# jzr99/Geo4D

Measured on AMD Instinct MI355X. Metric: denoised latent frames/sec (16x320x512, 50-step DDIM), higher is better.
Workload: dtype bf16x3m

## Files before the change

### geo4d_amd/_lib.py

```python
import ctypes as C
import os

import torch

_HERE = os.path.dirname(os.path.abspath(__file__))
LIB_PATH = os.environ.get("GEO4D_HIP_LIB") or os.path.join(_HERE, "csrc", "libgeo4d_hip.so")
ABI_VERSION = 9

F32, BF16, F16, BF16X3, F16X2 = 0, 1, 2, 3, 4


class Geo4DNativeError(RuntimeError):
    pass


class ConvGemm(C.Structure):
    _fields_ = [
        ("A", C.c_void_p), ("W", C.c_void_p), ("O", C.c_void_p),
        ("bias", C.c_void_p), ("rowbias", C.c_void_p), ("R", C.c_void_p),
        ("zeros", C.c_void_p), ("workspace", C.c_void_p), ("workspace_bytes", C.c_size_t),
        ("lda", C.c_long), ("ldw", C.c_long), ("ldo", C.c_long), ("ldr", C.c_long), ("ldrb", C.c_long),
        ("a_bs", C.c_long), ("w_bs", C.c_long), ("o_bs", C.c_long), ("r_bs", C.c_long),
        ("M", C.c_int), ("N", C.c_int), ("K", C.c_int), ("batch", C.c_int),
        ("Cin", C.c_int),
# ... 16 lines not shown
    _fields_ = [("tile_hint", C.c_int), ("generation", C.c_int), ("bm", C.c_int), ("bn", C.c_int), ("wm", C.c_int), ("wn", C.c_int),
                ("geglu", C.c_int)]


class GroupNorm(C.Structure):
    _fields_ = [
        ("x", C.c_void_p), ("y", C.c_void_p), ("gamma", C.c_void_p), ("beta", C.c_void_p),
        ("workspace", C.c_void_p), ("workspace_bytes", C.c_size_t),
        ("ldx", C.c_long), ("ldy", C.c_long),
        ("F", C.c_int), ("HW", C.c_int), ("C", C.c_int), ("groups", C.c_int), ("frames_per_stat", C.c_int),
        ("act", C.c_int), ("dtype", C.c_int), ("eps", C.c_float), ("colsum", C.c_void_p), ("split_out", C.c_int), ("colsum_rows", C.c_int),
        ("sat_count", C.c_void_p),
    ]


class GroupNormSrc(C.Structure):
    _fields_ = [("colsum", C.c_void_p), ("rows", C.c_int), ("c0", C.c_int), ("channels", C.c_int)]


class GroupNorm2(C.Structure):
    _fields_ = [("base", GroupNorm), ("src", GroupNormSrc * 2), ("nsrc", C.c_int), ("path", C.c_int), ("fuse_fraction", C.c_float),
                ("min_workgroups", C.c_int)]


class GroupNormPlan(C.Structure):
    _fields_ = [("path", C.c_int), ("launches", C.c_int), ("rows_per_wg", C.c_int), ("nchunk", C.c_int), ("channel_slices", C.c_int),
                ("stat_slices", C.c_int), ("workspace_bytes", C.c_size_t)]


GN_PATH_AUTO, GN_PATH_PARTIAL, GN_PATH_COLS, GN_PATH_FUSED, GN_PATH_SLICED = 0, 1, 2, 3, 4


class Attention(C.Structure):
    _fields_ = [
        ("q", C.c_void_p), ("o", C.c_void_p),
        ("k", C.c_void_p * 2), ("vt", C.c_void_p * 2), ("zeros", C.c_void_p),
        ("ldq", C.c_long), ("ldo", C.c_long), ("ldk", C.c_long * 2), ("ldvt", C.c_long * 2), ("vt_bs", C.c_long * 2),
        ("Nk", C.c_int * 2), ("kv_div", C.c_int * 2),
        ("B", C.c_int), ("H", C.c_int), ("Nq", C.c_int), ("nseg", C.c_int), ("head_dim", C.c_int), ("dtype", C.c_int),
        ("scale", C.c_float), ("split_out", C.c_int), ("variant", C.c_int), ("qkv_split", C.c_int),
    ]


class AttentionPlan(C.Structure):
    _fields_ = [("kernel", C.c_int), ("nseg", C.c_int), ("qb", C.c_int), ("occ", C.c_int), ("ps", C.c_int), ("rows_per_wg", C.c_int),
                ("grid", C.c_uint * 3), ("variant", C.c_int)]


class Align(C.Structure):
    _fields_ = [
        ("pred", C.c_void_p), ("conf", C.c_void_p), ("logdepth", C.c_void_p), ("cams", C.c_void_p), ("slot_trf", C.c_void_p),
        ("slot_ptr", C.c_void_p), ("slot_idx", C.c_void_p),
        ("grad_logdepth", C.c_void_p), ("img_sums", C.c_void_p), ("slot_sums", C.c_void_p),
        ("workspace", C.c_void_p), ("workspace_bytes", C.c_size_t),
        ("img_part", C.c_void_p), ("slot_part", C.c_void_p),
        ("invdepth", C.c_void_p), ("slot_st", C.c_void_p),
        ("n_imgs", C.c_int), ("n_slots", C.c_int), ("H", C.c_int), ("W", C.c_int), ("chunk_pixels", C.c_int), ("max_slots_per_image", C.c_int),
        ("conf_clamp", C.c_float), ("inv_area", C.c_float), ("depth_weight", C.c_float),
    ]


class AlignSmall(C.Structure):
    _fields_ = [
        ("im_poses", C.c_void_p), ("im_focals", C.c_void_p), ("pw_poses", C.c_void_p), ("cams", C.c_void_p), ("slot_trf", C.c_void_p),
        ("img_sums", C.c_void_p), ("slot_sums", C.c_void_p), ("group_ptr", C.c_void_p), ("group_entries", C.c_void_p), ("group_sums", C.c_void_p),
        ("scale_terms", C.c_void_p),
        ("grad_im_poses", C.c_void_p), ("grad_im_focals", C.c_void_p), ("grad_pw_poses", C.c_void_p), ("grad_s_depth", C.c_void_p),
        ("grad_t_depth", C.c_void_p), ("loss", C.c_void_p),
        ("slot_st", C.c_void_p), ("s_depth", C.c_void_p), ("t_depth", C.c_void_p), ("depth_ok", C.c_void_p),
        ("traj", C.c_void_p), ("traj_align", C.c_void_p), ("traj_valid", C.c_void_p), ("slot_img", C.c_void_p), ("img_slot_ptr", C.c_void_p),
        ("img_slot_idx", C.c_void_p), ("grad_traj", C.c_void_p),
        ("n_imgs", C.c_int), ("n_groups", C.c_int), ("n_slots", C.c_int), ("slots_per_group", C.c_int), ("n_listed_slots", C.c_int),
        ("n_focals", C.c_int), ("norm_pw_scale", C.c_int),
        ("focal_break", C.c_float), ("base_scale", C.c_float), ("ppx", C.c_float), ("ppy", C.c_float), ("smooth_weight", C.c_float),
        ("translation_weight", C.c_float), ("traj_weight", C.c_float),
    ]


SIGNATURES = {
    "geo4d_conv_gemm": (C.c_int, [C.POINTER(ConvGemm), C.c_void_p]),
    "geo4d_conv_gemm_plan": (C.c_int, [C.POINTER(ConvGemm), C.POINTER(ConvGemmPlan)]),
    "geo4d_conv_gemm_tiles": (C.c_int, [C.POINTER(ConvGemmTile), C.c_int]),
    "geo4d_conv_gemm_colsum_rows": (C.c_int, [C.POINTER(ConvGemm)]),
    "geo4d_groupnorm_workspace": (C.c_size_t, [C.c_int, C.c_int, C.c_int, C.c_int]),
    "geo4d_groupnorm": (C.c_int, [C.POINTER(GroupNorm), C.c_void_p]),
    "geo4d_groupnorm_plan": (C.c_int, [C.POINTER(GroupNorm2), C.POINTER(GroupNormPlan)]),
    "geo4d_groupnorm2": (C.c_int, [C.POINTER(GroupNorm2), C.c_void_p]),
    "geo4d_layernorm": (C.c_int, [C.c_void_p, C.c_long, C.c_void_p, C.c_long, C.c_int, C.c_int, C.c_float, C.c_void_p,
                                  C.c_void_p, C.c_int, C.c_void_p]),
    "geo4d_layernorm_split": (C.c_int, [C.c_void_p, C.c_long, C.c_void_p, C.c_long, C.c_int, C.c_int, C.c_float, C.c_void_p,
                                        C.c_void_p, C.c_int, C.c_void_p, C.c_void_p]),
    "geo4d_softmax_rows": (C.c_int, [C.c_void_p, C.c_long, C.c_void_p, C.c_long, C.c_long, C.c_int, C.c_float, C.c_int,
                                     C.c_void_p]),
    "geo4d_softmax_rows_causal": (C.c_int, [C.c_void_p, C.c_long, C.c_void_p, C.c_long, C.c_long, C.c_int, C.c_float, C.c_int,
                                            C.c_int, C.c_void_p]),
    "geo4d_attention_plan": (C.c_int, [C.POINTER(Attention), C.POINTER(AttentionPlan)]),
    "geo4d_attention": (C.c_int, [C.POINTER(Attention), C.c_void_p]),
    "geo4d_temporal_attention": (C.c_int, [C.c_void_p, C.c_long, C.c_void_p, C.c_long, C.c_void_p, C.c_long, C.c_void_p,
                                           C.c_long, C.c_int, C.c_int, C.c_int, C.c_int, C.c_int, C.c_float, C.c_int,
                                           C.c_void_p]),
    "geo4d_temporal_attention2": (C.c_int, [C.c_void_p, C.c_long, C.c_void_p, C.c_long, C.c_void_p, C.c_long, C.c_void_p,
                                            C.c_long, C.c_int, C.c_int, C.c_int, C.c_int, C.c_int, C.c_float, C.c_int,
                                            C.c_int, C.c_void_p]),
    "geo4d_tokens_from_ncthw": (C.c_int, [C.c_void_p, C.c_int, C.c_void_p, C.c_int, C.c_void_p, C.c_int, C.c_int, C.c_int,
                                          C.c_int, C.c_int, C.c_void_p]),
    "geo4d_cast_rows_f16": (C.c_int, [C.c_void_p, C.c_long, C.c_void_p, C.c_long, C.c_long, C.c_int, C.c_void_p, C.c_void_p]),
    "geo4d_split_rows_bf16": (C.c_int, [C.c_void_p, C.c_long, C.c_void_p, C.c_long, C.c_long, C.c_int, C.c_void_p]),
    "geo4d_concat_channels": (C.c_int, [C.c_void_p, C.c_long, C.c_int, C.c_void_p, C.c_long, C.c_int, C.c_void_p, C.c_long,
                                        C.c_long, C.c_int, C.c_void_p]),
    "geo4d_timestep_embedding": (C.c_int, [C.c_void_p, C.c_void_p, C.c_void_p, C.c_int, C.c_int, C.c_void_p]),
    "geo4d_linear_small": (C.c_int, [C.c_void_p, C.c_long, C.c_void_p, C.c_long, C.c_void_p, C.c_void_p, C.c_long,
                                     C.c_void_p, C.c_long, C.c_int, C.c_int, C.c_int, C.c_int, C.c_int, C.c_void_p]),
    "geo4d_ddim_step": (C.c_int, [C.c_void_p, C.c_void_p, C.c_void_p, C.c_void_p, C.c_void_p, C.c_void_p, C.c_long,
                                  C.c_void_p]),
    "geo4d_philox_fill": (C.c_int, [C.c_void_p, C.c_int, C.c_void_p, C.c_int, C.c_long, C.c_void_p, C.c_int, C.c_int, C.c_int, C.c_float,
                                    C.c_void_p]),
    "geo4d_ddim_step_rng": (C.c_int, [C.c_void_p, C.c_void_p, C.c_void_p, C.c_void_p, C.c_void_p, C.c_void_p, C.c_int, C.c_long, C.c_int,
                                      C.c_float, C.c_void_p]),
    "geo4d_cfg_combine_workspace": (C.c_size_t, [C.c_int]),
    "geo4d_cfg_combine": (C.c_int, [C.c_void_p, C.c_void_p, C.c_void_p, C.c_void_p, C.c_int, C.c_long, C.c_float, C.c_float,
                                    C.c_float, C.c_void_p, C.c_size_t, C.c_void_p]),
    "geo4d_embed_tokens": (C.c_int, [C.c_void_p, C.c_void_p, C.c_void_p, C.c_void_p, C.c_long, C.c_long, C.c_int, C.c_int, C.c_int,
                                     C.c_int, C.c_void_p]),
    "geo4d_advance_index": (C.c_int, [C.c_void_p, C.c_int, C.c_void_p]),
    "geo4d_gather_timestep": (C.c_int, [C.c_void_p, C.c_void_p, C.c_void_p, C.c_int, C.c_void_p]),
    "geo4d_plucker_cameras_workspace": (C.c_size_t, [C.c_int, C.c_int, C.c_int]),
    "geo4d_plucker_cameras": (C.c_int, [C.c_void_p, C.c_void_p, C.c_long, C.c_long, C.c_int, C.c_int, C.c_int, C.c_void_p,
                                        C.c_size_t, C.c_void_p, C.c_void_p]),
    "geo4d_align_workspace": (C.c_size_t, [C.c_int, C.c_int, C.c_int, C.c_int, C.c_int]),
    "geo4d_align_residual": (C.c_int, [C.POINTER(Align), C.c_void_p]),
    "geo4d_adam_step": (C.c_int, [C.c_void_p, C.c_void_p, C.c_void_p, C.c_void_p, C.c_long, C.c_float, C.c_float, C.c_float, C.c_float,
                                  C.c_int, C.c_void_p]),
    "geo4d_adam_step_dev": (C.c_int, [C.c_void_p, C.c_void_p, C.c_void_p, C.c_void_p, C.c_long, C.c_void_p, C.c_float, C.c_float, C.c_float,
                                      C.c_void_p]),
    "geo4d_lad_workspace": (C.c_size_t, [C.c_int, C.c_long]),
    "geo4d_lad_target": (C.c_int, [C.c_void_p, C.c_void_p, C.c_void_p, C.c_int, C.c_int, C.c_void_p]),
    "geo4d_lower_median": (C.c_int, [C.c_void_p, C.c_int, C.c_long, C.c_void_p, C.c_void_p, C.c_size_t, C.c_void_p]),
    "geo4d_lad_fit": (C.c_int, [C.c_void_p, C.c_void_p, C.c_int, C.c_long, C.c_void_p, C.c_float, C.c_int, C.c_float, C.c_void_p, C.c_void_p,
                                C.c_void_p, C.c_size_t, C.c_void_p]),
    "geo4d_lad_delta": (C.c_int, [C.c_void_p, C.c_void_p, C.c_void_p, C.c_void_p, C.c_int, C.c_long, C.c_float, C.c_float, C.c_float,
                                  C.c_void_p, C.c_void_p]),
    "geo4d_bicubic_resize": (C.c_int, [C.c_void_p, C.c_void_p, C.c_int, C.c_int, C.c_int, C.c_int, C.c_int, C.c_void_p]),
    "geo4d_masked_select_workspace": (C.c_size_t, [C.c_long]),
    "geo4d_masked_select": (C.c_int, [C.c_void_p, C.c_void_p, C.c_long, C.c_float, C.c_void_p, C.c_float, C.c_float, C.c_void_p, C.c_void_p,
                                      C.c_void_p, C.c_void_p, C.c_size_t, C.c_void_p]),
    "geo4d_depth_metrics_workspace": (C.c_size_t, [C.c_long]),
    "geo4d_depth_metrics": (C.c_int, [C.c_void_p, C.c_void_p, C.c_long, C.c_float, C.c_void_p, C.c_void_p, C.c_float, C.c_float, C.c_float,
                                      C.c_float, C.c_void_p, C.c_void_p, C.c_void_p, C.c_void_p, C.c_size_t, C.c_void_p]),
    "geo4d_scene_clean": (C.c_int, [C.c_void_p, C.c_void_p, C.c_void_p, C.c_void_p, C.c_int, C.c_int, C.c_int, C.c_double, C.c_float, C.c_void_p]),
    "geo4d_scene_points_workspace": (C.c_size_t, [C.c_int, C.c_int, C.c_int]),
    "geo4d_scene_points": (C.c_int, [C.c_void_p, C.c_void_p, C.c_void_p, C.c_int, C.c_int, C.c_int, C.c_void_p, C.c_void_p, C.c_void_p,
                                     C.c_void_p, C.c_size_t, C.c_void_p]),
    "geo4d_scene_mesh_faces_workspace": (C.c_size_t, [C.c_int, C.c_int, C.c_int]),
    "geo4d_scene_mesh_faces": (C.c_int, [C.c_void_p, C.c_int, C.c_int, C.c_int, C.c_void_p, C.c_void_p, C.c_void_p, C.c_size_t, C.c_void_p]),
    "geo4d_focal_shift_workspace": (C.c_size_t, [C.c_int, C.c_int, C.c_int]),
    "geo4d_focal_shift": (C.c_int, [C.c_void_p, C.c_long, C.c_void_p, C.c_long, C.c_float, C.c_void_p, C.c_int, C.c_int, C.c_int, C.c_int,
                                    C.c_int, C.c_int, C.c_void_p, C.c_void_p, C.c_void_p, C.c_void_p, C.c_size_t, C.c_void_p]),
    "geo4d_pnp_ransac_workspace": (C.c_size_t, [C.c_int, C.c_int, C.c_int, C.c_int, C.c_int, C.c_int]),
    "geo4d_pnp_ransac": (C.c_int, [C.c_void_p, C.c_long, C.c_void_p, C.c_long, C.c_float, C.c_void_p, C.c_double, C.c_double, C.c_double,
                                   C.c_int, C.c_int, C.c_void_p, C.c_void_p, C.c_void_p, C.c_void_p, C.c_int, C.c_int, C.c_int, C.c_int,
                                   C.c_int, C.c_void_p, C.c_void_p, C.c_void_p, C.c_void_p, C.c_void_p, C.c_size_t, C.c_void_p]),
    "geo4d_last_error": (C.c_char_p, []),
    "geo4d_align_refresh": (C.c_int, [C.POINTER(AlignSmall), C.c_void_p]),
    "geo4d_align_small_grads": (C.c_int, [C.POINTER(AlignSmall), C.c_void_p]),
    "geo4d_abi_version": (C.c_int, []),
    "geo4d_abi_struct_size": (C.c_size_t, [C.c_int]),
# ... 39 lines not shown
```

### geo4d_amd/csrc/gemm.hip

```cpp
#include "gemm_kernel.h"

namespace geo4d_gemm {
extern template int launch_typed<float>(const geo4d_conv_gemm_t&, const Plan&, hipStream_t);
extern template int launch_typed<bf16_t>(const geo4d_conv_gemm_t&, const Plan&, hipStream_t);
extern template int launch_typed<f16_t>(const geo4d_conv_gemm_t&, const Plan&, hipStream_t);
extern template int launch_typed<bf16x3_t>(const geo4d_conv_gemm_t&, const Plan&, hipStream_t);
extern template int launch_v2_typed<bf16_t>(const geo4d_conv_gemm_t&, const Plan&, hipStream_t);
extern template int launch_v2_typed<bf16x3_t>(const geo4d_conv_gemm_t&, const Plan&, hipStream_t);
extern template int launch_v2_typed<f16x2p_t>(const geo4d_conv_gemm_t&, const Plan&, hipStream_t);
extern template int launch_v3_typed<bf16_t>(const geo4d_conv_gemm_t&, const Plan&, hipStream_t);
extern template int launch_v3_typed<bf16x3_t>(const geo4d_conv_gemm_t&, const Plan&, hipStream_t);
extern template int launch_v3_typed<f16x2p_t>(const geo4d_conv_gemm_t&, const Plan&, hipStream_t);

template <typename T>
static int launch_v23(const geo4d_conv_gemm_t& p, const Plan& plan, hipStream_t s) {
    return generation(plan.hint) == 2 ? launch_v2_typed<T>(p, plan, s) : launch_v3_typed<T>(p, plan, s);
}
}
using namespace geo4d_gemm;

static_assert(MAX_TAPS == MAXTAP, "gemm_plan.h validates the tap count the kernels' gather tables hold");

static int conv_gemm_plan(const geo4d_conv_gemm_t* p, Plan& plan) {
    if (!p) return GEO4D_EINVAL;
    const char* error = validate(*p);
    if (!error) {
        plan = resolve(*p);
        error = plan.error;
    }
    if (error) geo4d_set_error(error);
    return error ? GEO4D_EINVAL : GEO4D_OK;
}

extern "C" int geo4d_conv_gemm(const geo4d_conv_gemm_t* pp, void* stream) {
    Plan plan;
    const int rc = conv_gemm_plan(pp, plan);
    if (rc != GEO4D_OK) return rc;
    const geo4d_conv_gemm_t& p = *pp;
    hipStream_t s = (hipStream_t)stream;
    const bool gen1 = generation(plan.hint) == 1;
    switch (p.dtype) {
        case GEO4D_F32: return launch_typed<float>(p, plan, s);
        case GEO4D_BF16: return gen1 ? launch_typed<bf16_t>(p, plan, s) : launch_v23<bf16_t>(p, plan, s);
        case GEO4D_BF16X3: return gen1 ? launch_typed<bf16x3_t>(p, plan, s) : launch_v23<bf16x3_t>(p, plan, s);
        case GEO4D_F16X2: return launch_v23<f16x2p_t>(p, plan, s);
        default: return launch_typed<f16_t>(p, plan, s);
    }
}

extern "C" int geo4d_conv_gemm_plan(const geo4d_conv_gemm_t* pp, geo4d_conv_gemm_plan_t* out) {
    Plan plan;
    if (!out) return GEO4D_EINVAL;
    const int rc = conv_gemm_plan(pp, plan);
    if (rc != GEO4D_OK) return rc;
    const Tile& t = *find_tile(plan.hint);
    *out = {t.hint, generation(t.hint), t.bm, t.bn, t.wm, t.wn, plan.splits, plan.hot, plan.osplit, plan.colsum_rows};
    return GEO4D_OK;
}

extern "C" int geo4d_conv_gemm_tiles(geo4d_conv_gemm_tile_t* out, int cap) {
    int n = 0;
    for (const Tile& t : TILES) {
        if (out && n < cap) out[n] = {t.hint, generation(t.hint), t.bm, t.bn, t.wm, t.wn, t.geglu()};
        ++n;
    }
    return n;
}

extern "C" int geo4d_conv_gemm_colsum_rows(const geo4d_conv_gemm_t* pp) {
    if (!pp || pp->Hout <= 0 || pp->Wout <= 0) return 0;
    return resolve(*pp).colsum_rows;
}
```

### geo4d_amd/csrc/gemm_epilogue.h

```cpp
#pragma once
#include "common.h"
#include "geo4d_hip.h"

namespace geo4d_gemm {

__device__ __forceinline__ void store_out(void* O, long idx, float v, int dt) {
    if (dt == GEO4D_F32) ((float*)O)[idx] = v;
    else if (dt == GEO4D_BF16) ((unsigned short*)O)[idx] = f32_to_bf16_bits(v);
    else ((unsigned short*)O)[idx] = f32_to_f16_bits(v);
}
__device__ __forceinline__ float load_res(const void* R, long idx, int dt) {
    if (dt == GEO4D_F32) return ((const float*)R)[idx];
    if (dt == GEO4D_BF16) return bf16_bits_to_f32(((const unsigned short*)R)[idx]);
    return f16_bits_to_f32(((const unsigned short*)R)[idx]);
}

struct EpiDest { void* O; long ldo, obase; int odt, oesz, nout; bool geglu; };
__device__ __forceinline__ EpiDest epi_dest(const geo4d_conv_gemm_t& p, const bool partial, const int kz, const long bz) {
    const int odt = partial ? GEO4D_F32 : p.out_dtype;
    void* O = partial ? (void*)((float*)p.workspace + ((long)kz * p.batch + bz) * (long)p.M * p.N) : p.O;
    const bool geglu = !partial && p.act == 2;
    return EpiDest{O, partial ? (long)p.N : p.ldo, partial ? 0 : bz * p.o_bs, odt, odt == GEO4D_F32 ? 4 : 2, geglu ? (p.N >> 1) : p.N, geglu};
}

template <bool GELU = true>
__device__ __forceinline__ float epi_value(const geo4d_conv_gemm_t& p, const float acc, const float brow, const long rboff, const int n, const bool inb = true) {
    float v = acc * p.alpha + brow;
    if (inb) {
        if (p.bias && !p.bias_per_row) v += p.bias[n];
        if (p.rowbias) v += p.rowbias[rboff + n];
    }
    if (p.act == 1) v = silu_f(v);
    else if (GELU && p.act == 3) v = gelu_erf_f(v);
    return v;
}
__device__ __forceinline__ float geglu_value(const float alpha, const float xacc, const float gacc, const float xbias, const float gbias) {
    const float xv = xacc * alpha + xbias;
    const float gv = gacc * alpha + gbias;
    return xv * gelu_erf_f(gv);
}

__device__ __forceinline__ u32x2 pack4_16(const float (&e)[4], const bool isbf) {
    return isbf ? u32x2{f32x2_to_bf16x2(e[0], e[1]), f32x2_to_bf16x2(e[2], e[3])} : u32x2{f32x2_to_f16x2(e[0], e[1]), f32x2_to_f16x2(e[2], e[3])};
}
__device__ __forceinline__ void unpack4_16(const u32x2 r, const bool isbf, float (&f)[4]) {
    if (isbf) {
        f[0] = __uint_as_float(r[0] << 16); f[1] = __uint_as_float(r[0] & 0xffff0000u);
        f[2] = __uint_as_float(r[1] << 16); f[3] = __uint_as_float(r[1] & 0xffff0000u);
    } else {
        f[0] = f16_bits_to_f32((unsigned short)(r[0] & 0xffffu)); f[1] = f16_bits_to_f32((unsigned short)(r[0] >> 16));
        f[2] = f16_bits_to_f32((unsigned short)(r[1] & 0xffffu)); f[3] = f16_bits_to_f32((unsigned short)(r[1] >> 16));
    }
}

constexpr unsigned EPI_OOB = 0x80000000u;
constexpr int EPI_RSRC_FLAGS = 0x00020000;
__device__ __forceinline__ void* uniform_ptr(const void* q) {
    const unsigned long long v = (unsigned long long)q;
    const unsigned lo = __builtin_amdgcn_readfirstlane((unsigned)v), hi = __builtin_amdgcn_readfirstlane((unsigned)(v >> 32));
    return (void*)(((unsigned long long)hi << 32) | lo);
}
__device__ __forceinline__ __amdgpu_buffer_rsrc_t tile_rsrc(const void* corner, const bool present = true) {
    return __builtin_amdgcn_make_buffer_rsrc(uniform_ptr(corner), 0, present ? EPI_OOB : 0u, EPI_RSRC_FLAGS);
}
__device__ __forceinline__ __amdgpu_buffer_rsrc_t bias_rsrc(const geo4d_conv_gemm_t& p, const bool has, const int n_w0) {
    const int nleft = p.N - n_w0;
    return __builtin_amdgcn_make_buffer_rsrc(uniform_ptr(has ? (const void*)(p.bias + n_w0) : p.zeros), 0, (has && nleft > 0) ? (unsigned)nleft * 4u : 0u, EPI_RSRC_FLAGS);
}

struct StoreF32 {
    static constexpr unsigned ES = 4;
    static __device__ __forceinline__ u32x4 pack(const geo4d_conv_gemm_t&, const float (&e)[4]) {
        return u32x4{__float_as_uint(e[0]), __float_as_uint(e[1]), __float_as_uint(e[2]), __float_as_uint(e[3])};
    }
    static __device__ __forceinline__ void store(const u32x4 v, const __amdgpu_buffer_rsrc_t rs, const unsigned off) { __builtin_amdgcn_raw_buffer_store_b128(v, rs, off, 0, 0); }
};
struct StoreSplit {
    static constexpr unsigned ES = 4;
    static __device__ __forceinline__ u32x4 pack(const geo4d_conv_gemm_t&, const float (&e)[4]) {
        unsigned int h0, h1, l0, l1;
        h0 = f32x2_to_bf16x2(e[0], e[1]); h1 = f32x2_to_bf16x2(e[2], e[3]);
        l0 = f32x2_to_bf16x2(e[0] - __uint_as_float(h0 << 16), e[1] - __uint_as_float(h0 & 0xffff0000u));
        l1 = f32x2_to_bf16x2(e[2] - __uint_as_float(h1 << 16), e[3] - __uint_as_float(h1 & 0xffff0000u));
        const u32x2 s0 = __builtin_amdgcn_permlane16_swap(h0, l0, false, false);
        const u32x2 s1 = __builtin_amdgcn_permlane16_swap(h1, l1, false, false);
        return u32x4{s0[0], s1[0], s0[1], s1[1]};
    }
    static __device__ __forceinline__ void store(const u32x4 v, const __amdgpu_buffer_rsrc_t rs, const unsigned off) { __builtin_amdgcn_raw_buffer_store_b128(v, rs, off, 0, 0); }
};
struct StoreRows16 {
    static constexpr unsigned ES = 2;
    static __device__ __forceinline__ bool isbf(const geo4d_conv_gemm_t& p) { return p.out_dtype == GEO4D_BF16; }
    static __device__ __forceinline__ u32x2 pack(const geo4d_conv_gemm_t& p, const float (&e)[4]) { return pack4_16(e, isbf(p)); }
    static __device__ __forceinline__ void store(const u32x2 v, const __amdgpu_buffer_rsrc_t rs, const unsigned off) { __builtin_amdgcn_raw_buffer_store_b64(v, rs, off, 0, 0); }
};
struct StoreF16Sat {
    static constexpr unsigned ES = 2;
    static __device__ __forceinline__ u32x2 pack(const geo4d_conv_gemm_t& p, const float (&e)[4]) {
        count_f16_saturation(p.sat_count, e);
        return pack4_f16_sat(e);
    }
    static __device__ __forceinline__ void store(const u32x2 v, const __amdgpu_buffer_rsrc_t rs, const unsigned off) { __builtin_amdgcn_raw_buffer_store_b64(v, rs, off, 0, 0); }
};

template <int MB, int NB, typename Store>
__device__ __forceinline__ void geglu_fast(const geo4d_conv_gemm_t& p, const f32x4 (&acc)[MB][NB], const void* corner, const long ldo,
// ... 65 lines not shown
```

### geo4d_amd/csrc/gemm_kernel.h

```cpp
#pragma once
#include <type_traits>
#include "common.h"
#include "geo4d_hip.h"
#include "gemm_plan.h"
#include "gemm_epilogue.h"

namespace geo4d_gemm {

constexpr int PITCH = 128;
constexpr int BKC = 8;
constexpr int MAXTAP = 9;
static_assert(BKC * 16 == KSLAB_BYTES, "gemm_plan.h counts K slabs of BKC 16-byte chunks");

template <int BM, int NT>
__device__ __forceinline__ void fill_gather_table(const geo4d_conv_gemm_t& p, const int tm, const int ntap, const int hw, int* rowpix, const int tid) {
    const int hlim = p.ups == 2 ? 2 * p.Hin : p.Hin, wlim = p.ups == 2 ? 2 * p.Win : p.Win;
    const int ush = p.ups == 2 ? 1 : 0;
    for (int e = tid; e < BM * ntap; e += NT) {
        const int row = e / ntap, tap = e - row * ntap;
        const int m = tm * BM + row;
        int pix = -1;
        if (m < p.M) {
            const int f = m / hw, rem = m - f * hw;
            const int oy = rem / p.Wout, ox = rem - oy * p.Wout;
            const int kt = tap / (p.KH * p.KW), r2 = tap - kt * (p.KH * p.KW);
            const int ky = r2 / p.KW, kx = r2 - ky * p.KW;
            const int iy = oy * p.stride - p.ph + ky, ix = ox * p.stride - p.pw + kx;
            const int tt = (f % p.T) + kt - p.pt;
            if ((unsigned)iy < (unsigned)hlim && (unsigned)ix < (unsigned)wlim && (unsigned)tt < (unsigned)p.T)
                pix = ((f + kt - p.pt) * p.Hin + (iy >> ush)) * p.Win + (ix >> ush);
        }
        rowpix[e] = pix;
    }
}
template <int HOT> __device__ __forceinline__ bool a_is_split(const geo4d_conv_gemm_t& p) { return HOT ? (HOT == 2) : (p.a_split != 0); }
template <int HOT> __device__ __forceinline__ bool w_is_split(const geo4d_conv_gemm_t& p) { return HOT ? true : (p.w_split != 0); }

template <int BM, int BN, int WM, int WN, int ST>
constexpr int stage_bytes() {
    constexpr int ring = ST * (BM + BN) * PITCH;
    constexpr int epi = WM * WN * 32 * ((((BN / WN / 32) % 2 == 0) ? 64 : 32) + 4) * 4;
    return ring > epi ? ring : epi;
}
template <int BM, int BN, int WM, int WN, int ST>
constexpr int smem_bytes() {
    return stage_bytes<BM, BN, WM, WN, ST>() + BM * MAXTAP * 4;
}

template <typename T, int BM, int BN, int WM, int WN, int ST, int HOT = 0>
__global__ __launch_bounds__(WM * WN * 64) void conv_gemm_kernel(const geo4d_conv_gemm_t p) {
    constexpr int NT = WM * WN * 64;
    constexpr int EPC = Elem<T>::EPC;
    constexpr int BK = BKC * EPC;
    constexpr int MB = BM / WM / 32, NB = BN / WN / 32;
    constexpr int ACH = BM * BKC / NT, BCH = BN * BKC / NT;
    constexpr int RSTEP = NT / 8;
    constexpr int WTM = MB * 32, WTN = NB * 32;
    constexpr int CG = (NB % 2 == 0) ? 64 : 32;
    constexpr int NG = WTN / CG;
    constexpr int SP = CG + 4;
    static_assert(WM * WN == 4 || WM * WN == 5 || WM * WN == 8 || WM * WN == 10, "4, 5, 8 or 10 waves");
    static_assert((BM * BKC) % NT == 0 && (BN * BKC) % NT == 0 && (NT / 8) % 2 == 0, "staging passes must tile the panel");
    static_assert(MB >= 1 && NB >= 1 && ACH >= 1 && BCH >= 1, "tile too small");
    extern __shared__ __attribute__((aligned(16))) char smem[];
    int* rowpix = (int*)(smem + stage_bytes<BM, BN, WM, WN, ST>());

    const int tid = threadIdx.x, lane = tid & 63, wave = tid >> 6;
    const int li = lane & 31, g = lane >> 5;
    const int wr = wave / WN, wc = wave % WN;
    const long lid = xcd_remap((long)blockIdx.x, (long)gridDim.x);
    const int tiles_n = (p.N + BN - 1) / BN;
    const int tm = (int)(lid / tiles_n), tn = (int)(lid - (long)tm * tiles_n);
    const long bz = blockIdx.y;
    const int kz = blockIdx.z;
    const T* __restrict__ A = (const T*)p.A + bz * p.a_bs;
    const T* __restrict__ W = (const T*)p.W + bz * p.w_bs;
    const int ntap = p.KT * p.KH * p.KW;
    const int hw = p.Hout * p.Wout;

    const bool direct_rows = ntap == 1 && p.stride == 1 && p.ups == 1 && p.ph == 0 && p.pw == 0 && p.pt == 0 &&
                             p.Hin * p.Win == hw;
    if (!direct_rows) {
        fill_gather_table<BM, NT>(p, tm, ntap, hw, rowpix, tid);
        __syncthreads();
    }

    const int ccol = tid & 7;
    const int r0 = tid >> 3;
    const int csrc = (ccol ^ ((r0 >> 1) & 7)) * EPC;
    constexpr bool SWZ_CONST = ((RSTEP / 2) % 8) == 0;
    auto csrc_of = [&](int i) { return SWZ_CONST ? csrc : (ccol ^ (((r0 + i * RSTEP) >> 1) & 7)) * EPC; };
    const T* __restrict__ Z = (const T*)p.zeros;
    const T* wptr[BCH];
#pragma unroll
    for (int i = 0; i < BCH; ++i) {
        const int n = tn * BN + r0 + i * RSTEP;
        wptr[i] = n < p.N ? W + (long)n * p.ldw + csrc_of(i) : nullptr;
    }

    const int nslab_all = p.K / BK;
    const int per = (nslab_all + (int)gridDim.z - 1) / (int)gridDim.z;
    const int s_begin = kz * per;
    const int s_end = min(nslab_all, s_begin + per);
    const int nslab = s_end - s_begin;

    int pix[ACH];
    int tap = s_begin % ntap;
    int c0 = (s_begin / ntap) * BK;
    auto fetch_pix = [&]() {
        if (direct_rows) {
#pragma unroll
            for (int i = 0; i < ACH; ++i) {
                const int m = tm * BM + r0 + i * RSTEP;
                pix[i] = m < p.M ? m : -1;
            }
            return;
// ... 367 lines not shown
    }
    const long rboff = p.rowbias ? (long)(m / p.rowbias_div) * (p.ldrb ? p.ldrb : (long)p.N) : 0;
#pragma unroll
    for (int j = 0; j < 8; ++j) {
        float v = e[j] * p.alpha;
        if (p.bias) v += p.bias[n + j];
        if (p.rowbias) v += p.rowbias[rboff + n + j];
        if (p.R) v += ((const float*)p.R)[(long)m * p.ldr + n + j];
        e[j] = v;
    }
    *(f32x4*)((float*)p.O + (long)m * p.ldo + n) = f32x4{e[0], e[1], e[2], e[3]};
    *(f32x4*)((float*)p.O + (long)m * p.ldo + n + 4) = f32x4{e[4], e[5], e[6], e[7]};
    float q[8];
#pragma unroll
    for (int j = 0; j < 8; ++j) q[j] = e[j] * e[j];
#pragma unroll
    for (int o = CG; o < 64; o <<= 1) {
#pragma unroll
        for (int j = 0; j < 8; ++j) { e[j] += __shfl_xor(e[j], o); q[j] += __shfl_xor(q[j], o); }
    }
    if (lane < CG) {
#pragma unroll
        for (int j = 0; j < 8; ++j) { part[wave][lane * 8 + j][0] = e[j]; part[wave][lane * 8 + j][1] = q[j]; }
    }
    __syncthreads();
    if (tid < CG * 8) {
        float s0 = part[0][tid][0], s1 = part[0][tid][1];
        for (int w2 = 1; w2 < 4; ++w2) { s0 += part[w2][tid][0]; s1 += part[w2][tid][1]; }
        float* dst = p.gn_colsum + ((long)bm * p.N + bn * CG * 8 + tid) * 2;
        dst[0] = s0; dst[1] = s1;
    }
}
template <typename T, bool COLSUM = true>
int launch_splitk_reduce(const geo4d_conv_gemm_t& p, const Plan& plan, hipStream_t stream) {
    if constexpr (COLSUM) {
        if (p.gn_colsum) {
            if (plan.colsum_rows == 32) hipLaunchKernelGGL((splitk_reduce_colsum_kernel<T, 32>), dim3((unsigned)((p.M / 32) * (p.N / 64))), dim3(256), 0, stream, p, plan.splits);
            else hipLaunchKernelGGL((splitk_reduce_colsum_kernel<T, 8>), dim3((unsigned)((p.M / 8) * (p.N / 256))), dim3(256), 0, stream, p, plan.splits);
            GEO4D_CHECK_LAUNCH();
            return GEO4D_OK;
        }
    }
    const long tot = (long)p.batch * p.M * (p.N / 8);
    hipLaunchKernelGGL(splitk_reduce_kernel<T>, dim3((unsigned)((tot + 255) / 256)), dim3(256), 0, stream, p, plan.splits);
    GEO4D_CHECK_LAUNCH();
    return GEO4D_OK;
}

template <typename T, int BM, int BN, int WM, int WN, int ST, int HOT>
int launch_kernel(const geo4d_conv_gemm_t& p, int splits, hipStream_t stream) {
    constexpr int smem = smem_bytes<BM, BN, WM, WN, ST>();
    static bool attr_set = false;
    auto kern = conv_gemm_kernel<T, BM, BN, WM, WN, ST, HOT>;
    if (!attr_set) {
        if (hipFuncSetAttribute((const void*)kern, hipFuncAttributeMaxDynamicSharedMemorySize, smem) != hipSuccess) {
            geo4d_set_error("hipFuncSetAttribute(max dynamic LDS) failed");
            return GEO4D_EIO;
        }
        attr_set = true;
    }
    const long tiles = (long)((p.M + BM - 1) / BM) * ((p.N + BN - 1) / BN);
    dim3 grid((unsigned)tiles, (unsigned)p.batch, (unsigned)splits);
    hipLaunchKernelGGL(kern, grid, dim3(WM * WN * 64), smem, stream, p);
    GEO4D_CHECK_LAUNCH();
    return GEO4D_OK;
}

template <typename T, int BM, int BN, int WM, int WN, int ST>
int launch_cfg(const geo4d_conv_gemm_t& p, const Plan& plan, hipStream_t stream) {
    int rc;
    if constexpr (IsX3<T>::value) {
        if (plan.hot == 1) rc = launch_kernel<T, BM, BN, WM, WN, ST, 1>(p, plan.splits, stream);
        else if (plan.hot == 2) rc = launch_kernel<T, BM, BN, WM, WN, ST, 2>(p, plan.splits, stream);
        else rc = launch_kernel<T, BM, BN, WM, WN, ST, 0>(p, plan.splits, stream);
    } else {
        rc = launch_kernel<T, BM, BN, WM, WN, ST, 0>(p, plan.splits, stream);
    }
    if (rc != GEO4D_OK || plan.splits == 1) return rc;
    return launch_splitk_reduce<T, false>(p, plan, stream);
}

template <typename T> int launch_v2_typed(const geo4d_conv_gemm_t& p, const Plan& plan, hipStream_t stream);
template <typename T> int launch_v3_typed(const geo4d_conv_gemm_t& p, const Plan& plan, hipStream_t stream);

template <typename T>
int launch_typed(const geo4d_conv_gemm_t& p, const Plan& plan, hipStream_t stream) {
    switch (plan.hint) {
        case 1: return launch_cfg<T, 128, 128, 2, 2, 2>(p, plan, stream);
        case 2: return launch_cfg<T, 128, 64, 4, 1, 2>(p, plan, stream);
        case 3: return launch_cfg<T, 64, 128, 2, 2, 2>(p, plan, stream);
        case 4: return launch_cfg<T, 64, 64, 2, 2, 2>(p, plan, stream);
        case 5: return launch_cfg<T, 128, 32, 4, 1, 2>(p, plan, stream);
        case 11: return launch_cfg<T, 256, 128, 4, 2, 2>(p, plan, stream);
        case 13: return launch_cfg<T, 256, 256, 4, 2, 2>(p, plan, stream);
        case 16: return launch_cfg<T, 160, 320, 5, 2, 2>(p, plan, stream);
        case 17: return launch_cfg<T, 160, 160, 5, 1, 2>(p, plan, stream);
    }
    geo4d_set_error("conv_gemm: unknown tile_hint");
    return GEO4D_EINVAL;
}

}
```

### geo4d_amd/csrc/gemm_kernel_v2.h

```cpp
#pragma once
#include "gemm_kernel.h"

namespace geo4d_gemm {

template <typename T> __device__ __forceinline__ void mma16(f32x4& acc, const u32x4& a, const u32x4& b);
template <> __device__ __forceinline__ void mma16<bf16_t>(f32x4& acc, const u32x4& a, const u32x4& b) {
    acc = __builtin_amdgcn_mfma_f32_16x16x32_bf16(__builtin_bit_cast(bf16x8_t, a), __builtin_bit_cast(bf16x8_t, b), acc, 0, 0, 0);
}
template <> __device__ __forceinline__ void mma16<f16_t>(f32x4& acc, const u32x4& a, const u32x4& b) {
    acc = __builtin_amdgcn_mfma_f32_16x16x32_f16(__builtin_bit_cast(f16x8_t, a), __builtin_bit_cast(f16x8_t, b), acc, 0, 0, 0);
}
__device__ __forceinline__ void mma16_x3(f32x4& acc, const u32x4& ah, const u32x4& al, const u32x4& bh, const u32x4& bl) {
    acc = __builtin_amdgcn_mfma_f32_16x16x32_bf16(__builtin_bit_cast(bf16x8_t, al), __builtin_bit_cast(bf16x8_t, bh), acc, 0, 0, 0);
    acc = __builtin_amdgcn_mfma_f32_16x16x32_bf16(__builtin_bit_cast(bf16x8_t, ah), __builtin_bit_cast(bf16x8_t, bl), acc, 0, 0, 0);
    acc = __builtin_amdgcn_mfma_f32_16x16x32_bf16(__builtin_bit_cast(bf16x8_t, ah), __builtin_bit_cast(bf16x8_t, bh), acc, 0, 0, 0);
}

__device__ __forceinline__ void mma16_x2(f32x4& acc, const u32x4& bh, const u32x4& bl, const u32x4& ah) {
    acc = __builtin_amdgcn_mfma_f32_16x16x32_f16(__builtin_bit_cast(f16x8_t, bl), __builtin_bit_cast(f16x8_t, ah), acc, 0, 0, 0);
    acc = __builtin_amdgcn_mfma_f32_16x16x32_f16(__builtin_bit_cast(f16x8_t, bh), __builtin_bit_cast(f16x8_t, ah), acc, 0, 0, 0);
}

template <typename T> __device__ __forceinline__ int swz_key(int row) {
    const int p = (row >> 1) & 7;
    if constexpr (IsX3<T>::value) return p ^ ((((p >> 2) ^ (p >> 1)) & 1) << 1);
    else return p;
}

template <typename T> __device__ __forceinline__ void frag_offsets(const int lr, const int lq, int (&foff)[2]) {
    const int fkey = swz_key<T>(lr);
    if constexpr (IsX3<T>::value) {
        foff[0] = lr * PITCH + (((2 * lq) ^ fkey) << 4);
        foff[1] = lr * PITCH + (((2 * lq + 1) ^ fkey) << 4);
    } else {
        foff[0] = lr * PITCH + ((lq ^ fkey) << 4);
        foff[1] = lr * PITCH + (((4 + lq) ^ fkey) << 4);
    }
}

__device__ __forceinline__ void tile_of(long t, int tiles_n, int tiles_mn, int group_m, int& tm, int& tn) {
    const int tiles_m = tiles_mn / tiles_n;
    if (group_m <= 1 || tiles_n < 2 || tiles_m < 2) {
        tm = (int)(t / tiles_n);
        tn = (int)(t - (long)tm * tiles_n);
        return;
    }
    const int per_band = group_m * tiles_n;
    const int band = (int)(t / per_band);
    const int first_m = band * group_m;
    const int rows = min(tiles_m - first_m, group_m);
    const int r = (int)(t - (long)band * per_band);
    tn = r / rows;
    tm = first_m + (r - tn * rows);
}
__device__ __forceinline__ int tile_group_m(const geo4d_conv_gemm_t& p) { return (p.debug_ablate >= 16 && p.debug_ablate < 48) ? p.debug_ablate - 16 : 1; }

__device__ __forceinline__ int swz_key_a64(int row) { return (4 - ((row >> 2) & 3)) & 3; }
constexpr int PITCH_A64 = 64;

__device__ __forceinline__ float row16_sum(float v) {
    v += __int_as_float(__builtin_amdgcn_mov_dpp(__float_as_int(v), 0xB1, 0xF, 0xF, true));
    v += __int_as_float(__builtin_amdgcn_mov_dpp(__float_as_int(v), 0x4E, 0xF, 0xF, true));
    v += __int_as_float(__builtin_amdgcn_mov_dpp(__float_as_int(v), 0x141, 0xF, 0xF, true));
    v += __int_as_float(__builtin_amdgcn_mov_dpp(__float_as_int(v), 0x140, 0xF, 0xF, true));
    return v;
}
template <int MB, int NB, typename Store>
__device__ __forceinline__ void wide_plain(const geo4d_conv_gemm_t& p, const f32x4 (&acc)[MB][NB], const EpiDest& d, const bool partial, const bool has_res, const long rbase,
                                           const int m_w0, const int n_w0, const int lr, const int lq) {
    constexpr unsigned OOB = EPI_OOB;
    const long ldo = d.ldo;
    const float alpha = partial ? 1.0f : p.alpha;
    const bool hb = !partial && p.bias != nullptr && !p.bias_per_row;
    const bool hr = !partial && p.bias != nullptr && p.bias_per_row;
    const bool ht = !partial && p.rowbias != nullptr;
    const __amdgpu_buffer_rsrc_t rsO = tile_rsrc((float*)d.O + d.obase + (long)m_w0 * ldo + n_w0);
    const __amdgpu_buffer_rsrc_t rsR = tile_rsrc(has_res ? (const void*)((const float*)p.R + rbase + (long)m_w0 * p.ldr + n_w0) : p.zeros, has_res);
    const int mleft = p.M - m_w0;
    const __amdgpu_buffer_rsrc_t rsB = bias_rsrc(p, hb, n_w0);
    const __amdgpu_buffer_rsrc_t rsBr = __builtin_amdgcn_make_buffer_rsrc(
        uniform_ptr(hr ? (const void*)(p.bias + m_w0) : p.zeros), 0, (hr && mleft > 0) ? (unsigned)mleft * 4u : 0u, EPI_RSRC_FLAGS);
    const __amdgpu_buffer_rsrc_t rsT = tile_rsrc(ht ? (const void*)(p.rowbias + n_w0) : p.zeros, ht);
    const unsigned offO = (unsigned)(lr * (int)ldo + 4 * lq) * 4u, offR = (unsigned)(lr * (int)p.ldr + 4 * lq) * 4u;
    const unsigned rowO = (unsigned)ldo * 64u, rowR = (unsigned)p.ldr * 64u;
    const bool gn = !partial && p.gn_colsum != nullptr && m_w0 < p.M;
    const __amdgpu_buffer_rsrc_t rsC = tile_rsrc(gn ? (const void*)(p.gn_colsum + ((long)(m_w0 / (16 * MB)) * p.N + n_w0) * 2) : p.zeros, gn);
    unsigned offT[MB];
#pragma unroll
    for (int a = 0; a < MB; ++a) offT[a] = 0u;
    if (ht) {
        const unsigned ldt = (unsigned)(p.ldrb ? p.ldrb : (long)p.N);
#pragma unroll
        for (int a = 0; a < MB; ++a) {
            const int m = m_w0 + a * 16 + lr;
            offT[a] = ((unsigned)((m < p.M ? m : p.M - 1) / p.rowbias_div) * ldt + 4u * lq) * 4u;
        }
    }
#pragma unroll
    for (int b = 0; b < NB; ++b) {
        const bool colok = n_w0 + 16 * b + 4 * lq < p.N;
        const u32x4 bcu = __builtin_amdgcn_raw_buffer_load_b128(rsB, (unsigned)(4 * lq) * 4u + 64u * b, 0, 0);
        u32x4 ru = __builtin_amdgcn_raw_buffer_load_b128(rsR, ((colok && m_w0 + lr < p.M) ? offR : OOB) + 64u * b, 0, 0);
        u32x4 tu = __builtin_amdgcn_raw_buffer_load_b128(rsT, (colok ? offT[0] : OOB) + 64u * b, 0, 0);
        unsigned bru = __builtin_amdgcn_raw_buffer_load_b32(rsBr, (unsigned)lr * 4u, 0, 0);
        float cs[4] = {0.f, 0.f, 0.f, 0.f}, cq[4] = {0.f, 0.f, 0.f, 0.f};
#pragma unroll
        for (int a = 0; a < MB; ++a) {
            const bool ok = colok && m_w0 + a * 16 + lr < p.M;
            const float brow = __uint_as_float(bru);
            float e[4];
#pragma unroll
            for (int j = 0; j < 4; ++j)
                e[j] = (((acc[a][b][j] * alpha + brow) + __uint_as_float(bcu[j])) + __uint_as_float(tu[j])) + __uint_as_float(ru[j]);
            if (gn) {
#pragma unroll
                for (int j = 0; j < 4; ++j) { cs[j] += e[j]; cq[j] += e[j] * e[j]; }
            }
            const u32x4 c = Store::pack(p, e);
            if (a + 1 < MB) {
                ru = __builtin_amdgcn_raw_buffer_load_b128(rsR, ((colok && m_w0 + (a + 1) * 16 + lr < p.M) ? offR : OOB) + 64u * b, (a + 1) * rowR, 0);
                tu = __builtin_amdgcn_raw_buffer_load_b128(rsT, (colok ? offT[a + 1 < MB ? a + 1 : a] : OOB) + 64u * b, 0, 0);
                bru = __builtin_amdgcn_raw_buffer_load_b32(rsBr, (unsigned)(lr + 16 * (a + 1)) * 4u, 0, 0);
            }
            Store::store(c, rsO, (ok ? offO + a * rowO : OOB) + 64u * b);
        }
        if (gn) {
#pragma unroll
            for (int j = 0; j < 4; ++j) { cs[j] = row16_sum(cs[j]); cq[j] = row16_sum(cq[j]); }
            const unsigned offC = (lr == 0 && colok) ? (unsigned)(16 * b + 4 * lq) * 8u : OOB;
            __builtin_amdgcn_raw_buffer_store_b128(u32x4{__float_as_uint(cs[0]), __float_as_uint(cq[0]), __float_as_uint(cs[1]), __float_as_uint(cq[1])}, rsC, offC, 0, 0);
            __builtin_amdgcn_raw_buffer_store_b128(u32x4{__float_as_uint(cs[2]), __float_as_uint(cq[2]), __float_as_uint(cs[3]), __float_as_uint(cq[3])}, rsC, offC + 16u, 0, 0);
        }
    }
}

template <bool OSPLIT>
__device__ __forceinline__ void store4_generic(const EpiDest& d, const bool vec_ok, const long row, const int col, const float (&e)[4]) {
    const long oidx = row + col;
    if (!vec_ok) {
#pragma unroll
        for (int j = 0; j < 4; ++j) store_out(d.O, oidx + j, e[j], d.odt);
        return;
    }
    if constexpr (OSPLIT) store_split4((float*)d.O + row, col >> 2, e);
    else if (d.odt == GEO4D_F32) *(f32x4*)((float*)d.O + oidx) = f32x4{e[0], e[1], e[2], e[3]};
    else *(u32x2*)((unsigned short*)d.O + oidx) = pack4_16(e, d.odt == GEO4D_BF16);
}

template <int MB, int NB, bool OSPLIT>
__device__ __forceinline__ void generic_rows(const geo4d_conv_gemm_t& p, const f32x4 (&acc)[MB][NB], const EpiDest& d, const bool partial, const bool vec_ok,
                                             const bool has_res, const long rbase, const int m_w0, const int n_w0, const int lr, const int lq) {
    const int odt = d.odt;
#pragma unroll
    for (int a = 0; a < MB; ++a) {
        const int m = m_w0 + a * 16 + lr;
        if (m >= p.M) continue;
        const float brow = (!partial && p.bias && p.bias_per_row) ? p.bias[m] : 0.f;
        const long rboff = (!partial && p.rowbias) ? (long)(m / p.rowbias_div) * (p.ldrb ? p.ldrb : (long)p.N) : 0;
        const long orow = d.obase + (long)m * d.ldo;
        if (d.geglu) {
            if constexpr (NB % 4 == 0) {
#pragma unroll
                for (int b = 0; b < NB; ++b) {
                    if ((b & 3) >= 2) continue;
                    const int n = n_w0 + 16 * b + 4 * lq;
                    if (n + 32 >= p.N) continue;
                    const int oc = (n_w0 >> 1) + 32 * (b >> 2) + 16 * (b & 1) + 4 * lq;
                    float e[4];
#pragma unroll
                    for (int j = 0; j < 4; ++j)
                        e[j] = geglu_value(p.alpha, acc[a][b][j], acc[a][b + 2 < NB ? b + 2 : b][j], p.bias ? p.bias[n + j] : 0.f, p.bias ? p.bias[n + 32 + j] : 0.f);
                    store4_generic<OSPLIT>(d, vec_ok, orow, oc, e);
                }
            }
            continue;
        }
#pragma unroll
        for (int b = 0; b < NB; ++b) {
            const int n = n_w0 + 16 * b + 4 * lq;
            if (n >= p.N) continue;
            float e[4];
#pragma unroll
            for (int j = 0; j < 4; ++j) e[j] = acc[a][b][j];
            if (!partial) {
#pragma unroll
                for (int j = 0; j < 4; ++j) e[j] = epi_value(p, e[j], brow, rboff, n + j, n + j < p.N);
            }
            if (vec_ok) {
                if (has_res) {
                    if (odt == GEO4D_F32) {
                        const f32x4 r = *(const f32x4*)((const float*)p.R + rbase + (long)m * p.ldr + n);
#pragma unroll
                        for (int j = 0; j < 4; ++j) e[j] += r[j];
                    } else {
                        float rf[4];
                        unpack4_16(*(const u32x2*)((const unsigned short*)p.R + rbase + (long)m * p.ldr + n), odt == GEO4D_BF16, rf);
#pragma unroll
                        for (int j = 0; j < 4; ++j) e[j] += rf[j];
                    }
                }
                store4_generic<OSPLIT>(d, true, orow, n, e);
            } else {
#pragma unroll
                for (int j = 0; j < 4; ++j) {
                    if (n + j >= p.N) continue;
                    float v = e[j];
                    if (has_res) v += load_res(p.R, rbase + (long)m * p.ldr + n + j, odt);
                    store_out(d.O, orow + n + j, v, odt);
                }
            }
        }
    }
}

template <typename T, int MB, int NB, bool OSPLIT, bool VECONLY = false>
__device__ __forceinline__ void reg_epilogue(const geo4d_conv_gemm_t& p, const f32x4 (&acc)[MB][NB], const int m_w0, const int n_w0,
                                             const long e_bz, const int e_kz, const bool partial, const int lr, const int lq) {
    const EpiDest d = epi_dest(p, partial, e_kz, e_bz);
    const int odt = d.odt, oesz = d.oesz;
    const bool geglu = d.geglu;
    const bool has_res = !partial && p.R != nullptr;
    const long rbase = e_bz * p.r_bs;
    const bool vec_ok = VECONLY || ((d.nout & 3) == 0 && (d.ldo & 3) == 0 && (((uintptr_t)d.O + d.obase * oesz) % (4 * oesz)) == 0 &&
                                    (!has_res || ((p.ldr & 3) == 0 && (((uintptr_t)p.R + rbase * oesz) % (4 * oesz)) == 0)));
    if constexpr (OSPLIT && IsTwoPass<T>::value) {
        const unsigned short* corner = (unsigned short*)p.O + e_bz * p.o_bs + (long)m_w0 * p.ldo + (geglu ? (n_w0 >> 1) : n_w0);
        if (geglu) geglu_fast<MB, NB, StoreF16Sat>(p, acc, corner, p.ldo, m_w0, n_w0, lr, lq);
        else plain_fast16<MB, NB, false, StoreF16Sat>(p, acc, corner, p.ldo, nullptr, false, m_w0, n_w0, lr, lq);
        return;
    }
    using Wide = std::conditional_t<OSPLIT, StoreSplit, StoreF32>;
    const bool wide = vec_ok && odt == GEO4D_F32;
    if (wide && !geglu && (partial || p.act == 0)) return wide_plain<MB, NB, Wide>(p, acc, d, partial, has_res, rbase, m_w0, n_w0, lr, lq);
    if (wide && geglu) return geglu_fast<MB, NB, Wide>(p, acc, (float*)d.O + d.obase + (long)m_w0 * d.ldo + (n_w0 >> 1), d.ldo, m_w0, n_w0, lr, lq);
    if constexpr (!IsX3<T>::value) {
        const unsigned short* row0 = (unsigned short*)d.O + d.obase + (long)m_w0 * d.ldo;
        if (vec_ok && odt != GEO4D_F32 && !geglu && p.act == 0 && !p.rowbias && !(p.bias && p.bias_per_row))
            return plain_fast16<MB, NB, true, StoreRows16>(p, acc, row0 + n_w0, d.ldo, (const unsigned short*)p.R + rbase + (long)m_w0 * p.ldr + n_w0, has_res, m_w0, n_w0, lr, lq);
        if (vec_ok && odt != GEO4D_F32 && geglu) return geglu_fast<MB, NB, StoreRows16>(p, acc, row0 + (n_w0 >> 1), d.ldo, m_w0, n_w0, lr, lq);
    }
    generic_rows<MB, NB, OSPLIT>(p, acc, d, partial, vec_ok, has_res, rbase, m_w0, n_w0, lr, lq);
}

template <int BM, int BN>
constexpr int v2_smem_bytes() { return (2 * BM + 2 * BN) * PITCH + BM * MAXTAP * 4; }

template <typename T, int BM, int BN, int WM, int WN, int HOT, bool OSPLIT = false>
__global__ __launch_bounds__(WM * WN * 64) void conv_gemm_v2_kernel(const geo4d_conv_gemm_t p, const int splits, const int tiles_mn) {
    constexpr int NT = WM * WN * 64;
    constexpr int EPC = Elem<T>::EPC;
    constexpr int BK = BKC * EPC;
    constexpr int WTM = BM / WM, WTN = BN / WN;
    constexpr int MB = WTM / 16, NB = WTN / 16;
    constexpr int RSTEP = NT / 8;
    constexpr bool A64 = IsTwoPass<T>::value;
    constexpr int RSTEP_A = A64 ? NT / 4 : RSTEP;
    constexpr int ACH = (BM + RSTEP_A - 1) / RSTEP_A, BCH = (BN + RSTEP - 1) / RSTEP;
    constexpr int RING = (2 * BM + 2 * BN) * PITCH;
    static_assert(BM % (WM * 16) == 0 && BN % (WN * 16) == 0 && BM % 8 == 0 && BN % 8 == 0, "wave tiles are multiples of 16");
    static_assert(!std::is_same<T, float>::value, "v2 serves the 16-bit MFMA forms (bf16, bf16x3)");
    extern __shared__ __attribute__((aligned(16))) char smem[];
    int* rowpix = (int*)(smem + RING);

    const int tid = threadIdx.x, lane = tid & 63, wave = tid >> 6;
    const int lr = lane & 15, lq = lane >> 4;
    const int wr = wave / WN, wc = wave % WN;
    const int tiles_n = (p.N + BN - 1) / BN;
    const int ntap = p.KT * p.KH * p.KW;
    const int hw = p.Hout * p.Wout;
    const long total = (long)tiles_mn * p.batch * splits;
    const long G = gridDim.x;
    const bool direct_rows = ntap == 1 && p.stride == 1 && p.ups == 1 && p.ph == 0 && p.pw == 0 && p.pt == 0 && p.Hin * p.Win == hw;
    const int nslab_all = p.K / BK;
    const int per = (nslab_all + splits - 1) / splits;
    const T* __restrict__ Z = (const T*)p.zeros;
    const int ccol = tid & 7;
    const int r0 = tid >> 3;
    const int r0a = A64 ? (tid >> 2) : r0;

    int tm = 0, tn = 0, kz = 0, nslab = 0, tap = 0, c0 = 0, tapB = 0, c0B = 0;
    long bz = 0;
    const T* __restrict__ A = nullptr;
    int pix[ACH];
    const T* wptr[BCH];
    int cA[ACH], cB[BCH];
#pragma unroll
    for (int i = 0; i < ACH; ++i)
        cA[i] = A64 ? ((tid & 3) ^ swz_key_a64(r0a + i * RSTEP_A)) * 16
                    : (ccol ^ swz_key<T>(r0 + i * RSTEP)) * EPC;
#pragma unroll
    for (int i = 0; i < BCH; ++i) cB[i] = (ccol ^ swz_key<T>(r0 + i * RSTEP)) * EPC;

    auto fetch_pix = [&]() {
#pragma unroll
        for (int i = 0; i < ACH; ++i) {
            const int row = r0a + i * RSTEP_A;
            if (direct_rows) {
                const int m = tm * BM + row;
                pix[i] = (row < BM && m < p.M) ? m : -1;
            } else {
                pix[i] = row < BM ? rowpix[row * ntap + tap] : -1;
            }
        }
    };
    auto setup_tile = [&](long w) {
        const long t = w % tiles_mn, rest = w / tiles_mn;
        bz = rest % p.batch;
        kz = (int)(rest / p.batch);
        tile_of(t, tiles_n, tiles_mn, tile_group_m(p), tm, tn);
        A = A64 ? (const T*)((const char*)p.A + bz * p.a_bs * 2) : (const T*)p.A + bz * p.a_bs;
        const T* __restrict__ W = (const T*)p.W + bz * p.w_bs;
#pragma unroll
        for (int i = 0; i < BCH; ++i) {
            const int row = r0 + i * RSTEP, n = tn * BN + row;
            wptr[i] = (row < BN && n < p.N) ? W + (long)n * p.ldw + cB[i] : nullptr;
        }
        const int s_begin = kz * per;
        nslab = min(nslab_all, s_begin + per) - s_begin;
        if (!direct_rows) {
            fill_gather_table<BM, NT>(p, tm, ntap, hw, rowpix, tid);
            __syncthreads();
        }
        tap = tapB = s_begin % ntap;
        c0 = c0B = (s_begin / ntap) * BK;
        fetch_pix();
    };
    auto issue_A = [&](int ab) {
        char* base = smem + ab * BM * PITCH + wave * 1024;
#pragma unroll
        for (int j = 0; j < ACH; ++j) {
            if ((ACH * RSTEP_A == BM) || (wave * (A64 ? 16 : 8) + j * RSTEP_A < BM)) {
                const T* src = pix[j] < 0 ? Z : A64 ? (const T*)((const char*)A + ((long)pix[j] * p.lda + c0) * 2 + cA[j]) : A + (long)pix[j] * p.lda + c0 + cA[j];
                __builtin_amdgcn_global_load_lds((const __attribute__((address_space(1))) void*)src,
                                                 (__attribute__((address_space(3))) void*)(base + j * RSTEP * PITCH), 16, 0, 0);
            }
        }
        if (++tap == ntap) { tap = 0; c0 += BK; }
        if (ntap > 1 && c0 < p.Cin) fetch_pix();
    };
    auto issue_B = [&](int bb) {
        char* base = smem + (2 * BM + bb * BN) * PITCH + wave * 1024;
#pragma unroll
        for (int i = 0; i < BCH; ++i) {
            if ((BCH * RSTEP == BN) || (wave * 8 + i * RSTEP < BN)) {
                const T* src = wptr[i] ? wptr[i] + (long)tapB * p.Cin + c0B : Z;
                __builtin_amdgcn_global_load_lds((const __attribute__((address_space(1))) void*)src,
                                                 (__attribute__((address_space(3))) void*)(base + i * RSTEP * PITCH), 16, 0, 0);
            }
        }
        if (++tapB == ntap) { tapB = 0; c0B += BK; }
    };
    f32x4 acc[MB][NB];
    int foff[2];
    frag_offsets<T>(lr, lq, foff);
    const bool a_split = a_is_split<HOT>(p), w_split = w_is_split<HOT>(p);
    auto compute_slab = [&](int buf) {
        const char* abase = smem + (buf * BM + wr * WTM) * PITCH;
        const char* bbase = smem + (2 * BM + buf * BN + wc * WTN) * PITCH;
        if constexpr (IsTwoPass<T>::value) {
            u32x4 ah[MB];
            const char* abase64 = smem + buf * BM * PITCH + (wr * WTM) * PITCH_A64 + lr * PITCH_A64 + ((lq ^ swz_key_a64(lr)) << 4);
#pragma unroll
            for (int a = 0; a < MB; ++a) ah[a] = *(const u32x4*)(abase64 + a * 16 * PITCH_A64);
#pragma unroll
            for (int b = 0; b < NB; ++b) {
                const u32x4 bh = *(const u32x4*)(bbase + b * 16 * PITCH + foff[0]);
                const u32x4 bl = *(const u32x4*)(bbase + b * 16 * PITCH + foff[1]);
#pragma unroll
                for (int a = 0; a < MB; ++a) mma16_x2(acc[a][b], bh, bl, ah[a]);
            }
        } else if constexpr (IsX3<T>::value) {
            u32x4 ah[MB], al[MB];
#pragma unroll
            for (int a = 0; a < MB; ++a) {
                const u32x4 x0 = *(const u32x4*)(abase + a * 16 * PITCH + foff[0]);
                const u32x4 x1 = *(const u32x4*)(abase + a * 16 * PITCH + foff[1]);
                if (a_split) { ah[a] = x0; al[a] = x1; }
                else split8_bf16(x0, x1, ah[a], al[a]);
            }
#pragma unroll
            for (int b = 0; b < NB; ++b) {
                const u32x4 y0 = *(const u32x4*)(bbase + b * 16 * PITCH + foff[0]);
                const u32x4 y1 = *(const u32x4*)(bbase + b * 16 * PITCH + foff[1]);
                u32x4 bh, bl;
                if (w_split) { bh = y0; bl = y1; }
                else split8_bf16(y0, y1, bh, bl);
#pragma unroll
                for (int a = 0; a < MB; ++a) mma16_x3(acc[a][b], bh, bl, ah[a], al[a]);
            }
        } else {
#pragma unroll
            for (int h = 0; h < 2; ++h) {
                u32x4 fa[MB];
#pragma unroll
                for (int a = 0; a < MB; ++a) fa[a] = *(const u32x4*)(abase + a * 16 * PITCH + foff[h]);
#pragma unroll
                for (int b = 0; b < NB; ++b) {
                    const u32x4 fb = *(const u32x4*)(bbase + b * 16 * PITCH + foff[h]);
#pragma unroll
                    for (int a = 0; a < MB; ++a) mma16<T>(acc[a][b], fb, fa[a]);
                }
            }
        }
    };

    const bool partial = splits > 1;
    auto epilogue = [&](int e_tm, int e_tn, long e_bz, int e_kz) {
        reg_epilogue<T, MB, NB, OSPLIT>(p, acc, e_tm * BM + wr * WTM, e_tn * BN + wc * WTN, e_bz, e_kz, partial, lr, lq);
    };

    long w = xcd_remap((long)blockIdx.x, G);
    if (w >= total) return;
    setup_tile(w);
    auto prologue = [&]() {
        if (nslab > 0) { issue_A(0); issue_B(0); }
    };
    prologue();
    while (true) {
#pragma unroll
        for (int a = 0; a < MB; ++a)
#pragma unroll
            for (int b = 0; b < NB; ++b) acc[a][b] = f32x4{0.f, 0.f, 0.f, 0.f};
        const int ns = nslab;
        asm volatile("s_waitcnt vmcnt(0)" ::: "memory");
        __syncthreads();
        for (int s = 0; s < ns; ++s) {
            const int buf = s & 1;
            if (s + 1 < ns) { issue_A(buf ^ 1); issue_B(buf ^ 1); }
            compute_slab(buf);
            asm volatile("s_waitcnt vmcnt(0)" ::: "memory");
            __syncthreads();
        }
        const int e_tm = tm, e_tn = tn, e_kz = kz;
        const long e_bz = bz;
        const long wn = w + G;
        const bool more = wn < total;
        if (more) {
            setup_tile(wn);
            prologue();
        }
        epilogue(e_tm, e_tn, e_bz, e_kz);
        if (!more) break;
        w = wn;
    }
}

struct GenV2 {
    template <typename T, int BM, int BN, int WM, int WN, int HOT, bool OSPLIT>
    static auto kernel() { return conv_gemm_v2_kernel<T, BM, BN, WM, WN, HOT, OSPLIT>; }
    template <int BM, int BN> static constexpr int smem() { return v2_smem_bytes<BM, BN>(); }
};

template <typename G, typename T, int BM, int BN, int WM, int WN, int HOT, bool OSPLIT = false>
int launch_persistent(const geo4d_conv_gemm_t& p, const Plan& plan, hipStream_t stream) {
    constexpr int smem = G::template smem<BM, BN>();
    static_assert(smem <= 160 * 1024, "LDS");
    static int resident = 0;
    auto kern = G::template kernel<T, BM, BN, WM, WN, HOT, OSPLIT>();
    if (!resident) {
        if (hipFuncSetAttribute((const void*)kern, hipFuncAttributeMaxDynamicSharedMemorySize, smem) != hipSuccess) {
            geo4d_set_error("hipFuncSetAttribute(max dynamic LDS) failed");
            return GEO4D_EIO;
        }
        int dev = 0, cus = 0, occ = 0;
        if (hipGetDevice(&dev) != hipSuccess || hipDeviceGetAttribute(&cus, hipDeviceAttributeMultiprocessorCount, dev) != hipSuccess ||
            hipOccupancyMaxActiveBlocksPerMultiprocessor(&occ, (const void*)kern, WM * WN * 64, smem) != hipSuccess || cus <= 0 || occ <= 0) {
            geo4d_set_error("conv_gemm: occupancy query failed");
            return GEO4D_EIO;
        }
        resident = cus * occ;
    }
    const int tiles_mn = ((p.M + BM - 1) / BM) * ((p.N + BN - 1) / BN);
    const long total = (long)tiles_mn * p.batch * plan.splits;
    const long cap = p.debug_ablate == 2 ? 3 : resident;
    const unsigned grid = (unsigned)(total < cap ? total : cap);
    hipLaunchKernelGGL(kern, dim3(grid), dim3(WM * WN * 64), smem, stream, p, plan.splits, tiles_mn);
    GEO4D_CHECK_LAUNCH();
    if (plan.splits > 1) return launch_splitk_reduce<T>(p, plan, stream);
    return GEO4D_OK;
}

template <typename G, typename T, int BM, int BN, int WM, int WN>
int launch_persistent_cfg(const geo4d_conv_gemm_t& p, const Plan& plan, hipStream_t stream) {
    if constexpr (IsX3<T>::value) {
        if (plan.osplit) return launch_persistent<G, T, BM, BN, WM, WN, 2, true>(p, plan, stream);
        if (plan.hot == 2) return launch_persistent<G, T, BM, BN, WM, WN, 2>(p, plan, stream);
        if constexpr (!IsTwoPass<T>::value) {
            if (plan.hot == 1) return launch_persistent<G, T, BM, BN, WM, WN, 1>(p, plan, stream);
        }
    }
    if constexpr (!IsTwoPass<T>::value) return launch_persistent<G, T, BM, BN, WM, WN, 0>(p, plan, stream);
    return GEO4D_EINVAL;
}

template <typename T>
int launch_v2_typed(const geo4d_conv_gemm_t& p, const Plan& plan, hipStream_t stream) {
    if constexpr (std::is_same<T, bf16_t>::value || IsX3<T>::value) {
        switch (plan.hint) {
            case 22:
                if constexpr (IsTwoPass<T>::value) break;
                else return launch_persistent_cfg<GenV2, T, 256, 256, 4, 2>(p, plan, stream);
            case 23: return launch_persistent_cfg<GenV2, T, 160, 320, 2, 4>(p, plan, stream);
            case 25: return launch_persistent_cfg<GenV2, T, 128, 128, 2, 2>(p, plan, stream);
            case 27: return launch_persistent_cfg<GenV2, T, 64, 128, 2, 2>(p, plan, stream);
            case 28: return launch_persistent_cfg<GenV2, T, 64, 64, 2, 2>(p, plan, stream);
        }
    }
    geo4d_set_error("conv_gemm: no second-generation kernel for this tile_hint and element type");
    return GEO4D_EINVAL;
}

}
```

### geo4d_amd/csrc/gemm_kernel_v3.h

```cpp
#pragma once
#include "gemm_kernel_v2.h"

namespace geo4d_gemm {

template <int BM, int BN>
constexpr int v3_smem_bytes() { return 2 * (BM + BN) * PITCH; }

#define GEO4D_V3_BAR()                          \
    do {                                        \
        __builtin_amdgcn_sched_barrier(0);      \
        __builtin_amdgcn_s_barrier();           \
        __builtin_amdgcn_sched_barrier(0);      \
    } while (0)

template <typename T, int BM, int BN, int WM, int WN, int HOT, bool OSPLIT = false>
__global__ __launch_bounds__(512) void conv_gemm_v3_kernel(const geo4d_conv_gemm_t p, const int splits, const int tiles_mn) {
    static_assert(WM * WN == 8, "two groups of four waves");
    static_assert(!std::is_same<T, float>::value, "v3 serves the 16-bit MFMA forms (bf16, bf16x3)");
    constexpr int EPC = Elem<T>::EPC;
    constexpr int BK = BKC * EPC;
    constexpr int WTM = BM / WM, WTN = BN / WN;
    constexpr int MB = WTM / 16, NB = WTN / 16;
    constexpr int MB0 = (MB + 1) / 2, MB1 = MB - MB0, NB0 = (NB + 1) / 2, NB1 = NB - NB0;
    static_assert(BM % (WM * 16) == 0 && BN % (WN * 16) == 0 && MB1 >= 1 && NB1 >= 1, "wave tiles of at least 32 x 32");
    constexpr int RA0 = WM * MB0 * 16, RA1 = WM * MB1 * 16, RB0 = WN * NB0 * 16, RB1 = WN * NB1 * 16;
    constexpr bool A64 = IsTwoPass<T>::value;
    constexpr int PITCH_A = A64 ? PITCH_A64 : PITCH, RPA = A64 ? 128 : 64, RWA = A64 ? 16 : 8;
    constexpr int OA0 = 0, OA1 = RA0 * PITCH_A, OB0 = BM * PITCH, OB1 = (BM + RB0) * PITCH;
    constexpr int STAGE = (BM + BN) * PITCH;
    constexpr int PA0 = (RA0 + RPA - 1) / RPA, PA1 = (RA1 + RPA - 1) / RPA, PB0 = (RB0 + 63) / 64, PB1 = (RB1 + 63) / 64;
    constexpr int CA0 = RA0 / RPA, CA1 = RA1 / RPA, CB0 = RB0 / 64, CB1 = RB1 / 64;
    constexpr int NWAIT = CA0 + CA1 + CB0 + CB1;
    extern __shared__ __attribute__((aligned(16))) char smem[];

    const int tid = threadIdx.x, lane = tid & 63;
    const int wave = __builtin_amdgcn_readfirstlane(tid >> 6);
    const int lr = lane & 15, lq = lane >> 4;
    const int wr = wave / WN, wc = wave % WN;
    const int tiles_n = (p.N + BN - 1) / BN;
    const int ntap = p.KT * p.KH * p.KW;
    const int hw = p.Hout * p.Wout;
    const long total = (long)tiles_mn * p.batch * splits;
    const long G = gridDim.x;
    const bool direct_rows = ntap == 1 && p.stride == 1 && p.ups == 1 && p.ph == 0 && p.pw == 0 && p.pt == 0 && p.Hin * p.Win == hw;
    const int ns = p.K / BK / splits;
    const int ccol = tid & 7;
    const int r0 = tid >> 3;
    const int r0a = A64 ? (tid >> 2) : r0;

    constexpr unsigned OOB = 0x80000000u;
    constexpr int ESZ = 16 / EPC;
    constexpr int ESZ_A = A64 ? 2 : ESZ;
    auto tile_row = [&](int r, int rows, int per_wave, int wt, int off) { return r < rows ? (r / per_wave) * wt + off + r % per_wave : -1; };
    auto rowA = [&](int h, int j) { return h ? tile_row(r0a + RPA * j, RA1, MB1 * 16, WTM, MB0 * 16) : tile_row(r0a + RPA * j, RA0, MB0 * 16, WTM, 0); };
    auto rowB = [&](int h, int j) { return h ? tile_row(r0 + 64 * j, RB1, NB1 * 16, WTN, NB0 * 16) : tile_row(r0 + 64 * j, RB0, NB0 * 16, WTN, 0); };
    auto chunk = [&](int j) { return (ccol ^ swz_key<T>(r0 + 64 * j)) * EPC; };
    auto chunkA = [&](int j) { return A64 ? ((tid & 3) ^ swz_key_a64(r0a + RPA * j)) * 8 : chunk(j); };
    const int khw = p.KH * p.KW;

    long wS = 0;
    bool validS = false;
    int tmS = 0, tnS = 0, kzS = 0;
    long bzS = 0;
    unsigned voffA[2][PA0], maskA[2][PA0];
    unsigned voffB[2][PB0];
    __amdgpu_buffer_rsrc_t rA = __builtin_amdgcn_make_buffer_rsrc((void*)p.zeros, 0, 0, 0x00020000);
    __amdgpu_buffer_rsrc_t rB = rA;
    int ktA = 0, kyA = 0, kxA = 0, c0A = 0, tapB = 0, c0B = 0, tap_beg = 0, c0_beg = 0;
    unsigned soffA = 0, bitA = 0, soffB = 0;
    auto refresh_A = [&]() {
        soffA = __builtin_amdgcn_readfirstlane((unsigned)((((long)ktA * p.Hin + kyA) * p.Win + kxA) * p.lda + c0A) * ESZ_A);
        bitA = __builtin_amdgcn_readfirstlane((unsigned)((ktA * p.KH + kyA) * p.KW + kxA));
    };
    auto refresh_B = [&]() { soffB = __builtin_amdgcn_readfirstlane((unsigned)(tapB * p.Cin + c0B) * ESZ); };
    auto begin_A = [&]() {
        ktA = tap_beg / khw;
        const int r2 = tap_beg - ktA * khw;
        kyA = r2 / p.KW;
        kxA = r2 - kyA * p.KW;
        c0A = c0_beg;
        refresh_A();
    };
    auto step_A = [&]() {
        if (++kxA == p.KW) {
            kxA = 0;
            if (++kyA == p.KH) {
                kyA = 0;
                if (++ktA == p.KT) {
                    ktA = 0;
                    c0A += BK;
                }
            }
        }
        refresh_A();
    };
    auto step_B = [&]() {
        if (++tapB == ntap) {
            tapB = 0;
            c0B += BK;
        }
        refresh_B();
    };
    auto tap0_pixel = [&](int m) -> long {
        const int f = m / hw, rem = m - f * hw;
        const int oy = rem / p.Wout, ox = rem - oy * p.Wout;
        return ((long)(f - p.pt) * p.Hin + (oy * p.stride - p.ph)) * p.Win + (ox * p.stride - p.pw);
    };
    auto window_A = [&](bool valid, int tm_, long bz_) {
        const long P0 = valid ? tap0_pixel(tm_ * BM) : 0;
        rA = __builtin_amdgcn_make_buffer_rsrc((void*)((const char*)p.A + (bz_ * p.a_bs + P0 * p.lda) * ESZ_A), 0, OOB, 0x00020000);
#pragma unroll
        for (int h = 0; h < 2; ++h) {
#pragma unroll
            for (int j = 0; j < (h ? PA1 : PA0); ++j) {
                const int row = rowA(h, j);
                const int m = tm_ * BM + row;
                unsigned off = 0, mask = 0;
                if (valid && row >= 0 && m < p.M) {
                    const int f = m / hw, rem = m - f * hw;
                    const int oy = rem / p.Wout, ox = rem - oy * p.Wout;
                    const int iy0 = oy * p.stride - p.ph, ix0 = ox * p.stride - p.pw, ft = (f % p.T) - p.pt;
                    const long px0 = ((long)(f - p.pt) * p.Hin + iy0) * p.Win + ix0;
                    off = (unsigned)(((px0 - P0) * p.lda + chunkA(j)) * ESZ_A);
                    unsigned bit = 1;
                    for (int kt = 0; kt < p.KT; ++kt)
                        for (int ky = 0; ky < p.KH; ++ky)
                            for (int kx = 0; kx < p.KW; ++kx, bit <<= 1)
                                if ((unsigned)(ft + kt) < (unsigned)p.T && (unsigned)(iy0 + ky) < (unsigned)p.Hin && (unsigned)(ix0 + kx) < (unsigned)p.Win)
                                    mask |= bit;
                }
                voffA[h][j] = off;
                maskA[h][j] = mask;
            }
        }
    };
    auto stage_tile = [&](long w_) {
        wS = w_;
        validS = w_ < total;
        if (!validS) {
#pragma unroll
            for (int h = 0; h < 2; ++h)
#pragma unroll
                for (int j = 0; j < PB0; ++j) voffB[h][j] = OOB;
            return;
        }
        const long t = w_ % tiles_mn, rest = w_ / tiles_mn;
        bzS = rest % p.batch;
        kzS = (int)(rest / p.batch);
        tile_of(t, tiles_n, tiles_mn, tile_group_m(p), tmS, tnS);
        rB = __builtin_amdgcn_make_buffer_rsrc((void*)((const T*)p.W + bzS * p.w_bs + (long)tnS * BN * p.ldw), 0, OOB, 0x00020000);
#pragma unroll
        for (int h = 0; h < 2; ++h) {
#pragma unroll
            for (int j = 0; j < (h ? PB1 : PB0); ++j) {
                const int row = rowB(h, j);
                voffB[h][j] = (row >= 0 && tnS * BN + row < p.N) ? (unsigned)(((long)row * p.ldw + chunk(j)) * ESZ) : OOB;
            }
        }
        const int s_begin = kzS * ns;
        tap_beg = s_begin % ntap;
        c0_beg = (s_begin / ntap) * BK;
    };
    auto issue_A = [&](auto hc, int st) {
        constexpr int H = decltype(hc)::value;
        constexpr int R = H ? RA1 : RA0;
        char* base = smem + st * STAGE + (H ? OA1 : OA0) + wave * 1024;
#pragma unroll
        for (int j = 0; j < (H ? PA1 : PA0); ++j) {
            if ((j + 1) * RPA <= R || wave * RWA + j * RPA < R) {
                const unsigned v = ((maskA[H][j] >> bitA) & 1u) ? voffA[H][j] : OOB;
                __builtin_amdgcn_raw_ptr_buffer_load_lds(rA, (__attribute__((address_space(3))) void*)(base + j * RPA * PITCH_A), 16, (int)v, (int)soffA, 0, 0);
            }
        }
    };
    auto issue_B = [&](auto hc, int st) {
        constexpr int H = decltype(hc)::value;
        constexpr int R = H ? RB1 : RB0;
        char* base = smem + st * STAGE + (H ? OB1 : OB0) + wave * 1024;
#pragma unroll
        for (int j = 0; j < (H ? PB1 : PB0); ++j) {
            if ((j + 1) * 64 <= R || wave * 8 + j * 64 < R)
                __builtin_amdgcn_raw_ptr_buffer_load_lds(rB, (__attribute__((address_space(3))) void*)(base + j * 64 * PITCH), 16, (int)voffB[H][j], (int)soffB, 0, 0);
        }
    };
    int sA = 0, sB = 0;
    auto advance_B = [&]() {
        if (++sB == ns) {
            sB = 0;
            stage_tile(wS + G);
            tapB = tap_beg;
            c0B = c0_beg;
            refresh_B();
        } else {
            step_B();
        }
    };
    auto advance_A = [&]() {
        if (++sA == ns) {
            sA = 0;
            window_A(validS, tmS, bzS);
            begin_A();
        } else {
            step_A();
        }
// ... 83 lines not shown
        } else {
#pragma unroll
            for (int h = 0; h < 2; ++h) {
#pragma unroll
                for (int b = 0; b < NBH; ++b) {
#pragma unroll
                    for (int a = 0; a < MBH; ++a) mma16<T>(acc[AO + a][BO + b], fb[HB][h][b], fa[HA][h][a]);
                }
            }
        }
    };
    using H0 = std::integral_constant<int, 0>;
    using H1 = std::integral_constant<int, 1>;
    const bool partial = splits > 1;

    const long w0 = xcd_remap((long)blockIdx.x, G);
    if (w0 >= total) return;
    stage_tile(w0);
    window_A(true, tmS, bzS);
    begin_A();
    tapB = tap_beg;
    c0B = c0_beg;
    refresh_B();
    issue_A(H0{}, 0);
    issue_B(H0{}, 0);
    issue_B(H1{}, 0);
    advance_B();
    issue_A(H1{}, 0);
    advance_A();
    issue_A(H0{}, 1);
    issue_B(H1{}, 1);
    issue_B(H0{}, 1);
    advance_B();
    int tmC = tmS, tnC = tnS, kzC = kzS;
    long bzC = bzS;
    asm volatile("s_waitcnt vmcnt(%0)" ::"n"(NWAIT) : "memory");
    __syncthreads();
    read_A(H0{}, smem);
    read_B(H0{}, smem);

    while (true) {
#pragma unroll
        for (int a = 0; a < MB; ++a)
#pragma unroll
            for (int b = 0; b < NB; ++b) acc[a][b] = f32x4{0.f, 0.f, 0.f, 0.f};
        auto slab = [&](auto xc) __attribute__((always_inline)) {
            constexpr int X = decltype(xc)::value, Y = 1 - X;
            using HX = std::integral_constant<int, X>;
            using HY = std::integral_constant<int, Y>;
            const char* sb = smem + X * STAGE;
            const char* so = smem + Y * STAGE;
            auto phase = [&](auto jc, auto issue, auto read, auto split, auto mma, auto after) __attribute__((always_inline)) {
                constexpr int J = decltype(jc)::value;
                constexpr int NW = J == 2 ? 2 * (X ? CB1 : CB0) + CA1 + CA0 : NWAIT;
                issue();
                read();
                split();
                mma();
                after();
                asm volatile("s_waitcnt vmcnt(%0)" ::"n"(NW) : "memory");
            };
            phase(std::integral_constant<int, 0>{}, [&] { issue_A(H1{}, Y); }, [&] { read_B(HY{}, sb); },
                  [&] { split_A(H0{}); split_B(HX{}); }, [&] { mma_quadrant(H0{}, HX{}); }, [&] { advance_A(); });
            GEO4D_V3_BAR();
            phase(std::integral_constant<int, 1>{}, [&] { issue_A(H0{}, X); }, [&] { read_A(H1{}, sb); },
                  [&] { split_B(HY{}); }, [&] { mma_quadrant(H0{}, HY{}); }, [&] {});
            GEO4D_V3_BAR();
            phase(std::integral_constant<int, 2>{}, [&] { issue_B(HX{}, X); }, [&] { read_A(H0{}, so); },
                  [&] { split_A(H1{}); }, [&] { mma_quadrant(H1{}, HY{}); }, [&] {});
            GEO4D_V3_BAR();
            phase(std::integral_constant<int, 3>{}, [&] { issue_B(HY{}, X); }, [&] { read_B(HY{}, so); },
                  [&] {}, [&] { mma_quadrant(H1{}, HX{}); }, [&] { advance_B(); });
        };
        for (int t = 0; t < ns; t += 2) {
            slab(H0{});
            GEO4D_V3_BAR();
            slab(H1{});
            if (t + 2 < ns) GEO4D_V3_BAR();
        }
        GEO4D_V3_BAR();
        {
            int lr_ = lr, lq_ = lq;
            asm volatile("" : "+v"(lr_), "+v"(lq_));
            reg_epilogue<T, MB, NB, OSPLIT, true>(p, acc, tmC * BM + wr * WTM, tnC * BN + wc * WTN, bzC, kzC, partial, lr_, lq_);
        }
        __builtin_amdgcn_s_waitcnt(0x0F70);
        if (!validS) break;
        tmC = tmS; tnC = tnS; kzC = kzS; bzC = bzS;
    }
    asm volatile("s_waitcnt vmcnt(0)" ::: "memory");
}

struct GenV3 {
    template <typename T, int BM, int BN, int WM, int WN, int HOT, bool OSPLIT>
    static auto kernel() { return conv_gemm_v3_kernel<T, BM, BN, WM, WN, HOT, OSPLIT>; }
    template <int BM, int BN> static constexpr int smem() { return v3_smem_bytes<BM, BN>(); }
};

template <typename T>
int launch_v3_typed(const geo4d_conv_gemm_t& p, const Plan& plan, hipStream_t stream) {
    if constexpr (std::is_same<T, bf16_t>::value || IsX3<T>::value) {
        switch (plan.hint) {
            case 71: return launch_persistent_cfg<GenV3, T, 192, 256, 2, 4>(p, plan, stream);
            case 72: return launch_persistent_cfg<GenV3, T, 160, 320, 2, 4>(p, plan, stream);
            case 73: return launch_persistent_cfg<GenV3, T, 256, 128, 2, 4>(p, plan, stream);
            case 74: return launch_persistent_cfg<GenV3, T, 128, 256, 2, 4>(p, plan, stream);
        }
    }
    geo4d_set_error("conv_gemm: no third-generation kernel for this tile_hint and element type");
    return GEO4D_EINVAL;
}

#undef GEO4D_V3_BAR

}
```

### geo4d_amd/csrc/gemm_plan.h

```cpp
#pragma once
#include <cstddef>
#include <cstdint>
#include "geo4d_hip.h"

namespace geo4d_gemm {

constexpr int KSLAB_BYTES = 128;
constexpr int MAX_TAPS = 9;

constexpr int generation(int hint) { return hint >= 71 ? 3 : hint >= 21 ? 2 : 1; }

struct Tile {
    int hint, bm, bn, wm, wn, alt, alt_geglu;
    constexpr bool geglu() const { return (bn / wn) % 64 == 0; }
    constexpr int colsum_rows() const { return generation(hint) == 1 ? 32 : bm / wm; }
};
constexpr Tile TILES[] = {
    {1, 128, 128, 2, 2, 25, 25},  {2, 128, 64, 4, 1, 25, 25},   {3, 64, 128, 2, 2, 27, 27},   {4, 64, 64, 2, 2, 28, 27},    {5, 128, 32, 4, 1, 25, 25},
    {11, 256, 128, 4, 2, 22, 22}, {13, 256, 256, 4, 2, 22, 22}, {16, 160, 320, 5, 2, 23, 22}, {17, 160, 160, 5, 1, 25, 25},
    {22, 256, 256, 4, 2, 23, 25}, {23, 160, 320, 2, 4, 0, 0},   {25, 128, 128, 2, 2, 0, 0},   {27, 64, 128, 2, 2, 0, 0},    {28, 64, 64, 2, 2, 0, 0},
    {71, 192, 256, 2, 4, 22, 22}, {72, 160, 320, 2, 4, 23, 23}, {73, 256, 128, 2, 4, 25, 25}, {74, 128, 256, 2, 4, 25, 25},
};
constexpr int N_SCORED = 5;
constexpr float SCORED_EFF[N_SCORED] = {1.00f, 0.85f, 0.80f, 0.62f, 0.50f};
constexpr int V2_DEFAULT = 25;
constexpr int TWO_PASS_SMALL = 25, TWO_PASS_LARGE = 72, TWO_PASS_LARGE_GEGLU = 71;

inline const Tile* find_tile(int hint) {
    for (const Tile& t : TILES)
        if (t.hint == hint) return &t;
    return nullptr;
}

struct Plan {
    int hint = 0;
    int splits = 1;
    int hot = 0;
    bool osplit = false;
    int colsum_rows = 0;
    const char* error = nullptr;
};

inline bool aligned(const void* ptr, int bytes) { return ((uintptr_t)ptr % bytes) == 0; }

inline bool colsum_gen1_ok(const geo4d_conv_gemm_t& p, int split_k) {
    const int oesz = p.out_dtype == GEO4D_F32 ? 4 : 2;
    return !(p.M % 32) && !(p.N % 8) && !p.out_nchw && p.act != 2 && p.batch == 1 && split_k == 1 && !((p.ldo * oesz) % 16) && aligned(p.O, 16) &&
           (!p.R || (!((p.ldr * oesz) % 16) && aligned(p.R, 16)));
}
inline bool colsum_fast_ok(const geo4d_conv_gemm_t& p, int sp) {
    return sp == 1 && p.act == 0 && !p.o_split && !p.out_nchw && p.batch == 1 && p.out_dtype == GEO4D_F32 && (p.N & 3) == 0 && (p.ldo & 3) == 0 &&
           aligned(p.O, 16) && (!p.R || ((p.ldr & 3) == 0 && aligned(p.R, 16)));
}
inline int splitk_colsum_rows(const geo4d_conv_gemm_t& p, int sp) {
    if (sp <= 1 || p.batch != 1 || p.act != 0 || p.o_split || p.out_nchw || p.out_dtype != GEO4D_F32 || p.bias_per_row || (p.ldo & 3) || !aligned(p.O, 16) ||
        (p.R && !aligned(p.R, 4))) return 0;
    const int hw = p.Hout * p.Wout;
    if (hw % 32 == 0 && p.M % 32 == 0 && p.N % 64 == 0) return 32;
    if (hw % 8 == 0 && p.M % 8 == 0 && p.N % 256 == 0) return 8;
    return 0;
}

inline bool o_split_ok(const geo4d_conv_gemm_t& p, int splits) {
    const long nout = p.act == 2 ? (p.N >> 1) : p.N;
    return splits == 1 && p.w_split && p.a_split && (nout & 7) == 0 && (p.ldo & 7) == 0 && aligned(p.O, 32) &&
           (p.batch == 1 || (p.o_bs & 7) == 0) && (!p.R || ((p.ldr & 3) == 0 && aligned(p.R, 16) && (p.batch == 1 || (p.r_bs & 3) == 0)));
}
inline bool o_f16_ok(const geo4d_conv_gemm_t& p, int splits) {
    const long nout = p.act == 2 ? (p.N >> 1) : p.N;
    return splits == 1 && p.w_split && p.a_split == 2 && (p.act == 0 || p.act == 2) && !p.R && !p.rowbias && !p.bias_per_row && (nout & 7) == 0 && (p.ldo & 7) == 0 &&
           aligned(p.O, 16) && (p.batch == 1 || (p.o_bs & 7) == 0);
}

inline bool v3_native(const geo4d_conv_gemm_t& p, int sp, int nslab, long esz, long esz_a) {
    const bool geglu = sp == 1 && p.act == 2;
    const long nout = geglu ? (p.N >> 1) : p.N;
    const long oesz = (sp > 1 || p.out_dtype == GEO4D_F32) ? 4 : 2;
    bool vec_ok = (nout & 3) == 0;
    if (sp > 1) {
        vec_ok = vec_ok && aligned(p.workspace, 16);
    } else {
        vec_ok = vec_ok && (p.ldo & 3) == 0 && aligned(p.O, 4 * oesz) && (p.batch == 1 || (p.o_bs & 3) == 0);
        if (p.R) vec_ok = vec_ok && (p.ldr & 3) == 0 && aligned(p.R, 4 * oesz) && (p.batch == 1 || (p.r_bs & 3) == 0);
    }
    const long frames = 256 / ((long)p.Hout * p.Wout) + 2 + p.KT;
    const bool window_ok = p.ups == 1 && frames * p.Hin * p.Win * p.lda * esz_a < (1L << 31) && (320L * p.ldw + p.K) * esz < (1L << 31);
    const bool forward = (long)p.Wout - 1 <= p.Win && ((long)(p.Hout - 1) * p.Win + (p.Wout - 1)) * p.stride <= (long)p.Hin * p.Win;
    return !(nslab % sp || ((nslab / sp) & 1) || nslab / sp < 4 || !vec_ok || !window_ok || !forward);
}

inline bool score_tiles(const geo4d_conv_gemm_t& p, int nslab, int& hint, int& splits) {
    const bool can_split = p.workspace && p.act != 2 && !p.out_nchw && (p.N % 8) == 0 && p.split_k != 1;
    int best = -1, best_split = 1;
    float best_score = -1.f;
    for (int i = 0; i < N_SCORED; ++i) {
        const Tile& c = TILES[i];
        if (p.act == 2 && !c.geglu()) continue;
        if (hint && c.hint != hint) continue;
        const double tm = (p.M + c.bm - 1) / c.bm, tn = (p.N + c.bn - 1) / c.bn;
        const double tiles = tm * tn * p.batch;
        const double useful = ((double)p.M * p.N * p.batch) / (tiles * c.bm * c.bn);
        for (int s = 1; s <= 16; s *= 2) {
            if (s > 1 && (!can_split || nslab / s < 8)) break;
            if (p.split_k > 1 && s != p.split_k) continue;
            if (s > 1 && (size_t)s * p.batch * p.M * p.N * 4 > p.workspace_bytes) break;
            const double wgs = tiles * s;
            const double waves = (double)(long)((wgs + 511) / 512);
            const double fill = wgs / (waves * 512);
            const double split_cost = s > 1 ? 0.92 : 1.0;
            const float score = (float)(SCORED_EFF[i] * useful * (0.30 + 0.70 * fill) * split_cost);
            if (score > best_score) { best_score = score; best = i; best_split = s; }
        }
    }
    if (best < 0) return false;
    hint = TILES[best].hint;
    splits = best_split;
    return true;
}

inline const char* validate(const geo4d_conv_gemm_t& p) {
    const int esz = (p.dtype == GEO4D_F32 || p.dtype == GEO4D_BF16X3 || p.dtype == GEO4D_F16X2) ? 4 : 2;
    const int bk = KSLAB_BYTES / esz;
// ... 8 lines not shown
            return "conv_gemm: o_split needs a pre-split x pre-split bf16x3 launch, f32 row-major output, stored columns % 8 == 0, 32-byte aligned rows, no split-K";
    }
    if (p.M <= 0 || p.N <= 0 || p.K <= 0 || p.batch <= 0) return "conv_gemm: empty problem";
    if (p.KT <= 0 || p.KH <= 0 || p.KW <= 0 || p.KT * p.KH * p.KW > MAX_TAPS) return "conv_gemm: at most 9 taps";
    if (p.Cin % bk || p.K != p.Cin * p.KT * p.KH * p.KW) return "conv_gemm: Cin must be a multiple of the 128-byte K slab and K = taps*Cin";
    const int esz_a = p.dtype == GEO4D_F16X2 ? 2 : esz;
    if ((p.lda * esz_a) % 16 || (p.ldw * esz) % 16 || ((uintptr_t)p.A % 16) || ((uintptr_t)p.W % 16) || (p.a_bs * esz_a) % 16 || (p.w_bs * esz) % 16)
        return "conv_gemm: operands must be 16-byte aligned";
    if (p.T <= 0 || p.Hout <= 0 || p.Wout <= 0 || p.Hin <= 0 || p.Win <= 0 || p.M % (p.Hout * p.Wout)) return "conv_gemm: bad geometry";
    if ((p.M / (p.Hout * p.Wout)) % p.T) return "conv_gemm: frames not a multiple of T";
    if ((long)(p.M / (p.Hout * p.Wout)) * p.Hin * p.Win > 2147483647L) return "conv_gemm: more than 2^31 input pixels";
    if (p.ups != 1 && p.ups != 2) return "conv_gemm: ups must be 1 or 2";
    if (p.act == 2 && (p.N % 64 || p.out_nchw || p.R)) return "conv_gemm: GEGLU needs N % 64 == 0, row-major output, no residual";
    if (p.act < 0 || p.act > 3) return "conv_gemm: act must be 0 (none), 1 (SiLU), 2 (GEGLU) or 3 (GELU)";
    if (p.act == 3) {
        const int oesz = p.out_dtype == GEO4D_F32 ? 4 : 2;
        if (p.out_nchw || p.R || (p.N % 8) || ((p.ldo * oesz) % 16) || ((uintptr_t)p.O % 16) || ((p.o_bs * oesz) % 16))
            return "conv_gemm: GELU needs a row-major output with N % 8 == 0, 16-byte aligned rows and no residual";
    }
    if (p.rowbias && p.rowbias_div <= 0) return "conv_gemm: rowbias_div";
    if (p.batch > 65535) return "conv_gemm: batch too large";
    if (!p.zeros || ((uintptr_t)p.zeros % 16)) return "conv_gemm: `zeros` must point at 16 zero bytes (16-byte aligned) in device memory";
    if (p.workspace && ((uintptr_t)p.workspace % 16)) return "conv_gemm: workspace alignment";
    return nullptr;
}

inline Plan resolve(const geo4d_conv_gemm_t& p) {
    Plan pl;
    auto refuse = [&pl](const char* why) { pl.error = why; pl.colsum_rows = 0; return pl; };
    const bool two_pass = p.dtype == GEO4D_F16X2, wide = two_pass || p.dtype == GEO4D_BF16X3;
    const long esz = (wide || p.dtype == GEO4D_F32) ? 4 : 2, esz_a = two_pass ? 2 : esz;
    const int nslab = p.K / (KSLAB_BYTES / (int)esz);
    int hint = p.tile_hint, split_k = p.split_k;
    if (two_pass) {
        if (hint == 0) hint = p.M < 4096 ? TWO_PASS_SMALL : p.act == 2 ? TWO_PASS_LARGE_GEGLU : TWO_PASS_LARGE;
        if (split_k == 0) split_k = 1;
    }
    const Tile* t = find_tile(hint);
    if (generation(hint) == 1 && p.o_split) {
        hint = !t ? V2_DEFAULT : p.act == 2 ? t->alt_geglu : t->alt;
        t = find_tile(hint);
    }
    int gen = generation(hint);
    if (gen > 1 && !wide && p.dtype != GEO4D_BF16)
        return refuse("conv_gemm: tile hints 22..28 and 71..74 serve bf16 / bf16x3 / f16x2 (the exact-f32 and the f16 modes stay on hints 0..17)");
    if (gen > 1 && p.out_nchw) return refuse("conv_gemm: tile hints 22..28 and 71..74 have no NCTHW epilogue");
    if (gen == 1 && hint <= N_SCORED) {
        if (!score_tiles(p, nslab, hint, pl.splits)) return refuse("conv_gemm: no tile configuration (split_k / tile_hint not applicable to this problem?)");
        t = find_tile(hint);
    } else if (split_k > 1) {
        if (!p.workspace || p.act == 2 || (gen == 1 && p.out_nchw) || (p.N % 8) || (size_t)split_k * p.batch * p.M * p.N * 4 > p.workspace_bytes || nslab / split_k < 1)
            return refuse("conv_gemm: split_k not applicable (workspace too small / epilogue not splittable)");
        pl.splits = split_k;
    }
    if (!t) return refuse("conv_gemm: unknown tile_hint");
    if (gen == 3 && !v3_native(p, pl.splits, nslab, esz, esz_a)) {
        t = find_tile(t->alt);
        gen = 2;
    }
    if (gen == 2 && two_pass && t->alt) t = find_tile(p.act == 2 ? t->alt_geglu : t->alt);
    pl.hint = t->hint;
    if (p.act == 2 && !t->geglu()) return refuse("conv_gemm: GEGLU needs wave tiles that are a multiple of 64 columns wide");
    if (p.o_split) {
        if (!wide) return refuse("conv_gemm: o_split is a bf16x3 / f16x2 option");
        if (two_pass ? !o_f16_ok(p, pl.splits) : !o_split_ok(p, pl.splits))
            return refuse(two_pass ? "conv_gemm: o_split = 2 (plain f16 rows out) needs no split-K / residual / row biases / SiLU / GELU, stored columns % 8 == 0 and 16-byte aligned output rows"
                                   : "conv_gemm: o_split needs pre-split x pre-split operands, no split-K, N % 8 == 0 and 32-byte aligned output rows");
        pl.hot = 2;
        pl.osplit = true;
    } else if (two_pass) {
        pl.hot = 2;
    } else if (wide && p.w_split) {
        pl.hot = p.a_split ? 2 : 1;
    }
    if (gen == 1) pl.colsum_rows = colsum_gen1_ok(p, split_k) ? t->colsum_rows() : 0;
    else if (pl.splits > 1) pl.colsum_rows = splitk_colsum_rows(p, pl.splits);
    else pl.colsum_rows = (colsum_fast_ok(p, 1) && p.M % t->colsum_rows() == 0) ? t->colsum_rows() : 0;
    if (p.gn_colsum && (!pl.colsum_rows || (pl.splits == 1 && !aligned(p.gn_colsum, 16))))
        return refuse("conv_gemm: this launch cannot emit gn_colsum (geo4d_conv_gemm_colsum_rows): it needs a row-major 16-byte aligned output, batch 1, no GEGLU, "
                      "M a multiple of the rows per entry; first generation: no split-K; later generations: f32 rows, no activation");
    return pl;
}

}
```

### geo4d_amd/ops.py

```python
import ctypes as C

import torch

from . import _lib
from ._lib import BF16, BF16X3, F16, F16X2, F32, Attention, AttentionPlan, ConvGemm, ConvGemmPlan, ConvGemmTile, GroupNorm2, GroupNormPlan
from .precision import resolve as _resolve_precision

_DT = {torch.float32: F32, torch.bfloat16: BF16, torch.float16: F16}
_TD = {F32: torch.float32, BF16: torch.bfloat16, F16: torch.float16}


def dt_code(dtype):
    try:
        return _DT[dtype]
    except KeyError:
        raise TypeError(f"geo4d_amd: unsupported dtype {dtype} (float32, bfloat16, float16 only)")


def k_align(dtype):
    return 32 if _resolve_precision(dtype).storage == torch.float32 else 64


class X2Weight(torch.Tensor):
    _KEEP = {"to", "clone", "detach", "contiguous", "cuda", "cpu", "pin_memory"}
# ... 233 lines not shown
                         tile_hint=0, split_k=0, x3=False):
    _dev(a, "A", True); _dev(w, "W", True); _dev(out, "out", True)
    for opt, nm in ((bias, "bias"), (rowbias, "rowbias"), (residual, "residual")):
        if opt is not None:
            _dev(opt, nm)
    if isinstance(out, SplitAct) and batch == 1:
        _split_out_ok(out, M)
    a_split, w_split = is_split(a, w), is_split(w, a)
    assert not is_x2_weight(a), "a pack.split_f16 weight is the W operand"
    if isinstance(w, X2Weight):
        assert is_x2_weight(w), "a two-pass weight without its scale"
        assert a.dtype == torch.float16 and not isinstance(a, SplitAct), "a pack.split_f16 weight multiplies plain float16 activation rows (the two-pass form has no raw-f32 launch)"
        assert out.dtype in (torch.float16, torch.float32) and not isinstance(out, SplitAct) and not out_nchw, "the two-pass f16 GEMM writes plain f32 rows or plain f16 rows"
        assert ldw % 2 == 0 and w_bs % 2 == 0
        a_split, w_split = 2, True
        code = F16X2
        alpha = alpha * w._x2_alpha
        ldw, w_bs = ldw // 2, w_bs // 2
    elif isinstance(a, SplitAct) or isinstance(w, SplitAct):
        assert a.dtype == torch.bfloat16 and w.dtype == torch.bfloat16 and lda % 2 == 0 and ldw % 2 == 0 and a_bs % 2 == 0 and w_bs % 2 == 0
        a_split = w_split = True
        code = BF16X3
        lda, a_bs, ldw, w_bs = lda // 2, a_bs // 2, ldw // 2, w_bs // 2
    elif a_split or w_split:
        code = BF16X3
        if a_split:
            assert lda % 2 == 0 and a_bs % 2 == 0
            lda, a_bs = lda // 2, a_bs // 2
        else:
            assert ldw % 2 == 0 and w_bs % 2 == 0
            ldw, w_bs = ldw // 2, w_bs // 2
    else:
        assert a.dtype == w.dtype, (a.dtype, w.dtype)
        code = dt_code(a.dtype)
        if x3:
            assert a.dtype == torch.float32, "x3=True multiplies two f32 operands with the bf16x3 scheme"
            code = BF16X3
    p = ConvGemm()
    p.A, p.W, p.O = a.data_ptr(), w.data_ptr(), out.data_ptr()
    p.bias, p.rowbias, p.R = _ptr(bias), _ptr(rowbias), _ptr(residual)
    if bias is not None:
        assert bias.dtype == torch.float32 and bias.is_contiguous()
    if rowbias is not None:
        assert rowbias.dtype == torch.float32 and rowbias.dim() == 2 and rowbias.stride(1) == 1
        p.ldrb = rowbias.stride(0)
    if residual is not None:
        assert residual.dtype == (torch.float32 if isinstance(out, SplitAct) else out.dtype)
    p.lda, p.ldw, p.ldo, p.ldr = lda, ldw, ldo, ldr
    p.a_bs, p.w_bs, p.o_bs, p.r_bs = a_bs, w_bs, o_bs, r_bs
    p.M, p.N, p.K, p.batch, p.Cin = M, N, K, batch, Cin
    p.T, p.Hin, p.Win, p.Hout, p.Wout = T, Hin, Win, Hout, Wout
    p.KT, p.KH, p.KW, p.pt, p.ph, p.pw, p.stride, p.ups = KT, KH, KW, pt, ph, pw, stride, ups
    p.rowbias_div, p.bias_per_row, p.act = rowbias_div, int(bias_per_row), act
    p.dtype, p.out_dtype, p.out_nchw, p.tile_hint = code, (F32 if code == F16X2 else dt_code(out.dtype)), int(out_nchw), tile_hint
    p.alpha, p.split_k = alpha, split_k
    p.debug_ablate = DEBUG_ABLATE
    p.a_split, p.w_split = int(a_split), int(w_split)
    p.o_split = 1 if isinstance(out, SplitAct) else 2 if (code == F16X2 and out.dtype == torch.float16) else 0
    if p.o_split == 1:
        assert code == BF16X3, "pre-split (bf16 hi | lo) outputs come from bf16x3 launches"
        assert ldo % 2 == 0 and o_bs % 2 == 0
        p.ldo, p.o_bs, p.out_dtype = ldo // 2, o_bs // 2, F32
    elif p.o_split == 2:
        assert residual is None and rowbias is None and not bias_per_row and act in (0, 2), "the f16-row epilogue of the two-pass GEMM: column bias (+ GEGLU) only"
    p.gn_colsum = 0
    p.sat_count = _ptr(SAT_COUNTER) if p.o_split == 2 else 0
    ws, zeros = workspace(a.device)
    p.workspace, p.workspace_bytes, p.zeros = ws.data_ptr(), ws.numel(), zeros.data_ptr()
    return p


def conv_gemm_plan(p):
    plan = ConvGemmPlan()
    _lib.check(_lib.load().geo4d_conv_gemm_plan(C.byref(p), C.byref(plan)), "geo4d_conv_gemm_plan")
    return plan


def _plan_on(p, tile_hint, split_k):
    p.tile_hint, p.split_k = tile_hint, split_k
    plan = ConvGemmPlan()
    return plan if _lib.load().geo4d_conv_gemm_plan(C.byref(p), C.byref(plan)) == 0 else None


def _launch_config(p, launch):
    def may_measure():
        return AUTOTUNE and not torch.cuda.is_current_stream_capturing()
    key = f"{p.dtype}/{p.out_dtype}|{p.M}x{p.N}x{p.K}|c{p.Cin}|t{p.KT}{p.KH}{p.KW}s{p.stride}u{p.ups}|a{p.act}r{int(bool(p.R))}n{p.out_nchw}|b{p.batch}"
    if p.dtype in (BF16X3, F16X2):
        key += f"|x{int(bool(p.a_split))}{p.w_split}" + ("o" if p.o_split else "")
    cfg = _tuned_config(_tune_table(), key, p.dtype, p.a_split, p.w_split, p.o_split, may_measure)
    if cfg is None and may_measure():
        cfg = _autotune(launch, key, lambda tile, split: _plan_on(p, tile, split) is not None)
    cfg = cfg if cfg is not None else (0, 0)
    return _f16_rows_config(cfg, p.act) if p.o_split == 2 else cfg


def _offer_colsums(p, out, tile_hint, split_k):
    def rows_on(tile, split):
        return getattr(_plan_on(p, tile, split), "colsum_rows", 0)
    rows = rows_on(tile_hint, split_k) if (_generation(tile_hint) > 1 or int(GN_FUSED_STATS) >= 2) else 0
    if split_k > 1 and not SPLITK_COLSUM:
        rows = 0
    if rows == 0 and int(GN_FUSED_STATS) >= 2:
        first = (tile_hint if _generation(tile_hint) == 1 else 0), 1
        rows = rows_on(*first)
        if rows > 0:
            tile_hint, split_k = first
    if rows > 0:
        split_k = split_k or 1
        cs = torch.empty((p.M // rows, p.N, 2), device=out.device, dtype=torch.float32)
        p.gn_colsum = cs.data_ptr()
        out._gn_colsum, out._gn_colsum_rows = cs, rows
        out._gn_colsum_tag = (out.data_ptr(), out._version)
    return tile_hint, split_k


def conv_gemm(a, w, out, *, tile_hint=0, split_k=0, gn_stats=False, **problem):
    lib = _lib.load()
    p = conv_gemm_descriptor(a, w, out, tile_hint=tile_hint, split_k=split_k, **problem)
    if getattr(out, "_gn_colsum", None) is not None:
        out._gn_colsum, out._gn_colsum_rows, out._gn_colsum_tag = None, 32, None

    def launch(tile, split):
        p.tile_hint, p.split_k = tile, split
        _lib.check(lib.geo4d_conv_gemm(C.byref(p), _stream()), "geo4d_conv_gemm")

    if tile_hint == 0 and split_k == 0:
        tile_hint, split_k = _launch_config(p, launch)
    if gn_stats and GN_FUSED_STATS and not p.o_split and p.batch == 1 and out.dim() == 2 and out.shape[0] == p.M:
        tile_hint, split_k = _offer_colsums(p, out, tile_hint, split_k)
    if GEMM_TIMELINE is None:
        launch(tile_hint, split_k)
    else:
        _on_timeline(GEMM_TIMELINE, lambda: launch(tile_hint, split_k), 2.0 * p.M * p.N * p.K * p.batch, {BF16X3: 3, F16X2: 2}.get(p.dtype, 1))
    return out


def _out_dtype(x, out_dtype, w=None):
    return out_dtype or (torch.float32 if (isinstance(x, SplitAct) or (w is not None and is_x2_weight(w))) else x.dtype)


def linear(x, w, bias=None, *, residual=None, act=0, out=None, out_dtype=None, alpha=1.0, tile_hint=0, split_k=0, gn_stats=False,
           split_out=False):
    M, K = x.shape[0], act_k(x)
    N = w.shape[0]
    assert kdim(w, x) == K, (w.shape, x.shape)
    if out is None:
        nout = N // 2 if act == 2 else N
        out = new_split(M, nout, x.device, split_fmt(split_out)[1]) if split_out else torch.empty((M, nout), device=x.device, dtype=_out_dtype(x, out_dtype, w))
    return conv_gemm(x, w, out, M=M, N=N, K=K, Cin=K, lda=_ld(x), ldw=_ld(w), ldo=_ld(out), bias=bias,
                     residual=residual, ldr=_ld(residual) if residual is not None else 0, act=act, alpha=alpha,
                     tile_hint=tile_hint, split_k=split_k, gn_stats=gn_stats)


def conv2d(x, w, bias, *, F, Hin, Win, KH, KW, stride=1, pad=0, pad_end=0, ups=1, T=1, rowbias=None, rowbias_div=0,
           residual=None, act=0, out=None, out_dtype=None, out_nchw=False, nchw_channels=None, tile_hint=0, split_k=0, gn_stats=False):
    Cin = act_k(x)
    N = w.shape[0]
    Hs, Ws = Hin * ups, Win * ups
    Hout = (Hs + 2 * pad + pad_end - KH) // stride + 1
    Wout = (Ws + 2 * pad + pad_end - KW) // stride + 1
    M = F * Hout * Wout
    assert x.shape[0] == F * Hin * Win, (x.shape, F, Hin, Win)
    assert kdim(w, x) == KH * KW * Cin, (w.shape, KH, KW, Cin)
    if out is None:
        if out_nchw:
            out = torch.empty((F // T, N, T, Hout, Wout), device=x.device, dtype=out_dtype or torch.float32)
        else:
            out = torch.empty((M, N), device=x.device, dtype=_out_dtype(x, out_dtype, w))
    conv_gemm(x, w, out, M=M, N=N, K=KH * KW * Cin, Cin=Cin, lda=_ld(x), ldw=_ld(w), ldo=(nchw_channels or N) if out_nchw else _ld(out), T=T,
              Hin=Hin, Win=Win, Hout=Hout, Wout=Wout, KH=KH, KW=KW, ph=pad, pw=pad, stride=stride, ups=ups, bias=bias,
              rowbias=rowbias, rowbias_div=rowbias_div, residual=residual,
              ldr=_ld(residual) if residual is not None else 0, act=act, out_nchw=out_nchw, tile_hint=tile_hint,
              split_k=split_k, gn_stats=gn_stats)
    return out, Hout, Wout


def conv_temporal(x, w, bias, *, B, T, HW, residual=None, out=None, gn_stats=False, tile_hint=0, split_k=0):
    Cin = act_k(x)
    N = w.shape[0]
    M = B * T * HW
    assert x.shape[0] == M and kdim(w, x) == 3 * Cin
    if out is None:
        out = torch.empty((M, N), device=x.device, dtype=_out_dtype(x, None, w))
    return conv_gemm(x, w, out, M=M, N=N, K=3 * Cin, Cin=Cin, lda=_ld(x), ldw=_ld(w), ldo=_ld(out), T=T, Hin=HW, Win=1,
                     Hout=HW, Wout=1, KT=3, pt=1, bias=bias, residual=residual,
                     ldr=_ld(residual) if residual is not None else 0, gn_stats=gn_stats, tile_hint=tile_hint, split_k=split_k)


def batched_gemm(a, b, out, *, batch, M, N, K, a_bs, b_bs, o_bs, bias=None, bias_per_row=False, alpha=1.0, x3=False):
    return conv_gemm(a, b, out, M=M, N=N, K=K, Cin=K, lda=_ld(a), ldw=_ld(b), ldo=_ld(out), batch=batch, a_bs=a_bs,
                     w_bs=b_bs, o_bs=o_bs, bias=bias, bias_per_row=bias_per_row, alpha=alpha, x3=x3)


_gn_ws = {}


def _gn_sums(t, stat_rows):
    cs = getattr(t, "_gn_colsum", None)
    if cs is None or getattr(t, "_gn_colsum_tag", None) != (t.data_ptr(), t._version):
        return None
    rows = getattr(t, "_gn_colsum_rows", 32)
    if stat_rows % rows or tuple(cs.shape) != (t.shape[0] // rows, t.shape[1], 2):
        return None
    return cs, rows


def concat_parts(buf, left, right):
    buf._gn_parts = (left, right)


def _gn_sources(x, stat_rows):
    one = _gn_sums(x, stat_rows)
    if one is not None:
        return [(one[0], one[1], 0, x.shape[1])]
    parts = getattr(x, "_gn_parts", None)
    if not parts or not GN_ONE_LAUNCH:
        return []
    src, c0 = [], 0
    for v in parts:
        if v.dim() != 2 or v.shape[0] != x.shape[0] or v.stride() != x.stride() or v.data_ptr() != x.data_ptr() + c0 * x.element_size():
            return []
        sums = _gn_sums(v, stat_rows)
        if sums is None:
            return []
        src.append((sums[0], sums[1], c0, v.shape[1]))
        c0 += v.shape[1]
    return src if c0 == x.shape[1] else []


def _gn_descriptor(x, out, gamma, beta, *, F, HW, eps, groups, frames_per_stat, silu, split_out, sources, path):
    q = GroupNorm2()
    p = q.base
    p.x, p.y, p.gamma, p.beta = x.data_ptr(), out.data_ptr(), gamma.data_ptr(), beta.data_ptr()
    p.ldx, p.ldy = _ld(x), (_ld(out) // 2 if split_out == 1 else _ld(out))
    p.split_out = int(split_out)
    p.sat_count = _ptr(SAT_COUNTER) if split_out == 2 else 0
    p.F, p.HW, p.C, p.groups, p.frames_per_stat = F, HW, x.shape[1], groups, frames_per_stat
    p.act, p.dtype, p.eps = int(silu), dt_code(x.dtype), eps
    q.nsrc = len(sources)
    for i, (cs, rows, c0, nc) in enumerate(sources):
        q.src[i].colsum, q.src[i].rows, q.src[i].c0, q.src[i].channels = cs.data_ptr(), rows, c0, nc
    q.path = path
    q.fuse_fraction, q.min_workgroups = GN_TUNE
    return q


def groupnorm_plan(q):
    plan = GroupNormPlan()
    _lib.check(_lib.load().geo4d_groupnorm_plan(C.byref(q), C.byref(plan)), "geo4d_groupnorm_plan")
    return plan


def groupnorm(x, gamma, beta, *, F, HW, eps, groups=32, frames_per_stat=1, silu=False, out=None, split_out=False, path=None):
    lib = _lib.load()
    _dev(x, "x")
    assert not isinstance(x, SplitAct), "GroupNorm reads plain activations"
    Cc = x.shape[1]
# ... 572 lines not shown
```

### geo4d_amd/pack.py

```python
import torch

from .ops import X2Weight, k_align
from .precision import resolve


def split_bf16(w):
    n, k = w.shape
    assert k % 8 == 0
    w = w.float()
    hi = w.to(torch.bfloat16)
    lo = (w - hi.float()).to(torch.bfloat16)
    return torch.stack([hi.reshape(n, k // 8, 8), lo.reshape(n, k // 8, 8)], dim=2).reshape(n, 2 * k).contiguous()


def split_f16(w):
    n, k = w.shape
    assert k % 8 == 0
    w = w.float()
    amax = float(w.abs().max())
    e = 0 if amax == 0.0 or not torch.isfinite(torch.tensor(amax)) else 13 - int(torch.floor(torch.log2(torch.tensor(amax))))
    e = max(-24, min(24, e))
    ws = w * (2.0 ** e)
    hi = ws.to(torch.float16)
    lo = (ws - hi.float()).to(torch.float16)
    out = torch.stack([hi.reshape(n, k // 8, 8), lo.reshape(n, k // 8, 8)], dim=2).reshape(n, 2 * k).contiguous()
    return X2Weight.wrap(out, 2.0 ** -e)


def pack_conv2d_x2(w, dtype, cin_pad=None):
    co, ci, kh, kw = w.shape
    cp = cin_pad or pad_to(ci, k_align(dtype))
    w = w.permute(0, 2, 3, 1)
    if cp != ci:
        w = torch.nn.functional.pad(w, (0, cp - ci))
    return split_f16(w.reshape(co, kh * kw * cp))


def pack_conv3d_t_x2(w, dtype):
    co, ci, kt, kh, kw = w.shape
    assert kh == 1 and kw == 1
    return split_f16(w.reshape(co, ci, kt).permute(0, 2, 1).reshape(co, kt * ci))


def pack_linear_x2(w, dtype):
    w = w.reshape(w.shape[0], -1)
    kp = pad_to(w.shape[1], k_align(dtype))
    if kp != w.shape[1]:
        w = torch.nn.functional.pad(w, (0, kp - w.shape[1]))
    return split_f16(w)


def pack_geglu_x2(w, b, dtype):
    inner = w.shape[0] // 2
    perm = geglu_perm(inner, w.device)
    return pack_linear_x2(w[perm], dtype), b[perm].float().contiguous()


def cast(w, dtype):
    prec = resolve(dtype)
    return split_bf16(w) if prec.x3 else w.to(prec.storage).contiguous()


def pad_to(n, m):
    return (n + m - 1) // m * m


def pack_linear(w, dtype):
    w = w.reshape(w.shape[0], -1)
    kp = pad_to(w.shape[1], k_align(dtype))
    if kp != w.shape[1]:
        w = torch.nn.functional.pad(w, (0, kp - w.shape[1]))
    return cast(w, dtype)


def pack_conv2d(w, dtype, cin_pad=None):
    co, ci, kh, kw = w.shape
    cp = cin_pad or pad_to(ci, k_align(dtype))
    w = w.permute(0, 2, 3, 1)
    if cp != ci:
        w = torch.nn.functional.pad(w, (0, cp - ci))
    return cast(w.reshape(co, kh * kw * cp), dtype)


def pack_conv3d_t(w, dtype):
    co, ci, kt, kh, kw = w.shape
    assert kh == 1 and kw == 1
    return cast(w.reshape(co, ci, kt).permute(0, 2, 1).reshape(co, kt * ci), dtype)


def geglu_perm(inner, device=None):
    assert inner % 32 == 0
    j = torch.arange(inner // 32, device=device)
    blk = torch.arange(32, device=device)
    val = (j[:, None] * 32 + blk[None, :])
    gate = val + inner
    return torch.cat([val, gate], dim=1).reshape(-1)


def pack_geglu(w, b, dtype):
    inner = w.shape[0] // 2
    perm = geglu_perm(inner, w.device)
    return pack_linear(w[perm], dtype), b[perm].float().contiguous()
```

### geo4d_amd/unet.py

```python
import math
import os

import torch
import torch.nn as nn

from . import ops, pack
from .precision import resolve as resolve_dtype


class ParamTree(nn.Module):

    def __init__(self):
        super().__init__()

    def insert(self, dotted, shape):
        node = self
        parts = dotted.split(".")
        for part in parts[:-1]:
            child = node._modules.get(part)
            if child is None:
                child = ParamTree()
                node.add_module(part, child)
            node = child
        node.register_parameter(parts[-1], nn.Parameter(torch.empty(shape), requires_grad=False))
# ... 218 lines not shown
        P = {}
        f32 = lambda n: sd[n].float().contiguous()

        def norm(p):
            return f32(p + ".weight"), f32(p + ".bias")

        x2 = lambda cls: bool(dt.two_pass(cls) and self.presplit)
        lin_ln = pack.pack_linear_x2 if x2("ln") else pack.pack_linear

        def block(p, cross):
            b = {"x2ln": x2("ln"), "x2ff": x2("ff"), "x2attn": bool(cross and x2("attn")), "x2tattn": bool(not cross and x2("tattn") and x2("ln")),
                 "x2cattn": bool(cross and x2("cattn") and x2("ln"))}
            for a in ("attn1", "attn2"):
                x2o = False
                if a == "attn2" and cross:
                    b[a + ".q"] = lin_ln(sd[f"{p}.{a}.to_q.weight"], dt)
                    x2o = b["x2cattn"]
                elif cross:
                    wqk = torch.cat([sd[f"{p}.{a}.to_q.weight"], sd[f"{p}.{a}.to_k.weight"]], 0)
                    if b["x2attn"]:
                        b[a + ".qk"] = pack.pack_linear_x2(wqk, dt)
                        b[a + ".v"] = pack.pack_linear(sd[f"{p}.{a}.to_v.weight"], "f16")
                        x2o = True
                    else:
                        b[a + ".qk"] = pack.pack_linear(wqk, dt)
                        b[a + ".v"] = pack.pack_linear(sd[f"{p}.{a}.to_v.weight"], dt)
                else:
                    b[a + ".qkv"] = lin_ln(torch.cat([sd[f"{p}.{a}.to_q.weight"], sd[f"{p}.{a}.to_k.weight"],
                                                      sd[f"{p}.{a}.to_v.weight"]], 0), dt)
                    x2o = b["x2tattn"]
                b[a + ".o"] = ((pack.pack_linear_x2 if x2o else pack.pack_linear)(sd[f"{p}.{a}.to_out.0.weight"], dt), f32(f"{p}.{a}.to_out.0.bias"))
            if x2("ff"):
                b["ff1"] = pack.pack_geglu_x2(sd[p + ".ff.net.0.proj.weight"], sd[p + ".ff.net.0.proj.bias"], dt)
                b["ff2"] = (pack.pack_linear_x2(sd[p + ".ff.net.2.weight"], dt), f32(p + ".ff.net.2.bias"))
            else:
                b["ff1"] = pack.pack_geglu(sd[p + ".ff.net.0.proj.weight"], sd[p + ".ff.net.0.proj.bias"], dt)
                b["ff2"] = (pack.pack_linear(sd[p + ".ff.net.2.weight"], dt), f32(p + ".ff.net.2.bias"))
            for n in ("norm1", "norm2", "norm3"):
                b[n] = norm(f"{p}.{n}")
            return b

        emb_w, emb_b, off = [], [], 0
        k_text, k_img, kv_off = [], [], 0
        for L in self.all_layers():
            p, e = L.prefix, {}
            if L.kind == "conv_in":
                e["w"] = pack.pack_conv2d(sd[p + ".weight"], dt); e["b"] = f32(p + ".bias")
                e["cpad"] = pack.pad_to(L.cin, ops.k_align(dt))
            elif L.kind == "res":
                e["gn1"], e["gn2"] = norm(p + ".in_layers.0"), norm(p + ".out_layers.0")
                pk = pack.pack_conv2d_x2 if x2("conv3x3") else pack.pack_conv2d
                e["x2"] = pk is pack.pack_conv2d_x2
                e["w1"], e["b1"] = pk(sd[p + ".in_layers.2.weight"], dt), f32(p + ".in_layers.2.bias")
                e["w2"], e["b2"] = pk(sd[p + ".out_layers.3.weight"], dt), f32(p + ".out_layers.3.bias")
                emb_w.append(sd[p + ".emb_layers.1.weight"].float()); emb_b.append(sd[p + ".emb_layers.1.bias"].float())
                e["emb"] = (off, off + L.cout); off += L.cout
                if L.cin != L.cout:
                    e["skip"] = (pack.pack_linear(sd[p + ".skip_connection.weight"], dt), f32(p + ".skip_connection.bias"))
                if self.cfg["temporal_conv"]:
                    e["tc"] = []
                    e["x2t"] = x2("tconv")
                    pkt = pack.pack_conv3d_t_x2 if e["x2t"] else pack.pack_conv3d_t
                    for name, ci in (("conv1", 2), ("conv2", 3), ("conv3", 3), ("conv4", 3)):
                        q = f"{p}.temopral_conv.{name}"
                        e["tc"].append((norm(q + ".0"), pkt(sd[f"{q}.{ci}.weight"], dt), f32(f"{q}.{ci}.bias")))
            elif L.kind in ("spatial", "temporal"):
                e["norm"] = norm(p + ".norm")
                e["x2in"] = x2("proj_in")
                e["in"] = ((pack.pack_linear_x2 if e["x2in"] else pack.pack_linear)(sd[p + ".proj_in.weight"], dt), f32(p + ".proj_in.bias"))
                e["out"] = (pack.pack_linear(sd[p + ".proj_out.weight"], dt), f32(p + ".proj_out.bias"))
                e["blk"] = block(p + ".transformer_blocks.0", cross=L.kind == "spatial")
                if L.kind == "spatial":
                    a = p + ".transformer_blocks.0.attn2"
                    k_text.append(sd[a + ".to_k.weight"])
                    e["wv_text"] = pack.pack_linear(sd[a + ".to_v.weight"], dt)
                    if self.cfg["image_cross_attention"]:
                        k_img.append(sd[a + ".to_k_ip.weight"])
                        e["wv_img"] = pack.pack_linear(sd[a + ".to_v_ip.weight"], dt)
                    e["kv"] = (kv_off, L.inner); kv_off += L.inner
            elif L.kind == "down":
                e["w"], e["b"] = pack.pack_conv2d(sd[p + ".op.weight"], dt), f32(p + ".op.bias")
            elif L.kind == "up":
                e["w"], e["b"] = pack.pack_conv2d(sd[p + ".conv.weight"], dt), f32(p + ".conv.bias")
            P[p] = e
        P["emb_w"], P["emb_b"] = torch.cat(emb_w, 0).contiguous(), torch.cat(emb_b, 0).contiguous()
        P["k_text"] = pack.pack_linear(torch.cat(k_text, 0), dt)
        P["k_img"] = pack.pack_linear(torch.cat(k_img, 0), dt) if k_img else None
        P["time"] = [f32("time_embed.0.weight"), f32("time_embed.0.bias"), f32("time_embed.2.weight"), f32("time_embed.2.bias")]
        if self.fs_condition:
            P["fps"] = [f32("fps_embedding.0.weight"), f32("fps_embedding.0.bias"), f32("fps_embedding.2.weight"), f32("fps_embedding.2.bias")]
        P["out_gn"] = norm("out.0")
        P["out_w"], P["out_b"] = pack.pack_conv2d(sd["out.2.weight"], dt), f32("out.2.bias")
        half = self.model_channels // 2
        P["freqs"] = torch.exp(-math.log(10000) * torch.arange(0, half, dtype=torch.float32) / half).to(dev)
        self._packed = P
        return P

    def _context_kv(self, P, context, B, T):
        key = (context.data_ptr(), tuple(context.shape), context.dtype, self.compute_dtype)
        hit = self._ctx_cache.get(key)
        if hit is not None and hit["version"] == context._version:
            return hit["kv"]
        L = context.shape[1]
        if L != 77 + 16 * T:
            raise NotImplementedError(f"context length {L} != 77 + 16*T ({77 + 16 * T}): only the per-frame image-token "
                                      "layout of Geo4D inference (openaimodel3d.py:576-580) has a HIP path")
        dt = self.storage_dtype
        ctx = context.to(dt)
        text = ctx[:, :77].reshape(B * 77, -1).contiguous()
        img = ctx[:, 77:].reshape(B * T * 16, -1).contiguous()
        if hit is None:
            k_t = k_i = None
            vt_t, vt_i = {}, {}
        else:
            k_t, k_i, vt_t, vt_i = hit["kv"][:4]
        k_t = ops.linear(text, P["k_text"], out=k_t)
        k_i = ops.linear(img, P["k_img"], out=k_i) if P["k_img"] is not None else None
        for L in self.all_layers():
            if L.kind != "spatial":
                continue
            e = P[L.prefix]
            v = vt_t.get(L.prefix)
            if v is None:
                v = vt_t[L.prefix] = torch.zeros((B, L.inner, 80), device=ctx.device, dtype=dt)
            for b in range(B):
                ops.linear_t(e["wv_text"], text[b * 77:(b + 1) * 77], out=v[b])
            if k_i is not None:
                vt_i[L.prefix] = ops.linear_t(e["wv_img"], img, out=vt_i.get(L.prefix))
        h16 = hit["kv"][5] if hit is not None else {}
        if self.compute_dtype.two_pass("cattn") and self.compute_dtype.two_pass("ln") and self.presplit:
            def half(name, t):
                if t is None:
                    return None
                c = h16.get(name)
                if c is None:
                    c = h16[name] = torch.empty(t.shape, device=t.device, dtype=torch.float16)
                c.copy_(t)
                return c
            half("k_t", k_t); half("k_i", k_i)
            for pfx, v in vt_t.items():
                half("vt_t." + pfx, v)
            for pfx, v in vt_i.items():
                half("vt_i." + pfx, v)
        kv = (k_t, k_i, vt_t, vt_i, context, h16)
        if hit is None:
            if len(self._ctx_cache) >= 8:
                self._ctx_cache.pop(next(iter(self._ctx_cache)))
                self.generation += 1
            self._ctx_cache[key] = {"version": context._version, "kv": kv}
        else:
            hit["version"] = context._version
        return kv

    def prepare_context(self, context, T):
        P = self._packed or self._pack()
        kv = self._context_kv(P, context, context.shape[0], T)
        return (self.generation, kv[0].data_ptr())

    def _res(self, e, L, h, emb_all, B, T, H, W, out=None):
        F_, HW = B * T, H * W
        sp = self.presplit
        sp3 = "f16" if e.get("x2") else sp
        a = ops.groupnorm(h, *e["gn1"], F=F_, HW=HW, eps=1e-5, silu=True, split_out=sp3)
        lo, hi = e["emb"]
        h1, _, _ = ops.conv2d(a, e["w1"], e["b1"], F=F_, Hin=H, Win=W, KH=3, KW=3, pad=1, rowbias=emb_all[:, lo:hi],
                              rowbias_div=T * HW, gn_stats=True)
# ... 5 lines not shown
            spt = "f16" if e.get("x2t") else sp
            for i, (gn, w, b) in enumerate(e["tc"]):
                a = ops.groupnorm(y, *gn, F=F_, HW=HW, eps=1e-5, frames_per_stat=T, silu=True, split_out=spt)
                y = ops.conv_temporal(a, w, b, B=B, T=T, HW=HW, residual=h2 if i == 3 else None, gn_stats=True, out=out if i == 3 else None)
            h2 = y
        return h2

    def _ff(self, blk, x):
        sp = "f16" if blk.get("x2ff") else self.presplit
        g = ops.linear(ops.layernorm(x, *blk["norm3"], split_out=sp), *blk["ff1"], act=2, split_out=sp)
        return ops.linear(g, *blk["ff2"], residual=x)

    def _spatial(self, e, L, h, kv, B, T, H, W, out=None):
        F_, N, C_, heads = B * T, H * W, L.inner, L.heads
        blk = e["blk"]
        sp = self.presplit
        x = ops.linear(ops.groupnorm(h, *e["norm"], F=F_, HW=N, eps=1e-6, split_out="f16" if e.get("x2in") else sp), *e["in"])
        x3 = self.compute_dtype.x3
        if blk.get("x2attn"):
            n1 = ops.layernorm(x, *blk["norm1"], split_out="f16")
            qk = ops.linear(n1, blk["attn1.qk"], split_out="f16")
            vt, npad = ops.linear_t_batched(blk["attn1.v"], n1, F_, N)
            att = ops.attention(qk[:, :C_], [(qk[:, C_:], vt.reshape(-1, npad), N, 1, C_ * npad)], B=F_, H=heads, Nq=N, scale=0.125)
        elif sp and N % 8 == 0:
            n1 = ops.layernorm(x, *blk["norm1"], split_out=sp)
            qk = ops.linear(n1, blk["attn1.qk"], split_out=True)
            vt, npad = ops.linear_t_batched(blk["attn1.v"], n1, F_, N, split_out=True)
            att = ops.attention(qk[:, :2 * C_], [(qk[:, 2 * C_:], vt.reshape(-1, 2 * npad), N, 1, C_ * 2 * npad)], B=F_, H=heads, Nq=N,
                                scale=0.125, x3=True, split_out=sp, qkv_split=True)
        else:
            n1 = ops.layernorm(x, *blk["norm1"], split_out=sp)
            qk = ops.linear(n1, blk["attn1.qk"])
            vt, npad = ops.linear_t_batched(blk["attn1.v"], n1, F_, N)
            att = ops.attention(qk[:, :C_], [(qk[:, C_:], vt.reshape(-1, npad), N, 1, C_ * npad)], B=F_, H=heads, Nq=N, scale=0.125, x3=x3, split_out=sp)
        x = ops.linear(att, *blk["attn1.o"], residual=x)
        c16 = blk.get("x2cattn")
        q = ops.linear(ops.layernorm(x, *blk["norm2"], split_out="f16" if blk.get("x2ln") else sp), blk["attn2.q"], split_out="f16" if c16 else False)
        k_t, k_i, vt_t, vt_i, _, h16 = kv
        off, _ = e["kv"]
        if c16:
            sets = [(h16["k_t"][:, off:off + C_], h16["vt_t." + L.prefix].reshape(-1, 80), 77, T, C_ * 80)]
            if k_i is not None:
                sets.append((h16["k_i"][:, off:off + C_], h16["vt_i." + L.prefix], 16, 1, 16))
            att = ops.attention(q, sets, B=F_, H=heads, Nq=N, scale=0.125)
        else:
            sets = [(k_t[:, off:off + C_], vt_t[L.prefix].reshape(-1, 80), 77, T, C_ * 80)]
            if k_i is not None:
                sets.append((k_i[:, off:off + C_], vt_i[L.prefix], 16, 1, 16))
            att = ops.attention(q, sets, B=F_, H=heads, Nq=N, scale=0.125, x3=x3, split_out=sp)
        x = ops.linear(att, *blk["attn2.o"], residual=x)
        x = self._ff(blk, x)
        return ops.linear(x, *e["out"], residual=h, gn_stats=True, out=out)

    def _temporal(self, e, L, h, B, T, H, W, out=None):
        F_, HW, C_, heads = B * T, H * W, L.inner, L.heads
        blk = e["blk"]
        sp = self.presplit
        x = ops.linear(ops.groupnorm(h, *e["norm"], F=F_, HW=HW, eps=1e-6, frames_per_stat=T, split_out="f16" if e.get("x2in") else sp), *e["in"])
        t16 = blk.get("x2tattn")
        for a, n in (("attn1", "norm1"), ("attn2", "norm2")):
            qkv = ops.linear(ops.layernorm(x, *blk[n], split_out="f16" if blk.get("x2ln") else sp), blk[a + ".qkv"], split_out="f16" if t16 else False)
            att = ops.temporal_attention(qkv[:, :C_], qkv[:, C_:2 * C_], qkv[:, 2 * C_:], B=B, T=T, HW=HW, H=heads, scale=0.125, split_out=False if t16 else sp)
            x = ops.linear(att, *blk[a + ".o"], residual=x)
        x = self._ff(blk, x)
        return ops.linear(x, *e["out"], residual=h, gn_stats=True, out=out)

    def _run(self, P, layers, h, emb_all, kv, B, T, H, W, out=None):
        for L in layers:
            e = P[L.prefix]
            o = None
            if out is not None and L is layers[-1]:
                Ho, Wo = ((H - 1) // 2 + 1, (W - 1) // 2 + 1) if L.kind == "down" else (2 * H, 2 * W) if L.kind == "up" else (H, W)
                o = out(B * T * Ho * Wo)
            if L.kind == "res":
                h = self._res(e, L, h, emb_all, B, T, H, W, out=o)
            elif L.kind == "spatial":
                h = self._spatial(e, L, h, kv, B, T, H, W, out=o)
            elif L.kind == "temporal":
                h = self._temporal(e, L, h, B, T, H, W, out=o)
            elif L.kind == "down":
                h, H, W = ops.conv2d(h, e["w"], e["b"], F=B * T, Hin=H, Win=W, KH=3, KW=3, stride=2, pad=1, gn_stats=True, out=o)
            elif L.kind == "up":
                a = ops.presplit(h) if (self.presplit and PRESPLIT_UP) else h
                h, H, W = ops.conv2d(a, e["w"], e["b"], F=B * T, Hin=H, Win=W, KH=3, KW=3, pad=1, ups=2, out=o)
        return h, H, W

    @torch.no_grad()
    def forward(self, x, timesteps, context=None, features_adapter=None, fs=None, task=None, c_concat=None, **kwargs):
        if features_adapter is not None or task is not None:
            raise NotImplementedError("features_adapter / task conditioning are not part of Geo4D inference")
        if timesteps.dim() != 1:
            raise NotImplementedError("per-frame timesteps (2-D) have no HIP path")
        P = self._packed or self._pack()
        B, C0, T, H, W = x.shape
        C1 = 0 if c_concat is None else c_concat.shape[1]
        assert C0 + C1 == self.in_channels, f"expected {self.in_channels} input channels, got {C0}+{C1}"
        if T > 16:
            raise NotImplementedError("temporal_length > 16 has no HIP path (configs/inference_geo4d.yaml:89)")
        dt = self.storage_dtype
        inputs, middle, outputs, init_attn, _ = self.layout
        t_emb = ops.timestep_embedding(timesteps.to(torch.int64), P["freqs"])
        w0, b0, w2, b2 = P["time"]
        emb = ops.linear_small(ops.linear_small(t_emb, w0, b0, act_out=True), w2, b2)
        if self.fs_condition:
            if fs is None:
                fs = torch.full((B,), self.default_fs, dtype=torch.int64, device=x.device)
            w0, b0, w2, b2 = P["fps"]
            f_emb = ops.timestep_embedding(fs.to(torch.int64), P["freqs"])
            emb = ops.linear_small(ops.linear_small(f_emb, w0, b0, act_out=True), w2, b2, add=emb)
        emb_all = ops.linear_small(emb, P["emb_w"], P["emb_b"], act_in=True)
        kv = self._context_kv(P, context, B, T)
        e0 = P[inputs[0][0].prefix]
        h = ops.tokens_from_ncthw(x.float().contiguous(), None if c_concat is None else c_concat.float().contiguous(), e0["cpad"], dt)
        n_in = len(inputs)
        cats = {}
        halves = {}

        def half(j, left):
            if not FUSED_CONCAT or j >= len(outputs):
                return None
            ccat = outputs[j][0].cin

            def view(rows, j=j, left=left, ccat=ccat):
                buf = cats.get(j)
                if buf is None:
                    buf = cats[j] = torch.empty((rows, ccat), device=x.device, dtype=dt)
                assert buf.shape[0] == rows, "latent height/width must be multiples of 8"
                cs = skip_ch[n_in - 1 - j]
                v = buf[:, :ccat - cs] if left else buf[:, ccat - cs:]
                halves[(j, left)] = v
                if (j, True) in halves and (j, False) in halves:
                    ops.concat_parts(buf, halves[(j, True)], halves[(j, False)])
                return v
            return view
        skip_ch = [blk[-1].cout if blk[-1].kind != "temporal" and blk[-1].kind != "spatial" else blk[-1].cin for blk in inputs]
        o0 = half(n_in - 1, False)
        if init_attn is not None:
            h, _, _ = ops.conv2d(h, e0["w"], e0["b"], F=B * T, Hin=H, Win=W, KH=3, KW=3, pad=1, gn_stats=True)
            h = self._temporal(P[init_attn.prefix], init_attn, h, B, T, H, W, out=None if o0 is None else o0(B * T * H * W))
        else:
            h, _, _ = ops.conv2d(h, e0["w"], e0["b"], F=B * T, Hin=H, Win=W, KH=3, KW=3, pad=1, gn_stats=True, out=None if o0 is None else o0(B * T * H * W))
        hs = [(h, H, W)]
        for i, blk in enumerate(inputs[1:], start=1):
            h, H, W = self._run(P, blk, h, emb_all, kv, B, T, H, W, out=half(n_in - 1 - i, False))
            hs.append((h, H, W))
        h, H, W = self._run(P, middle, h, emb_all, kv, B, T, H, W, out=half(0, True))
        for j, blk in enumerate(outputs):
            s, sh, sw = hs.pop()
            assert (sh, sw) == (H, W), "latent height/width must be multiples of 8"
            hc = cats.pop(j) if j in cats else ops.concat_channels(h, s)
            h, H, W = self._run(P, blk, hc, emb_all, kv, B, T, H, W, out=half(j + 1, True))
        a = ops.groupnorm(h, *P["out_gn"], F=B * T, HW=H * W, eps=1e-5, silu=True, split_out=self.presplit)
        y, _, _ = ops.conv2d(a, P["out_w"], P["out_b"], F=B * T, Hin=H, Win=W, KH=3, KW=3, pad=1, T=T, out_nchw=True,
                             out_dtype=torch.float32)
        return y if x.dtype == torch.float32 else y.to(x.dtype)
```

### geo4d_amd/vae.py

```python
import torch

from . import ops, pack
from .posterior import DiagonalGaussianDistribution
from .unet import ParamTree, init_params_, resolve_dtype


def _resnet_shapes(add, p, cin, cout):
    add(p + ".norm1.weight", (cin,)); add(p + ".norm1.bias", (cin,))
    add(p + ".conv1.weight", (cout, cin, 3, 3)); add(p + ".conv1.bias", (cout,))
    add(p + ".norm2.weight", (cout,)); add(p + ".norm2.bias", (cout,))
    add(p + ".conv2.weight", (cout, cout, 3, 3)); add(p + ".conv2.bias", (cout,))
    if cin != cout:
        add(p + ".nin_shortcut.weight", (cout, cin, 1, 1)); add(p + ".nin_shortcut.bias", (cout,))


def _attn_shapes(add, p, c):
    add(p + ".norm.weight", (c,)); add(p + ".norm.bias", (c,))
    for n in ("q", "k", "v", "proj_out"):
        add(f"{p}.{n}.weight", (c, c, 1, 1)); add(f"{p}.{n}.bias", (c,))


def decoder_plan(dd):
    ch, mult, nres = dd["ch"], list(dd["ch_mult"]), dd["num_res_blocks"]
    block_in = ch * mult[-1]
# ... 55 lines not shown
        add("quant_conv.weight", (2 * embed_dim, 2 * zc, 1, 1)); add("quant_conv.bias", (2 * embed_dim,))
        add("post_quant_conv.weight", (zc, embed_dim, 1, 1)); add("post_quant_conv.bias", (zc,))
        if self.adaptorconfig is not None:
            ad = self.adaptorconfig
            assert len(ad["ch_mult"]) == 1
            ach = ad["ch"] * ad["ch_mult"][0]
            add("encoder_adaptor.conv_in.weight", (ad["ch"], ad["in_channels"], 3, 3)); add("encoder_adaptor.conv_in.bias", (ad["ch"],))
            for b in range(ad["num_res_blocks"]):
                _resnet_shapes(add, f"encoder_adaptor.down.0.block.{b}", ad["ch"] if b == 0 else ach, ach)
            add("encoder_adaptor.norm_out.weight", (ach,)); add("encoder_adaptor.norm_out.bias", (ach,))
            add("encoder_adaptor.conv_out.weight", (ad["in_channels"], ach, 3, 3)); add("encoder_adaptor.conv_out.bias", (ad["in_channels"],))
            for b in range(ad["num_res_blocks"] + 1):
                _resnet_shapes(add, f"decoder_adaptor.up.0.block.{b}", ach, ach)
            add("decoder_adaptor.norm_out.weight", (ach,)); add("decoder_adaptor.norm_out.bias", (ach,))
            add("decoder_adaptor.conv_out.weight", (ad["out_ch"], ach, 3, 3)); add("decoder_adaptor.conv_out.bias", (ad["out_ch"],))
        init_params_(self)
        self._packed = None
        self.register_load_state_dict_post_hook(lambda module, incompatible: module.invalidate())
        if ckpt_path is not None:
            sd = torch.load(ckpt_path, map_location="cpu")
            sd = sd.get("state_dict", sd)
            sd = {k: v for k, v in sd.items() if not any(k.startswith(i) for i in ignore_keys)}
            self.load_state_dict(sd, strict=False)

    def invalidate(self):
        self._packed = None

    def set_compute_dtype(self, d):
        self.compute_dtype = resolve_dtype(d)
        self.invalidate()
        return self

    @property
    def storage_dtype(self):
        return self.compute_dtype.storage

    def _apply(self, fn, *a, **k):
        self.invalidate()
        return super()._apply(fn, *a, **k)

    @torch.no_grad()
    def _pack(self):
        sd = dict(self.named_parameters())
        dev = sd["decoder.conv_in.weight"].device
        if dev.type != "cuda":
            raise ops._lib.Geo4DNativeError("geo4d_amd.AutoencoderKL runs only on a HIP device: call .cuda() first "
                                            "(there is no CPU fallback)")
        ops._lib.load()
        dt = self.compute_dtype
        ka = ops.k_align(dt)
        f32 = lambda n: sd[n].float().contiguous()
        norm = lambda p: (f32(p + ".weight"), f32(p + ".bias"))
        P = {}
        zc = self.ddconfig["z_channels"]
        wq = torch.zeros((ka, ka), device=dev)
        wq[:zc, : self.embed_dim] = sd["post_quant_conv.weight"].reshape(zc, self.embed_dim)
        bq = torch.zeros((ka,), device=dev)
        bq[:zc] = sd["post_quant_conv.bias"]
        P["pq"] = (pack.cast(wq, dt), bq.contiguous())
        P["cpad"] = ka
        P["conv_in"] = (pack.pack_conv2d(sd["decoder.conv_in.weight"], dt, cin_pad=ka), f32("decoder.conv_in.bias"))

        def resnet(p, two_pass=False):
            pk = pack.pack_conv2d_x2 if (two_pass and dt.two_pass("vae3x3") and self.presplit) else pack.pack_conv2d
            e = dict(gn1=norm(p + ".norm1"), gn2=norm(p + ".norm2"),
                     c1=(pk(sd[p + ".conv1.weight"], dt), f32(p + ".conv1.bias")),
                     c2=(pk(sd[p + ".conv2.weight"], dt), f32(p + ".conv2.bias")))
            e["x2"] = pk is pack.pack_conv2d_x2
            if (p + ".nin_shortcut.weight") in sd:
                e["nin"] = (pack.pack_linear(sd[p + ".nin_shortcut.weight"], dt), f32(p + ".nin_shortcut.bias"))
            return e
        for kind, p, ci, co in self.plan:
            if kind == "res":
                P[p] = resnet(p, two_pass=True)
            elif kind == "attn":
                P[p] = dict(norm=norm(p + ".norm"),
                            qk=(pack.pack_linear(torch.cat([sd[p + ".q.weight"], sd[p + ".k.weight"]], 0), dt),
                                torch.cat([sd[p + ".q.bias"], sd[p + ".k.bias"]]).float().contiguous()),
                            v=(pack.pack_linear(sd[p + ".v.weight"], dt), f32(p + ".v.bias")),
                            o=(pack.pack_linear(sd[p + ".proj_out.weight"], dt), f32(p + ".proj_out.bias")))
            else:
                up2 = bool(dt.two_pass("vaeup") and self.presplit)
                P[p] = ((pack.pack_conv2d_x2 if up2 else pack.pack_conv2d)(sd[p + ".weight"], dt), f32(p + ".bias"))
        P["head"] = (norm("decoder.norm_out"), pack.pack_conv2d(sd["decoder.conv_out.weight"], dt), f32("decoder.conv_out.bias"))
        P["head_mean"] = (P["head"][0], pack.pack_conv2d(sd["decoder.conv_out.weight"].mean(0, keepdim=True), dt),
                          sd["decoder.conv_out.bias"].mean().reshape(1).float().contiguous())
        if self.adaptorconfig is not None:
            nb = self.adaptorconfig["num_res_blocks"] + 1
            P["adaptor"] = [resnet(f"decoder_adaptor.up.0.block.{b}", two_pass=True) for b in range(nb)]
            P["adaptor_head"] = (norm("decoder_adaptor.norm_out"), pack.pack_conv2d(sd["decoder_adaptor.conv_out.weight"], dt),
                                 f32("decoder_adaptor.conv_out.bias"))
        ch, mult, nres = self.ddconfig["ch"], list(self.ddconfig["ch_mult"]), self.ddconfig["num_res_blocks"]
        P["enc_in"] = (pack.pack_conv2d(sd["encoder.conv_in.weight"], dt, cin_pad=ka), f32("encoder.conv_in.bias"))
        enc = []
        for lvl in range(len(mult)):
            for b in range(nres):
                enc.append(("res", resnet(f"encoder.down.{lvl}.block.{b}")))
            if lvl != len(mult) - 1:
                q = f"encoder.down.{lvl}.downsample.conv"
                enc.append(("down", (pack.pack_conv2d(sd[q + ".weight"], dt), f32(q + ".bias"))))
        enc.append(("res", resnet("encoder.mid.block_1")))
        p = "encoder.mid.attn_1"
        enc.append(("attn", dict(norm=norm(p + ".norm"),
                                 qk=(pack.pack_linear(torch.cat([sd[p + ".q.weight"], sd[p + ".k.weight"]], 0), dt),
                                     torch.cat([sd[p + ".q.bias"], sd[p + ".k.bias"]]).float().contiguous()),
                                 v=(pack.pack_linear(sd[p + ".v.weight"], dt), f32(p + ".v.bias")),
                                 o=(pack.pack_linear(sd[p + ".proj_out.weight"], dt), f32(p + ".proj_out.bias")))))
        enc.append(("res", resnet("encoder.mid.block_2")))
        P["enc"] = enc
        wq2 = sd["quant_conv.weight"].float().reshape(2 * self.embed_dim, 2 * zc)
        wfold = torch.einsum("om,mikl->oikl", wq2, sd["encoder.conv_out.weight"].float())
        bfold = wq2 @ sd["encoder.conv_out.bias"].float() + sd["quant_conv.bias"].float()
        P["enc_head"] = (norm("encoder.norm_out"), pack.pack_conv2d(wfold, dt), bfold.contiguous())
        if self.adaptorconfig is not None:
            ad = self.adaptorconfig
            P["enc_adaptor_in"] = (pack.pack_conv2d(sd["encoder_adaptor.conv_in.weight"], dt, cin_pad=ka), f32("encoder_adaptor.conv_in.bias"))
            P["enc_adaptor"] = [resnet(f"encoder_adaptor.down.0.block.{b}") for b in range(ad["num_res_blocks"])]
            wo = torch.zeros((ka,) + tuple(sd["encoder_adaptor.conv_out.weight"].shape[1:]), device=dev)
            wo[: ad["in_channels"]] = sd["encoder_adaptor.conv_out.weight"]
            bo = torch.zeros((ka,), device=dev)
            bo[: ad["in_channels"]] = sd["encoder_adaptor.conv_out.bias"]
            P["enc_adaptor_head"] = (norm("encoder_adaptor.norm_out"), pack.pack_conv2d(wo, dt), bo.contiguous())
        self._packed = P
        return P

    @property
    def presplit(self):
        from .unet import PRESPLIT
        return bool(self.compute_dtype.x3) and PRESPLIT

    def _resnet(self, e, x, F_, H, W):
        sp = "f16" if e.get("x2") else self.presplit
        a = ops.groupnorm(x, *e["gn1"], F=F_, HW=H * W, eps=1e-6, silu=True, split_out=sp)
        h, _, _ = ops.conv2d(a, *e["c1"], F=F_, Hin=H, Win=W, KH=3, KW=3, pad=1, gn_stats=True)
        a = ops.groupnorm(h, *e["gn2"], F=F_, HW=H * W, eps=1e-6, silu=True, split_out=sp)
        skip = ops.linear(x, *e["nin"]) if "nin" in e else x
        out, _, _ = ops.conv2d(a, *e["c2"], F=F_, Hin=H, Win=W, KH=3, KW=3, pad=1, residual=skip, gn_stats=True)
        return out

    ATTN_SCRATCH_BYTES = 2 << 30

    def _attn(self, e, x, F_, H, W):
        N, C_ = H * W, x.shape[1]
        dt = x.dtype
        x3 = self.compute_dtype.x3
        ka = ops.k_align(self.compute_dtype)
        Np = (N + ka - 1) // ka * ka
        hn = ops.groupnorm(x, *e["norm"], F=F_, HW=N, eps=1e-6)
        qk = ops.linear(hn, *e["qk"])
        wv, bv = e["v"]
        vt = torch.zeros((F_ * C_, Np), device=x.device, dtype=dt) if Np != N else torch.empty((F_ * C_, N), device=x.device, dtype=dt)
        ops.batched_gemm(wv, hn, vt, batch=F_, M=C_, N=N, K=C_, a_bs=0, b_bs=N * C_, o_bs=C_ * Np, bias=bv, bias_per_row=True)
        o = torch.empty((F_ * N, C_), device=x.device, dtype=dt)
        esz = torch.empty((), dtype=dt).element_size()
        fc = max(1, min(F_, int(self.ATTN_SCRATCH_BYTES // (N * (4 * N + esz * Np)))))
        scores = torch.empty((fc * N, N), device=x.device, dtype=torch.float32)
        probs = torch.zeros((fc * N, Np), device=x.device, dtype=dt) if Np != N else torch.empty((fc * N, N), device=x.device, dtype=dt)
        lib = ops._lib.load()
        for f0 in range(0, F_, fc):
            nf = min(fc, F_ - f0)
            qk_c = qk[f0 * N:(f0 + nf) * N]
            ops.batched_gemm(qk_c[:, :C_], qk_c[:, C_:], scores, batch=nf, M=N, N=N, K=C_, a_bs=N * 2 * C_, b_bs=N * 2 * C_,
                             o_bs=N * N, alpha=float(int(C_) ** -0.5), x3=x3)
            ops._lib.check(lib.geo4d_softmax_rows(scores.data_ptr(), N, probs.data_ptr(), Np, nf * N, N, 1.0, ops.dt_code(dt),
                                                  ops._stream()), "geo4d_softmax_rows")
            ops.batched_gemm(probs, vt[f0 * C_:(f0 + nf) * C_], o[f0 * N:(f0 + nf) * N], batch=nf, M=N, N=C_, K=Np, a_bs=N * Np,
                             b_bs=C_ * Np, o_bs=N * C_, x3=x3)
        return ops.linear(o, *e["o"], residual=x, gn_stats=True)

    def decoder_features(self, z):
        P = self._packed or self._pack()
        n, zc, H, W = z.shape
        dt = self.storage_dtype
        x = ops.tokens_from_ncthw(z.float().reshape(n, zc, 1, H, W).contiguous(), None, P["cpad"], dt)
        x = ops.linear(x, *P["pq"])
        x, _, _ = ops.conv2d(x, *P["conv_in"], F=n, Hin=H, Win=W, KH=3, KW=3, pad=1, gn_stats=True)
        for kind, p, ci, co in self.plan:
            if kind == "res":
                x = self._resnet(P[p], x, n, H, W)
            elif kind == "attn":
                x = self._attn(P[p], x, n, H, W)
            else:
                from .unet import PRESPLIT_UP
                a = ops.cast_f16(x) if ops.is_x2_weight(P[p][0]) else ops.presplit(x) if (self.presplit and PRESPLIT_UP) else x
                x, H, W = ops.conv2d(a, *P[p], F=n, Hin=H, Win=W, KH=3, KW=3, pad=1, ups=2, gn_stats=True)
        return x, H, W

    def _head(self, head, feat, F_, H, W, out, T, nchw_channels):
        gn, w, b = head
        a = ops.groupnorm(feat, *gn, F=F_, HW=H * W, eps=1e-6, silu=True, split_out=self.presplit)
        ops.conv2d(a, w, b, F=F_, Hin=H, Win=W, KH=3, KW=3, pad=1, T=T, out=out, out_nchw=True, nchw_channels=nchw_channels)

    def _conf(self, P, feat, F_, H, W):
        h = feat
        for e in P["adaptor"]:
            h = self._resnet(e, h, F_, H, W)
        return h

    @torch.no_grad()
    def decode(self, z, **kwargs):
        n = z.shape[0]
        feat, H, W = self.decoder_features(z)
        P = self._packed
        out = torch.empty((n, self.ddconfig["out_ch"], H, W), device=z.device, dtype=torch.float32)
        self._head(P["head"], feat, n, H, W, out, 1, self.ddconfig["out_ch"])
        return out

    @torch.no_grad()
    def decode_with_conf_adaptor(self, z, **kwargs):
        if self.adaptorconfig is None:
            raise RuntimeError("decode_with_conf_adaptor needs adaptorconfig")
        n = z.shape[0]
        feat, H, W = self.decoder_features(z)
        P = self._packed
        c_rgb, c_conf = self.ddconfig["out_ch"], self.adaptorconfig["out_ch"]
        out = torch.empty((n, c_rgb + c_conf, H, W), device=z.device, dtype=torch.float32)
        self._head(P["head"], feat, n, H, W, out, 1, c_rgb + c_conf)
        self._head(P["adaptor_head"], self._conf(P, feat, n, H, W), n, H, W, out[:, c_rgb:], 1, c_rgb + c_conf)
        return out

    def _moments(self, x, with_adaptor):
        P = self._packed or self._pack()
        n, ci, H, W = x.shape
        nlev = len(self.ddconfig["ch_mult"])
        if H % (1 << (nlev - 1)) or W % (1 << (nlev - 1)):
            raise ValueError(f"encode: H, W must be multiples of {1 << (nlev - 1)} (got {H}x{W})")
        dt = self.storage_dtype
        t = ops.tokens_from_ncthw(x.float().reshape(n, ci, 1, H, W).contiguous(), None, P["cpad"], dt)
        if with_adaptor:
            if self.adaptorconfig is None:
                raise RuntimeError("encode_with_adaptor needs adaptorconfig")
            h, _, _ = ops.conv2d(t, *P["enc_adaptor_in"], F=n, Hin=H, Win=W, KH=3, KW=3, pad=1)
            for e in P["enc_adaptor"]:
                h = self._resnet(e, h, n, H, W)
            gn, w, b = P["enc_adaptor_head"]
            a = ops.groupnorm(h, *gn, F=n, HW=H * W, eps=1e-6, silu=True, split_out=self.presplit)
            t, _, _ = ops.conv2d(a, w, b, F=n, Hin=H, Win=W, KH=3, KW=3, pad=1, residual=t)
        h, _, _ = ops.conv2d(t, *P["enc_in"], F=n, Hin=H, Win=W, KH=3, KW=3, pad=1)
        for kind, e in P["enc"]:
            if kind == "res":
                h = self._resnet(e, h, n, H, W)
            elif kind == "attn":
                h = self._attn(e, h, n, H, W)
            else:
                h, H, W = ops.conv2d(h, *e, F=n, Hin=H, Win=W, KH=3, KW=3, stride=2, pad=0, pad_end=1)
        out = torch.empty((n, 2 * self.embed_dim, H, W), device=x.device, dtype=torch.float32)
        self._head(P["enc_head"], h, n, H, W, out, 1, 2 * self.embed_dim)
        return out

    @torch.no_grad()
    def encode(self, x, **kwargs):
        return DiagonalGaussianDistribution(self._moments(x, False))

    @torch.no_grad()
    def encode_with_adaptor(self, x, **kwargs):
        return DiagonalGaussianDistribution(self._moments(x, True))

    def forward(self, *a, **k):
        raise NotImplementedError("training forward is out of scope; use decode / decode_with_conf_adaptor")
```

### include/geo4d_hip.h

```cpp
#ifndef GEO4D_HIP_H
#define GEO4D_HIP_H
#include <stddef.h>
#ifdef __cplusplus
extern "C" {
#endif

#define GEO4D_ABI_VERSION 9

typedef struct geo4d_conv_gemm_t {
    const void* A;
    const void* W;
    void* O;
    const float* bias;
    const float* rowbias;
    const void* R;
    const void* zeros;
    void* workspace;
    size_t workspace_bytes;
    long lda, ldw, ldo, ldr;
    long ldrb;
    long a_bs, w_bs, o_bs, r_bs;
    int M, N, K, batch;
    int Cin;
    int T, Hin, Win, Hout, Wout;
    int KT, KH, KW, pt, ph, pw, stride, ups;
    int rowbias_div;
    int bias_per_row;
    int act;
    int dtype;
    int out_dtype;
    int out_nchw;
    int tile_hint;
    int split_k;
    int debug_ablate;
    float alpha;
    int a_split, w_split;
    int o_split;
    float* gn_colsum;
    unsigned long long* sat_count;
} geo4d_conv_gemm_t;
int geo4d_conv_gemm(const geo4d_conv_gemm_t* p, void* stream);
typedef struct geo4d_conv_gemm_plan_t {
    int tile_hint;
    int generation;
    int bm, bn, wm, wn;
    int splits;
    int hot;
    int osplit;
    int colsum_rows;
} geo4d_conv_gemm_plan_t;
int geo4d_conv_gemm_plan(const geo4d_conv_gemm_t* p, geo4d_conv_gemm_plan_t* plan);
typedef struct geo4d_conv_gemm_tile_t {
    int tile_hint, generation, bm, bn, wm, wn;
    int geglu;
} geo4d_conv_gemm_tile_t;
int geo4d_conv_gemm_tiles(geo4d_conv_gemm_tile_t* out, int cap);
int geo4d_conv_gemm_colsum_rows(const geo4d_conv_gemm_t* p);

typedef struct geo4d_groupnorm_t {
    const void* x; void* y;
    const float* gamma; const float* beta;
    void* workspace; size_t workspace_bytes;
    long ldx, ldy;
    int F, HW, C, groups, frames_per_stat;
    int act;
    int dtype;
    float eps;
    const float* colsum;
    int split_out;
    int colsum_rows;
    unsigned long long* sat_count;
} geo4d_groupnorm_t;
size_t geo4d_groupnorm_workspace(int F, int HW, int groups, int frames_per_stat);
int geo4d_groupnorm(const geo4d_groupnorm_t* p, void* stream);

typedef struct geo4d_groupnorm_src_t {
    const float* colsum;
    int rows;
    int c0, channels;
} geo4d_groupnorm_src_t;
typedef struct geo4d_groupnorm2_t {
    geo4d_groupnorm_t base;
    geo4d_groupnorm_src_t src[2];
    int nsrc;
    int path;
    float fuse_fraction;
    int min_workgroups;
} geo4d_groupnorm2_t;
enum {
    GEO4D_GN_PATH_PARTIAL = 1,
    GEO4D_GN_PATH_COLS = 2,
    GEO4D_GN_PATH_FUSED = 3,
    GEO4D_GN_PATH_SLICED = 4
};
typedef struct geo4d_groupnorm_plan_t {
    int path;
    int launches;
    int rows_per_wg;
    int nchunk;
    int channel_slices;
    int stat_slices;
    size_t workspace_bytes;
} geo4d_groupnorm_plan_t;
int geo4d_groupnorm_plan(const geo4d_groupnorm2_t* p, geo4d_groupnorm_plan_t* plan);
int geo4d_groupnorm2(const geo4d_groupnorm2_t* p, void* stream);

int geo4d_layernorm(const void* x, long ldx, void* y, long ldy, int M, int C, float eps, const float* gamma,
                    const float* beta, int dtype, void* stream);

int geo4d_layernorm_split(const void* x, long ldx, void* y, long ldy, int M, int C, float eps, const float* gamma,
                          const float* beta, int fmt, unsigned long long* sat_count, void* stream);

int geo4d_softmax_rows(const float* x, long ldx, void* y, long ldy, long rows, int cols, float scale, int out_dtype,
                       void* stream);
int geo4d_softmax_rows_causal(const float* x, long ldx, void* y, long ldy, long rows, int cols, float scale, int out_dtype,
                              int causal_period, void* stream);

typedef struct geo4d_attention_t {
    const void* q; void* o;
    const void* k[2]; const void* vt[2];
    const void* zeros;
    long ldq, ldo, ldk[2], ldvt[2], vt_bs[2];
    int Nk[2], kv_div[2];
    int B, H, Nq, nseg, head_dim, dtype;
    float scale;
    int split_out;
    int variant;
    int qkv_split;
} geo4d_attention_t;
typedef struct geo4d_attention_plan_t {
    int kernel;
    int nseg;
    int qb;
    int occ;
    int ps;
    int rows_per_wg;
    unsigned grid[3];
    int variant;
} geo4d_attention_plan_t;
int geo4d_attention_plan(const geo4d_attention_t* p, geo4d_attention_plan_t* plan);
// ... 119 lines not shown
```

Before: 6.906.

## Replace nearest-upsample 3x3 conv with four folded 2x2 subpixel-phase convs

Nearest-neighbour 2x upsampling followed by a 3x3 convolution is rewritten as four 2x2 convolutions, one per output phase, each reading the source-resolution input. Each phase's weights are folded from the 3x3 kernel at pack time. New up2 kernel variants write rows through a phase-aware output map and keep the fused group-norm column sums. This cuts the K dimension from 9*Cin to 4*Cin, removing redundant MACs on duplicated pixels, at the cost of extra packed weights, new kernel instantiations and restriction to the bf16x3 f32-output path.

```diff
diff --git a/geo4d_amd/_lib.py b/geo4d_amd/_lib.py
--- a/geo4d_amd/_lib.py
+++ b/geo4d_amd/_lib.py
@@ -122,6 +122,8 @@
     "geo4d_conv_gemm_plan": (C.c_int, [C.POINTER(ConvGemm), C.POINTER(ConvGemmPlan)]),
     "geo4d_conv_gemm_tiles": (C.c_int, [C.POINTER(ConvGemmTile), C.c_int]),
     "geo4d_conv_gemm_colsum_rows": (C.c_int, [C.POINTER(ConvGemm)]),
+    "geo4d_conv_gemm_up2": (C.c_int, [C.POINTER(ConvGemm), C.c_int, C.c_int, C.c_void_p]),
+    "geo4d_conv_gemm_up2_plan": (C.c_int, [C.POINTER(ConvGemm), C.c_int, C.c_int, C.POINTER(ConvGemmPlan)]),
     "geo4d_groupnorm_workspace": (C.c_size_t, [C.c_int, C.c_int, C.c_int, C.c_int]),
     "geo4d_groupnorm": (C.c_int, [C.POINTER(GroupNorm), C.c_void_p]),
     "geo4d_groupnorm_plan": (C.c_int, [C.POINTER(GroupNorm2), C.POINTER(GroupNormPlan)]),
diff --git a/geo4d_amd/csrc/gemm.hip b/geo4d_amd/csrc/gemm.hip
--- a/geo4d_amd/csrc/gemm.hip
+++ b/geo4d_amd/csrc/gemm.hip
@@ -11,6 +11,8 @@
 extern template int launch_v3_typed<bf16_t>(const geo4d_conv_gemm_t&, const Plan&, hipStream_t);
 extern template int launch_v3_typed<bf16x3_t>(const geo4d_conv_gemm_t&, const Plan&, hipStream_t);
 extern template int launch_v3_typed<f16x2p_t>(const geo4d_conv_gemm_t&, const Plan&, hipStream_t);
+extern template int launch_v2_up2<bf16x3_t>(const geo4d_conv_gemm_t&, const Plan&, hipStream_t);
+extern template int launch_v3_up2<bf16x3_t>(const geo4d_conv_gemm_t&, const Plan&, hipStream_t);
 
 template <typename T>
 static int launch_v23(const geo4d_conv_gemm_t& p, const Plan& plan, hipStream_t s) {
@@ -58,6 +60,35 @@
     return GEO4D_OK;
 }
 
+static int conv_gemm_up2_plan(const geo4d_conv_gemm_t* p, int src_w, int phase, Plan& plan) {
+    if (!p) return GEO4D_EINVAL;
+    const char* error = validate(*p);
+    if (!error) {
+        plan = resolve_up2(*p, src_w, phase);
+        error = plan.error;
+    }
+    if (error) geo4d_set_error(error);
+    return error ? GEO4D_EINVAL : GEO4D_OK;
+}
+
+extern "C" int geo4d_conv_gemm_up2(const geo4d_conv_gemm_t* pp, int src_w, int phase, void* stream) {
+    Plan plan;
+    const int rc = conv_gemm_up2_plan(pp, src_w, phase, plan);
+    if (rc != GEO4D_OK) return rc;
+    hipStream_t s = (hipStream_t)stream;
+    return generation(plan.hint) == 2 ? launch_v2_up2<bf16x3_t>(*pp, plan, s) : launch_v3_up2<bf16x3_t>(*pp, plan, s);
+}
+
+extern "C" int geo4d_conv_gemm_up2_plan(const geo4d_conv_gemm_t* pp, int src_w, int phase, geo4d_conv_gemm_plan_t* out) {
+    Plan plan;
+    if (!out) return GEO4D_EINVAL;
+    const int rc = conv_gemm_up2_plan(pp, src_w, phase, plan);
+    if (rc != GEO4D_OK) return rc;
+    const Tile& t = *find_tile(plan.hint);
+    *out = {t.hint, generation(t.hint), t.bm, t.bn, t.wm, t.wn, plan.splits, plan.hot, plan.osplit, plan.colsum_rows};
+    return GEO4D_OK;
+}
+
 extern "C" int geo4d_conv_gemm_tiles(geo4d_conv_gemm_tile_t* out, int cap) {
     int n = 0;
     for (const Tile& t : TILES) {
diff --git a/geo4d_amd/csrc/gemm_epilogue.h b/geo4d_amd/csrc/gemm_epilogue.h
--- a/geo4d_amd/csrc/gemm_epilogue.h
+++ b/geo4d_amd/csrc/gemm_epilogue.h
@@ -22,6 +22,18 @@
     const bool geglu = !partial && p.act == 2;
     return EpiDest{O, partial ? (long)p.N : p.ldo, partial ? 0 : bz * p.o_bs, odt, odt == GEO4D_F32 ? 4 : 2, geglu ? (p.N >> 1) : p.N, geglu};
 }
+
+struct Up2Map {
+    int w, phase;
+    __device__ __forceinline__ long row(const int m) const {
+        const int q = m / w;
+        return 4L * w * q + 2 * (m - q * w) + (phase >> 1) * 2 * w + (phase & 1);
+    }
+};
+
+struct Up2Args { int w, phase; };
+__host__ __device__ __forceinline__ Up2Args up2_args() { return Up2Args{0, 0}; }
+__host__ __device__ __forceinline__ Up2Args up2_args(const Up2Args& a) { return a; }
 
 template <bool GELU = true>
 __device__ __forceinline__ float epi_value(const geo4d_conv_gemm_t& p, const float acc, const float brow, const long rboff, const int n, const bool inb = true) {
diff --git a/geo4d_amd/csrc/gemm_kernel.h b/geo4d_amd/csrc/gemm_kernel.h
--- a/geo4d_amd/csrc/gemm_kernel.h
+++ b/geo4d_amd/csrc/gemm_kernel.h
@@ -13,7 +13,7 @@
 static_assert(BKC * 16 == KSLAB_BYTES, "gemm_plan.h counts K slabs of BKC 16-byte chunks");
 
 template <int BM, int NT>
-__device__ __forceinline__ void fill_gather_table(const geo4d_conv_gemm_t& p, const int tm, const int ntap, const int hw, int* rowpix, const int tid) {
+__device__ __forceinline__ void fill_gather_table(const geo4d_conv_gemm_t& p, const int tm, const int ntap, const int hw, int* rowpix, const int tid, const int ph, const int pw) {
     const int hlim = p.ups == 2 ? 2 * p.Hin : p.Hin, wlim = p.ups == 2 ? 2 * p.Win : p.Win;
     const int ush = p.ups == 2 ? 1 : 0;
     for (int e = tid; e < BM * ntap; e += NT) {
@@ -25,13 +25,17 @@
             const int oy = rem / p.Wout, ox = rem - oy * p.Wout;
             const int kt = tap / (p.KH * p.KW), r2 = tap - kt * (p.KH * p.KW);
             const int ky = r2 / p.KW, kx = r2 - ky * p.KW;
-            const int iy = oy * p.stride - p.ph + ky, ix = ox * p.stride - p.pw + kx;
+            const int iy = oy * p.stride - ph + ky, ix = ox * p.stride - pw + kx;
             const int tt = (f % p.T) + kt - p.pt;
             if ((unsigned)iy < (unsigned)hlim && (unsigned)ix < (unsigned)wlim && (unsigned)tt < (unsigned)p.T)
                 pix = ((f + kt - p.pt) * p.Hin + (iy >> ush)) * p.Win + (ix >> ush);
         }
         rowpix[e] = pix;
     }
+}
+template <int BM, int NT>
+__device__ __forceinline__ void fill_gather_table(const geo4d_conv_gemm_t& p, const int tm, const int ntap, const int hw, int* rowpix, const int tid) {
+    fill_gather_table<BM, NT>(p, tm, ntap, hw, rowpix, tid, p.ph, p.pw);
 }
 template <int HOT> __device__ __forceinline__ bool a_is_split(const geo4d_conv_gemm_t& p) { return HOT ? (HOT == 2) : (p.a_split != 0); }
 template <int HOT> __device__ __forceinline__ bool w_is_split(const geo4d_conv_gemm_t& p) { return HOT ? true : (p.w_split != 0); }
@@ -565,6 +569,8 @@
 
 template <typename T> int launch_v2_typed(const geo4d_conv_gemm_t& p, const Plan& plan, hipStream_t stream);
 template <typename T> int launch_v3_typed(const geo4d_conv_gemm_t& p, const Plan& plan, hipStream_t stream);
+template <typename T> int launch_v2_up2(const geo4d_conv_gemm_t& p, const Plan& plan, hipStream_t stream);
+template <typename T> int launch_v3_up2(const geo4d_conv_gemm_t& p, const Plan& plan, hipStream_t stream);
 
 template <typename T>
 int launch_typed(const geo4d_conv_gemm_t& p, const Plan& plan, hipStream_t stream) {
diff --git a/geo4d_amd/csrc/gemm_kernel_v2.h b/geo4d_amd/csrc/gemm_kernel_v2.h
--- a/geo4d_amd/csrc/gemm_kernel_v2.h
+++ b/geo4d_amd/csrc/gemm_kernel_v2.h
@@ -65,16 +65,23 @@
     v += __int_as_float(__builtin_amdgcn_mov_dpp(__float_as_int(v), 0x140, 0xF, 0xF, true));
     return v;
 }
-template <int MB, int NB, typename Store>
+template <int MB, int NB, typename Store, bool UP2 = false>
 __device__ __forceinline__ void wide_plain(const geo4d_conv_gemm_t& p, const f32x4 (&acc)[MB][NB], const EpiDest& d, const bool partial, const bool has_res, const long rbase,
-                                           const int m_w0, const int n_w0, const int lr, const int lq) {
+                                           const int m_w0, const int n_w0, const int lr, const int lq, const Up2Map map = Up2Map{0, 0}) {
     constexpr unsigned OOB = EPI_OOB;
     const long ldo = d.ldo;
     const float alpha = partial ? 1.0f : p.alpha;
     const bool hb = !partial && p.bias != nullptr && !p.bias_per_row;
     const bool hr = !partial && p.bias != nullptr && p.bias_per_row;
     const bool ht = !partial && p.rowbias != nullptr;
-    const __amdgpu_buffer_rsrc_t rsO = tile_rsrc((float*)d.O + d.obase + (long)m_w0 * ldo + n_w0);
+    long row0 = m_w0;
+    unsigned offU[MB];
+    if constexpr (UP2) {
+        row0 = map.row(m_w0);
+#pragma unroll
+        for (int a = 0; a < MB; ++a) offU[a] = (unsigned)((map.row(m_w0 + a * 16 + lr) - row0) * ldo + 4 * lq) * 4u;
+    }
+    const __amdgpu_buffer_rsrc_t rsO = tile_rsrc((float*)d.O + d.obase + row0 * ldo + n_w0);
     const __amdgpu_buffer_rsrc_t rsR = tile_rsrc(has_res ? (const void*)((const float*)p.R + rbase + (long)m_w0 * p.ldr + n_w0) : p.zeros, has_res);
     const int mleft = p.M - m_w0;
     const __amdgpu_buffer_rsrc_t rsB = bias_rsrc(p, hb, n_w0);
@@ -84,7 +91,8 @@
     const unsigned offO = (unsigned)(lr * (int)ldo + 4 * lq) * 4u, offR = (unsigned)(lr * (int)p.ldr + 4 * lq) * 4u;
     const unsigned rowO = (unsigned)ldo * 64u, rowR = (unsigned)p.ldr * 64u;
     const bool gn = !partial && p.gn_colsum != nullptr && m_w0 < p.M;
-    const __amdgpu_buffer_rsrc_t rsC = tile_rsrc(gn ? (const void*)(p.gn_colsum + ((long)(m_w0 / (16 * MB)) * p.N + n_w0) * 2) : p.zeros, gn);
+    const long chunk = UP2 ? (long)(m_w0 / (16 * MB)) * 4 + map.phase : (long)(m_w0 / (16 * MB));
+    const __amdgpu_buffer_rsrc_t rsC = tile_rsrc(gn ? (const void*)(p.gn_colsum + (chunk * p.N + n_w0) * 2) : p.zeros, gn);
     unsigned offT[MB];
 #pragma unroll
     for (int a = 0; a < MB; ++a) offT[a] = 0u;
@@ -122,7 +130,8 @@
                 tu = __builtin_amdgcn_raw_buffer_load_b128(rsT, (colok ? offT[a + 1 < MB ? a + 1 : a] : OOB) + 64u * b, 0, 0);
                 bru = __builtin_amdgcn_raw_buffer_load_b32(rsBr, (unsigned)(lr + 16 * (a + 1)) * 4u, 0, 0);
             }
-            Store::store(c, rsO, (ok ? offO + a * rowO : OOB) + 64u * b);
+            if constexpr (UP2) Store::store(c, rsO, (ok ? offU[a] : OOB) + 64u * b);
+            else Store::store(c, rsO, (ok ? offO + a * rowO : OOB) + 64u * b);
         }
         if (gn) {
 #pragma unroll
@@ -213,10 +222,13 @@
     }
 }
 
-template <typename T, int MB, int NB, bool OSPLIT, bool VECONLY = false>
+template <typename T, int MB, int NB, bool OSPLIT, bool VECONLY = false, bool UP2 = false>
 __device__ __forceinline__ void reg_epilogue(const geo4d_conv_gemm_t& p, const f32x4 (&acc)[MB][NB], const int m_w0, const int n_w0,
-                                             const long e_bz, const int e_kz, const bool partial, const int lr, const int lq) {
+                                             const long e_bz, const int e_kz, const bool partial, const int lr, const int lq, const Up2Map map = Up2Map{0, 0}) {
     const EpiDest d = epi_dest(p, partial, e_kz, e_bz);
+    if constexpr (UP2) {
+        return wide_plain<MB, NB, StoreF32, true>(p, acc, d, false, false, 0, m_w0, n_w0, lr, lq, map);
+    }
     const int odt = d.odt, oesz = d.oesz;
     const bool geglu = d.geglu;
     const bool has_res = !partial && p.R != nullptr;
@@ -245,8 +257,11 @@
 template <int BM, int BN>
 constexpr int v2_smem_bytes() { return (2 * BM + 2 * BN) * PITCH + BM * MAXTAP * 4; }
 
-template <typename T, int BM, int BN, int WM, int WN, int HOT, bool OSPLIT = false>
-__global__ __launch_bounds__(WM * WN * 64) void conv_gemm_v2_kernel(const geo4d_conv_gemm_t p, const int splits, const int tiles_mn) {
+template <typename T, int BM, int BN, int WM, int WN, int HOT, bool OSPLIT = false, typename... Up>
+__global__ __launch_bounds__(WM * WN * 64) void conv_gemm_v2_kernel(const geo4d_conv_gemm_t p, const int splits, const int tiles_mn, const Up... up) {
+    constexpr bool UP2 = sizeof...(Up) != 0;
+    static_assert(!UP2 || !OSPLIT, "the mapped epilogue writes plain f32 rows");
+    const int up_w = up2_args(up...).w, up_phase = up2_args(up...).phase;
     constexpr int NT = WM * WN * 64;
     constexpr int EPC = Elem<T>::EPC;
     constexpr int BK = BKC * EPC;
@@ -318,7 +333,12 @@
         const int s_begin = kz * per;
         nslab = min(nslab_all, s_begin + per) - s_begin;
         if (!direct_rows) {
-            fill_gather_table<BM, NT>(p, tm, ntap, hw, rowpix, tid);
+            if constexpr (UP2) {
+                const int phase = up_phase < 0 ? (int)bz : up_phase;
+                fill_gather_table<BM, NT>(p, tm, ntap, hw, rowpix, tid, 1 - (phase >> 1), 1 - (phase & 1));
+            } else {
+                fill_gather_table<BM, NT>(p, tm, ntap, hw, rowpix, tid);
+            }
             __syncthreads();
         }
         tap = tapB = s_begin % ntap;
@@ -406,7 +426,11 @@
 
     const bool partial = splits > 1;
     auto epilogue = [&](int e_tm, int e_tn, long e_bz, int e_kz) {
-        reg_epilogue<T, MB, NB, OSPLIT>(p, acc, e_tm * BM + wr * WTM, e_tn * BN + wc * WTN, e_bz, e_kz, partial, lr, lq);
+        if constexpr (UP2)
+            reg_epilogue<T, MB, NB, false, false, true>(p, acc, e_tm * BM + wr * WTM, e_tn * BN + wc * WTN, e_bz, e_kz, false, lr, lq,
+                                                        Up2Map{up_w, up_phase < 0 ? (int)e_bz : up_phase});
+        else
+            reg_epilogue<T, MB, NB, OSPLIT>(p, acc, e_tm * BM + wr * WTM, e_tn * BN + wc * WTN, e_bz, e_kz, partial, lr, lq);
     };
 
     long w = xcd_remap((long)blockIdx.x, G);
@@ -448,15 +472,23 @@
 struct GenV2 {
     template <typename T, int BM, int BN, int WM, int WN, int HOT, bool OSPLIT>
     static auto kernel() { return conv_gemm_v2_kernel<T, BM, BN, WM, WN, HOT, OSPLIT>; }
+    template <typename T, int BM, int BN, int WM, int WN, int HOT>
+    static auto kernel_up2() { return conv_gemm_v2_kernel<T, BM, BN, WM, WN, HOT, false, Up2Args>; }
     template <int BM, int BN> static constexpr int smem() { return v2_smem_bytes<BM, BN>(); }
 };
 
-template <typename G, typename T, int BM, int BN, int WM, int WN, int HOT, bool OSPLIT = false>
+template <typename G, typename T, int BM, int BN, int WM, int WN, int HOT, bool OSPLIT, bool UP2>
+auto persistent_kernel() {
+    if constexpr (UP2) return G::template kernel_up2<T, BM, BN, WM, WN, HOT>();
+    else return G::template kernel<T, BM, BN, WM, WN, HOT, OSPLIT>();
+}
+
+template <typename G, typename T, int BM, int BN, int WM, int WN, int HOT, bool OSPLIT = false, bool UP2 = false>
 int launch_persistent(const geo4d_conv_gemm_t& p, const Plan& plan, hipStream_t stream) {
     constexpr int smem = G::template smem<BM, BN>();
     static_assert(smem <= 160 * 1024, "LDS");
     static int resident = 0;
-    auto kern = G::template kernel<T, BM, BN, WM, WN, HOT, OSPLIT>();
+    auto kern = persistent_kernel<G, T, BM, BN, WM, WN, HOT, OSPLIT, UP2>();
     if (!resident) {
         if (hipFuncSetAttribute((const void*)kern, hipFuncAttributeMaxDynamicSharedMemorySize, smem) != hipSuccess) {
             geo4d_set_error("hipFuncSetAttribute(max dynamic LDS) failed");
@@ -474,7 +506,8 @@
     const long total = (long)tiles_mn * p.batch * plan.splits;
     const long cap = p.debug_ablate == 2 ? 3 : resident;
     const unsigned grid = (unsigned)(total < cap ? total : cap);
-    hipLaunchKernelGGL(kern, dim3(grid), dim3(WM * WN * 64), smem, stream, p, plan.splits, tiles_mn);
+    if constexpr (UP2) hipLaunchKernelGGL(kern, dim3(grid), dim3(WM * WN * 64), smem, stream, p, plan.splits, tiles_mn, Up2Args{plan.up_w, plan.up_phase});
+    else hipLaunchKernelGGL(kern, dim3(grid), dim3(WM * WN * 64), smem, stream, p, plan.splits, tiles_mn);
     GEO4D_CHECK_LAUNCH();
     if (plan.splits > 1) return launch_splitk_reduce<T>(p, plan, stream);
     return GEO4D_OK;
@@ -510,4 +543,20 @@
     return GEO4D_EINVAL;
 }
 
-}
+template <typename G, typename T, int BM, int BN, int WM, int WN>
+int launch_persistent_up2(const geo4d_conv_gemm_t& p, const Plan& plan, hipStream_t stream) {
+    if (plan.hot == 2) return launch_persistent<G, T, BM, BN, WM, WN, 2, false, true>(p, plan, stream);
+    return launch_persistent<G, T, BM, BN, WM, WN, 1, false, true>(p, plan, stream);
+}
+template <typename T>
+int launch_v2_up2(const geo4d_conv_gemm_t& p, const Plan& plan, hipStream_t stream) {
+    switch (plan.hint) {
+        case 22: return launch_persistent_up2<GenV2, T, 256, 256, 4, 2>(p, plan, stream);
+        case 23: return launch_persistent_up2<GenV2, T, 160, 320, 2, 4>(p, plan, stream);
+        case 25: return launch_persistent_up2<GenV2, T, 128, 128, 2, 2>(p, plan, stream);
+    }
+    geo4d_set_error("conv_gemm_up2: no second-generation kernel for this tile_hint");
+    return GEO4D_EINVAL;
+}
+
+}
diff --git a/geo4d_amd/csrc/gemm_kernel_v3.h b/geo4d_amd/csrc/gemm_kernel_v3.h
--- a/geo4d_amd/csrc/gemm_kernel_v3.h
+++ b/geo4d_amd/csrc/gemm_kernel_v3.h
@@ -13,8 +13,11 @@
         __builtin_amdgcn_sched_barrier(0);      \
     } while (0)
 
-template <typename T, int BM, int BN, int WM, int WN, int HOT, bool OSPLIT = false>
-__global__ __launch_bounds__(512) void conv_gemm_v3_kernel(const geo4d_conv_gemm_t p, const int splits, const int tiles_mn) {
+template <typename T, int BM, int BN, int WM, int WN, int HOT, bool OSPLIT = false, typename... Up>
+__global__ __launch_bounds__(512) void conv_gemm_v3_kernel(const geo4d_conv_gemm_t p, const int splits, const int tiles_mn, const Up... up) {
+    constexpr bool UP2 = sizeof...(Up) != 0;
+    static_assert(!UP2 || !OSPLIT, "the mapped epilogue writes plain f32 rows");
+    const int up_w = up2_args(up...).w, up_phase = up2_args(up...).phase;
     static_assert(WM * WN == 8, "two groups of four waves");
     static_assert(!std::is_same<T, float>::value, "v3 serves the 16-bit MFMA forms (bf16, bf16x3)");
     constexpr int EPC = Elem<T>::EPC;
@@ -101,13 +104,19 @@
         }
         refresh_B();
     };
-    auto tap0_pixel = [&](int m) -> long {
+    auto tap0_pixel = [&](int m, int ph, int pw) -> long {
         const int f = m / hw, rem = m - f * hw;
         const int oy = rem / p.Wout, ox = rem - oy * p.Wout;
-        return ((long)(f - p.pt) * p.Hin + (oy * p.stride - p.ph)) * p.Win + (ox * p.stride - p.pw);
+        return ((long)(f - p.pt) * p.Hin + (oy * p.stride - ph)) * p.Win + (ox * p.stride - pw);
     };
     auto window_A = [&](bool valid, int tm_, long bz_) {
-        const long P0 = valid ? tap0_pixel(tm_ * BM) : 0;
+        int ph = p.ph, pw = p.pw;
+        if constexpr (UP2) {
+            const int phase = up_phase < 0 ? (int)bz_ : up_phase;
+            ph = 1 - (phase >> 1);
+            pw = 1 - (phase & 1);
+        }
+        const long P0 = valid ? tap0_pixel(tm_ * BM, ph, pw) : 0;
         rA = __builtin_amdgcn_make_buffer_rsrc((void*)((const char*)p.A + (bz_ * p.a_bs + P0 * p.lda) * ESZ_A), 0, OOB, 0x00020000);
 #pragma unroll
         for (int h = 0; h < 2; ++h) {
@@ -119,7 +128,7 @@
                 if (valid && row >= 0 && m < p.M) {
                     const int f = m / hw, rem = m - f * hw;
                     const int oy = rem / p.Wout, ox = rem - oy * p.Wout;
-                    const int iy0 = oy * p.stride - p.ph, ix0 = ox * p.stride - p.pw, ft = (f % p.T) - p.pt;
+                    const int iy0 = oy * p.stride - ph, ix0 = ox * p.stride - pw, ft = (f % p.T) - p.pt;
                     const long px0 = ((long)(f - p.pt) * p.Hin + iy0) * p.Win + ix0;
                     off = (unsigned)(((px0 - P0) * p.lda + chunkA(j)) * ESZ_A);
                     unsigned bit = 1;
@@ -369,7 +378,11 @@
         {
             int lr_ = lr, lq_ = lq;
             asm volatile("" : "+v"(lr_), "+v"(lq_));
-            reg_epilogue<T, MB, NB, OSPLIT, true>(p, acc, tmC * BM + wr * WTM, tnC * BN + wc * WTN, bzC, kzC, partial, lr_, lq_);
+            if constexpr (UP2)
+                reg_epilogue<T, MB, NB, false, true, true>(p, acc, tmC * BM + wr * WTM, tnC * BN + wc * WTN, bzC, kzC, false, lr_, lq_,
+                                                           Up2Map{up_w, up_phase < 0 ? (int)bzC : up_phase});
+            else
+                reg_epilogue<T, MB, NB, OSPLIT, true>(p, acc, tmC * BM + wr * WTM, tnC * BN + wc * WTN, bzC, kzC, partial, lr_, lq_);
         }
         __builtin_amdgcn_s_waitcnt(0x0F70);
         if (!validS) break;
@@ -381,6 +394,8 @@
 struct GenV3 {
     template <typename T, int BM, int BN, int WM, int WN, int HOT, bool OSPLIT>
     static auto kernel() { return conv_gemm_v3_kernel<T, BM, BN, WM, WN, HOT, OSPLIT>; }
+    template <typename T, int BM, int BN, int WM, int WN, int HOT>
+    static auto kernel_up2() { return conv_gemm_v3_kernel<T, BM, BN, WM, WN, HOT, false, Up2Args>; }
     template <int BM, int BN> static constexpr int smem() { return v3_smem_bytes<BM, BN>(); }
 };
 
@@ -398,6 +413,16 @@
     return GEO4D_EINVAL;
 }
 
+template <typename T>
+int launch_v3_up2(const geo4d_conv_gemm_t& p, const Plan& plan, hipStream_t stream) {
+    switch (plan.hint) {
+        case 71: return launch_persistent_up2<GenV3, T, 192, 256, 2, 4>(p, plan, stream);
+        case 72: return launch_persistent_up2<GenV3, T, 160, 320, 2, 4>(p, plan, stream);
+    }
+    geo4d_set_error("conv_gemm_up2: no third-generation kernel for this tile_hint");
+    return GEO4D_EINVAL;
+}
+
 #undef GEO4D_V3_BAR
 
 }
diff --git a/geo4d_amd/csrc/gemm_plan.h b/geo4d_amd/csrc/gemm_plan.h
--- a/geo4d_amd/csrc/gemm_plan.h
+++ b/geo4d_amd/csrc/gemm_plan.h
@@ -38,6 +38,7 @@
     int hot = 0;
     bool osplit = false;
     int colsum_rows = 0;
+    int up_w = 0, up_phase = 0;
     const char* error = nullptr;
 };
 
@@ -212,4 +213,34 @@
     return pl;
 }
 
-}
+inline Plan resolve_up2(const geo4d_conv_gemm_t& p, int src_w, int phase) {
+    Plan pl;
+    auto refuse = [&pl](const char* why) { pl.error = why; pl.colsum_rows = 0; return pl; };
+    if (p.dtype != GEO4D_BF16X3 || !p.w_split)
+        return refuse("conv_gemm_up2: the sub-pixel form serves bf16x3 (dtype 3) against a pre-split weight; the other modes keep the ups = 2 gather");
+    if (p.ups != 1 || p.KT != 1 || p.KH != 2 || p.KW != 2 || p.stride != 1 || p.pt != 0 || src_w <= 0 || p.Win != src_w || p.Wout != src_w || p.Hout != p.Hin)
+        return refuse("conv_gemm_up2: the descriptor must be the 2x2 stride-1 convolution on the source grid (ups = 1, Hout = Hin, Wout = Win = src_w)");
+    if (phase < -1 || phase > 3) return refuse("conv_gemm_up2: phase must be 2 py + px (0..3), or -1 for the four phases in the batch index");
+    if (phase >= 0 ? (p.batch != 1 || p.ph != 1 - (phase >> 1) || p.pw != 1 - (phase & 1)) : (p.batch != 4 || p.a_bs != 0 || p.o_bs != 0))
+        return refuse("conv_gemm_up2: a phase launch has batch 1, ph = 1 - py, pw = 1 - px; the batch form has batch 4 with a_bs = o_bs = 0");
+    if (p.split_k > 1) return refuse("conv_gemm_up2: no split-K (the reduce kernel writes unmapped rows)");
+    if (p.act != 0 || p.R || p.rowbias || p.bias_per_row || p.out_nchw || p.o_split || p.out_dtype != GEO4D_F32 || (p.N & 3) || (p.ldo & 3) || !aligned(p.O, 16))
+        return refuse("conv_gemm_up2: the mapped epilogue writes plain f32 rows with a column bias only (N % 4 == 0, 16-byte aligned rows)");
+    if ((4L * (128 + src_w) + 2L * src_w) * p.ldo * 4 >= (1L << 31)) return refuse("conv_gemm_up2: a wave tile's output rows span more than the 2 GB buffer window");
+    geo4d_conv_gemm_t q = p;
+    q.batch = 1;
+    q.gn_colsum = nullptr;
+    q.split_k = 1;
+    pl = resolve(q);
+    if (pl.error) return pl;
+    if (pl.hint != 22 && pl.hint != 23 && pl.hint != 25 && pl.hint != 71 && pl.hint != 72)
+        return refuse("conv_gemm_up2: the mapped epilogue lives on tile hints 22, 23, 25, 71 and 72");
+    if ((p.Hin * p.Win) % (pl.colsum_rows ? pl.colsum_rows : 1)) pl.colsum_rows = 0;
+    if (p.gn_colsum && (!pl.colsum_rows || !aligned(p.gn_colsum, 16)))
+        return refuse("conv_gemm_up2: this launch cannot emit gn_colsum: it needs a frame's source rows and M to be multiples of the wave tile's rows");
+    pl.up_w = src_w;
+    pl.up_phase = phase;
+    return pl;
+}
+
+}
diff --git a/geo4d_amd/csrc/gemm_v2_bf16x3_up2.hip b/geo4d_amd/csrc/gemm_v2_bf16x3_up2.hip
--- /dev/null
+++ b/geo4d_amd/csrc/gemm_v2_bf16x3_up2.hip
@@ -0,0 +1,5 @@
+#include "gemm_kernel_v2.h"
+
+namespace geo4d_gemm {
+template int launch_v2_up2<bf16x3_t>(const geo4d_conv_gemm_t&, const Plan&, hipStream_t);
+}
diff --git a/geo4d_amd/csrc/gemm_v3_bf16x3_up2.hip b/geo4d_amd/csrc/gemm_v3_bf16x3_up2.hip
--- /dev/null
+++ b/geo4d_amd/csrc/gemm_v3_bf16x3_up2.hip
@@ -0,0 +1,5 @@
+#include "gemm_kernel_v3.h"
+
+namespace geo4d_gemm {
+template int launch_v3_up2<bf16x3_t>(const geo4d_conv_gemm_t&, const Plan&, hipStream_t);
+}
diff --git a/geo4d_amd/ops.py b/geo4d_amd/ops.py
--- a/geo4d_amd/ops.py
+++ b/geo4d_amd/ops.py
@@ -339,7 +339,7 @@
     return plan if _lib.load().geo4d_conv_gemm_plan(C.byref(p), C.byref(plan)) == 0 else None
 
 
-def _launch_config(p, launch):
+def _launch_config(p, launch, plan_on=_plan_on):
     def may_measure():
         return AUTOTUNE and not torch.cuda.is_current_stream_capturing()
     key = f"{p.dtype}/{p.out_dtype}|{p.M}x{p.N}x{p.K}|c{p.Cin}|t{p.KT}{p.KH}{p.KW}s{p.stride}u{p.ups}|a{p.act}r{int(bool(p.R))}n{p.out_nchw}|b{p.batch}"
@@ -347,7 +347,7 @@
         key += f"|x{int(bool(p.a_split))}{p.w_split}" + ("o" if p.o_split else "")
     cfg = _tuned_config(_tune_table(), key, p.dtype, p.a_split, p.w_split, p.o_split, may_measure)
     if cfg is None and may_measure():
-        cfg = _autotune(launch, key, lambda tile, split: _plan_on(p, tile, split) is not None)
+        cfg = _autotune(launch, key, lambda tile, split: plan_on(p, tile, split) is not None)
     cfg = cfg if cfg is not None else (0, 0)
     return _f16_rows_config(cfg, p.act) if p.o_split == 2 else cfg
 
@@ -431,6 +431,70 @@
               ldr=_ld(residual) if residual is not None else 0, act=act, out_nchw=out_nchw, tile_hint=tile_hint,
               split_k=split_k, gn_stats=gn_stats)
     return out, Hout, Wout
+
+
+UP_SUBPIXEL = _env_level("GEO4D_UP_SUBPIXEL", 1)
+UP2_FORM = _os.environ.get("GEO4D_UP2_FORM", "batch")
+UP2_MIN_ROWS = 2048
+_UP2_TILES = (22, 23, 25, 71, 72)
+_UP2_SUMS_TILE = {71: 22}
+
+
+def up_subpixel(x, w4, rows):
+    return bool(UP_SUBPIXEL) and w4 is not None and rows >= UP2_MIN_ROWS and (isinstance(x, SplitAct) or x.dtype == torch.float32)
+
+
+def _up2_plan_on(p, src_w, phase):
+    def plan_on(p_, tile_hint, split_k):
+        if split_k != 1 or tile_hint not in _UP2_TILES:
+            return None
+        p_.tile_hint, p_.split_k = tile_hint, 1
+        plan = ConvGemmPlan()
+        return plan if _lib.load().geo4d_conv_gemm_up2_plan(C.byref(p_), src_w, phase, C.byref(plan)) == 0 else None
+    return plan_on
+
+
+def conv2d_up2(x, w4, bias, *, F, Hin, Win, out=None, gn_stats=False, tile_hint=0, form=None):
+    lib = _lib.load()
+    Cin, N, M = act_k(x), w4.shape[1], F * Hin * Win
+    assert w4.dim() == 3 and w4.shape[0] == 4 and w4.stride(2) == 1 and kdim(w4[0], x) == 4 * Cin, (w4.shape, Cin)
+    assert x.shape[0] == M, (x.shape, F, Hin, Win)
+    if out is None:
+        out = torch.empty((4 * M, N), device=x.device, dtype=torch.float32)
+    assert out.dim() == 2 and out.shape[0] == 4 * M and out.dtype == torch.float32 and not isinstance(out, SplitAct)
+    batched = (form or UP2_FORM) == "batch"
+    p = conv_gemm_descriptor(x, w4[0], out, M=M, N=N, K=4 * Cin, Cin=Cin, lda=_ld(x), ldw=w4.stride(1), ldo=_ld(out), Hin=Hin, Win=Win,
+                             Hout=Hin, Wout=Win, KH=2, KW=2, ph=1, pw=1, bias=bias, batch=4 if batched else 1,
+                             w_bs=w4.stride(0) if batched else 0, tile_hint=tile_hint, split_k=1)
+    if getattr(out, "_gn_colsum", None) is not None:
+        out._gn_colsum, out._gn_colsum_rows, out._gn_colsum_tag = None, 32, None
+    phases = (-1,) if batched else (0, 1, 2, 3)
+
+    def launch(tile, split):
+        p.tile_hint, p.split_k = tile, 1
+        for ph in phases:
+            if ph >= 0:
+                p.W, p.ph, p.pw = w4[ph].data_ptr(), 1 - (ph >> 1), 1 - (ph & 1)
+            _lib.check(lib.geo4d_conv_gemm_up2(C.byref(p), Win, ph, _stream()), "geo4d_conv_gemm_up2")
+
+    plan_on = _up2_plan_on(p, Win, phases[0])
+    if tile_hint == 0:
+        tile_hint = _launch_config(p, launch, plan_on)[0] or (72 if M >= 8192 else 25)
+    if gn_stats and GN_FUSED_STATS:
+        rows = getattr(plan_on(p, tile_hint, 1), "colsum_rows", 0)
+        if rows == 0 and tile_hint in _UP2_SUMS_TILE:
+            rows = getattr(plan_on(p, _UP2_SUMS_TILE[tile_hint], 1), "colsum_rows", 0)
+            tile_hint = _UP2_SUMS_TILE[tile_hint] if rows > 0 else tile_hint
+        if rows > 0:
+            cs = torch.empty((4 * M // rows, N, 2), device=out.device, dtype=torch.float32)
+            p.gn_colsum = cs.data_ptr()
+            out._gn_colsum, out._gn_colsum_rows = cs, rows
+            out._gn_colsum_tag = (out.data_ptr(), out._version)
+    if GEMM_TIMELINE is None:
+        launch(tile_hint, 1)
+    else:
+        _on_timeline(GEMM_TIMELINE, lambda: launch(tile_hint, 1), 2.0 * 4 * M * N * p.K, 3)
+    return out, 2 * Hin, 2 * Win
 
 
 def conv_temporal(x, w, bias, *, B, T, HW, residual=None, out=None, gn_stats=False, tile_hint=0, split_k=0):
diff --git a/geo4d_amd/pack.py b/geo4d_amd/pack.py
--- a/geo4d_amd/pack.py
+++ b/geo4d_amd/pack.py
@@ -82,6 +82,21 @@
     return cast(w.reshape(co, kh * kw * cp), dtype)
 
 
+def fold_up2(w):
+    assert w.shape[2:] == (3, 3), w.shape
+    r = torch.tensor([[[1, 0, 0], [0, 1, 1]], [[1, 1, 0], [0, 0, 1]]], dtype=torch.float64, device=w.device)
+    w64 = w.double()
+    return torch.stack([torch.einsum("ak,oikl,bl->oiab", r[py], w64, r[px]) for py in (0, 1) for px in (0, 1)]).float()
+
+
+def up2_row(m, W, py, px):
+    return 4 * W * (m // W) + 2 * (m % W) + py * 2 * W + px
+
+
+def pack_conv2d_up2(w, dtype):
+    return torch.stack([pack_conv2d(f, dtype) for f in fold_up2(w)])
+
+
 def pack_conv3d_t(w, dtype):
     co, ci, kt, kh, kw = w.shape
     assert kh == 1 and kw == 1
diff --git a/geo4d_amd/unet.py b/geo4d_amd/unet.py
--- a/geo4d_amd/unet.py
+++ b/geo4d_amd/unet.py
@@ -324,6 +324,7 @@
                 e["w"], e["b"] = pack.pack_conv2d(sd[p + ".op.weight"], dt), f32(p + ".op.bias")
             elif L.kind == "up":
                 e["w"], e["b"] = pack.pack_conv2d(sd[p + ".conv.weight"], dt), f32(p + ".conv.bias")
+                e["w4"] = pack.pack_conv2d_up2(sd[p + ".conv.weight"], dt) if dt.x3 else None
             P[p] = e
         P["emb_w"], P["emb_b"] = torch.cat(emb_w, 0).contiguous(), torch.cat(emb_b, 0).contiguous()
         P["k_text"] = pack.pack_linear(torch.cat(k_text, 0), dt)
@@ -495,7 +496,10 @@
                 h, H, W = ops.conv2d(h, e["w"], e["b"], F=B * T, Hin=H, Win=W, KH=3, KW=3, stride=2, pad=1, gn_stats=True, out=o)
             elif L.kind == "up":
                 a = ops.presplit(h) if (self.presplit and PRESPLIT_UP) else h
-                h, H, W = ops.conv2d(a, e["w"], e["b"], F=B * T, Hin=H, Win=W, KH=3, KW=3, pad=1, ups=2, out=o)
+                if ops.up_subpixel(a, e["w4"], B * T * H * W):
+                    h, H, W = ops.conv2d_up2(a, e["w4"], e["b"], F=B * T, Hin=H, Win=W, out=o)
+                else:
+                    h, H, W = ops.conv2d(a, e["w"], e["b"], F=B * T, Hin=H, Win=W, KH=3, KW=3, pad=1, ups=2, out=o)
         return h, H, W
 
     @torch.no_grad()
diff --git a/geo4d_amd/vae.py b/geo4d_amd/vae.py
--- a/geo4d_amd/vae.py
+++ b/geo4d_amd/vae.py
@@ -161,6 +161,7 @@
             else:
                 up2 = bool(dt.two_pass("vaeup") and self.presplit)
                 P[p] = ((pack.pack_conv2d_x2 if up2 else pack.pack_conv2d)(sd[p + ".weight"], dt), f32(p + ".bias"))
+                P[p + ".w4"] = pack.pack_conv2d_up2(sd[p + ".weight"], dt) if (dt.x3 and not up2) else None
         P["head"] = (norm("decoder.norm_out"), pack.pack_conv2d(sd["decoder.conv_out.weight"], dt), f32("decoder.conv_out.bias"))
         P["head_mean"] = (P["head"][0], pack.pack_conv2d(sd["decoder.conv_out.weight"].mean(0, keepdim=True), dt),
                           sd["decoder.conv_out.bias"].mean().reshape(1).float().contiguous())
@@ -262,7 +263,10 @@
             else:
                 from .unet import PRESPLIT_UP
                 a = ops.cast_f16(x) if ops.is_x2_weight(P[p][0]) else ops.presplit(x) if (self.presplit and PRESPLIT_UP) else x
-                x, H, W = ops.conv2d(a, *P[p], F=n, Hin=H, Win=W, KH=3, KW=3, pad=1, ups=2, gn_stats=True)
+                if ops.up_subpixel(a, P[p + ".w4"], n * H * W):
+                    x, H, W = ops.conv2d_up2(a, P[p + ".w4"], P[p][1], F=n, Hin=H, Win=W, gn_stats=True)
+                else:
+                    x, H, W = ops.conv2d(a, *P[p], F=n, Hin=H, Win=W, KH=3, KW=3, pad=1, ups=2, gn_stats=True)
         return x, H, W
 
     def _head(self, head, feat, F_, H, W, out, T, nchw_channels):
diff --git a/include/geo4d_hip.h b/include/geo4d_hip.h
--- a/include/geo4d_hip.h
+++ b/include/geo4d_hip.h
@@ -56,6 +56,8 @@
 } geo4d_conv_gemm_tile_t;
 int geo4d_conv_gemm_tiles(geo4d_conv_gemm_tile_t* out, int cap);
 int geo4d_conv_gemm_colsum_rows(const geo4d_conv_gemm_t* p);
+int geo4d_conv_gemm_up2(const geo4d_conv_gemm_t* p, int src_w, int phase, void* stream);
+int geo4d_conv_gemm_up2_plan(const geo4d_conv_gemm_t* p, int src_w, int phase, geo4d_conv_gemm_plan_t* plan);
 
 typedef struct geo4d_groupnorm_t {
     const void* x; void* y;
```

Measured after the change: 7.121 (median of 6 runs). +3.1%, better.
